# MIT-SPARK/TEASER-plusplus

Measured on AMD Instinct MI355X. Metric: registrations/sec at N=10000 correspondences, 95% outliers, higher is better.
Workload: dtype bf16x3-split MFMA + f32 filter with FP64 fix-up for K1 (bitmap bit-identical to FP64); f64 estimators

## Files before the change

include/teaser_hip.h:

```cpp
#ifndef TEASER_HIP_H_
#define TEASER_HIP_H_

#include <stddef.h>
#include <stdint.h>

#ifdef __cplusplus
extern "C" {
#endif

#define TEASER_HIP_ABI_VERSION 1

#if defined(__GNUC__)
#define TEASER_HIP_API __attribute__((visibility("default")))
#else
#define TEASER_HIP_API
#endif

typedef enum teaser_hip_status {
  TEASER_HIP_OK = 0,
  TEASER_HIP_ERR_BAD_ARG = 1,
  TEASER_HIP_ERR_HIP = 2,
  TEASER_HIP_ERR_NO_DEVICE = 3,
  TEASER_HIP_ERR_UNSUPPORTED = 4,
  TEASER_HIP_ERR_TIME_LIMIT = 5,
// ... 53 lines not shown
  float rotation_ms;
  float translation_ms;
  float d2h_ms;
  float total_ms;
  int64_t tim_graph_pairs;
  int64_t tim_graph_bytes;
  float colour_ms;
  float tim_aux_ms;
} teaser_profile_c;

typedef struct teaser_hip_solver teaser_hip_solver;

TEASER_HIP_API int32_t teaser_hip_params_default(teaser_params_c* params);

TEASER_HIP_API int32_t teaser_hip_solver_create(const teaser_params_c* params, int32_t device,
                                 teaser_hip_solver** out);
TEASER_HIP_API int32_t teaser_hip_solver_destroy(teaser_hip_solver* h);

TEASER_HIP_API int32_t teaser_hip_solver_reset(teaser_hip_solver* h, const teaser_params_c* params);
TEASER_HIP_API int32_t teaser_hip_solver_get_params(const teaser_hip_solver* h, teaser_params_c* params);

TEASER_HIP_API int32_t teaser_hip_solve(teaser_hip_solver* h, const double* src, const double* dst, int32_t n,
                         teaser_solution_c* out);

TEASER_HIP_API int32_t teaser_hip_solve_device(teaser_hip_solver* h, const double* d_src, const double* d_dst,
                                int32_t n, teaser_solution_c* out);

TEASER_HIP_API int32_t teaser_hip_solve_correspondences(teaser_hip_solver* h, const float* src_cloud_xyz,
                                         int32_t n_src, const float* dst_cloud_xyz, int32_t n_dst,
                                         const int32_t* corr_pairs ,
                                         int32_t n_corr, teaser_solution_c* out);

TEASER_HIP_API int32_t teaser_hip_solve_batch(teaser_hip_solver* h, const double* const* src,
                               const double* const* dst, const int32_t* n, int32_t batch,
                               teaser_solution_c* out );

TEASER_HIP_API int32_t teaser_hip_solve_batch_device(teaser_hip_solver* h, const double* d_src,
                                      const double* d_dst, const int64_t* point_offset,
                                      const int32_t* n, int32_t batch, teaser_solution_c* out);

enum { TEASER_HIP_INPUT_DEVICE = 0, TEASER_HIP_INPUT_HOST = 1 };
TEASER_HIP_API int32_t teaser_hip_submit_batch(teaser_hip_solver* h, const double* src, const double* dst,
                                const int64_t* point_offset, const int32_t* n, int32_t batch,
                                int32_t flags, int32_t* ticket);
TEASER_HIP_API int32_t teaser_hip_wait(teaser_hip_solver* h, int32_t ticket, teaser_solution_c* out );
TEASER_HIP_API int32_t teaser_hip_set_pipeline_depth(teaser_hip_solver* h, int32_t depth );

typedef struct teaser_hip_multi teaser_hip_multi;
TEASER_HIP_API int32_t teaser_hip_multi_create(const teaser_params_c* params, const int32_t* devices,
                                int32_t n_devices , teaser_hip_multi** out);
TEASER_HIP_API int32_t teaser_hip_multi_destroy(teaser_hip_multi* mh);
TEASER_HIP_API int32_t teaser_hip_multi_solve_batch(teaser_hip_multi* mh, const double* const* src,
                                     const double* const* dst, const int32_t* n, int32_t batch,
                                     teaser_solution_c* out );
TEASER_HIP_API int32_t teaser_hip_multi_route(teaser_hip_multi* mh, int32_t problem, teaser_hip_solver** h,
                               int32_t* local_problem);
TEASER_HIP_API int32_t teaser_hip_multi_device_count(const teaser_hip_multi* mh);

#define TEASER_HIP_COMM_ID_BYTES 128
typedef struct teaser_hip_comm teaser_hip_comm;
TEASER_HIP_API int32_t teaser_hip_comm_shard(int64_t total, int32_t rank, int32_t world, int64_t* first, int64_t* last);
TEASER_HIP_API int32_t teaser_hip_comm_unique_id(uint8_t* id );
TEASER_HIP_API int32_t teaser_hip_comm_create(const uint8_t* id, int32_t rank, int32_t world, int32_t device,
                               teaser_hip_comm** out);
TEASER_HIP_API int32_t teaser_hip_comm_destroy(teaser_hip_comm* c);
TEASER_HIP_API int32_t teaser_hip_comm_gather_solutions(teaser_hip_comm* c, const teaser_solution_c* local,
                                         int64_t n_local, int64_t total, teaser_solution_c* all );
TEASER_HIP_API int32_t teaser_hip_comm_gather_indices(teaser_hip_comm* c, teaser_hip_solver* h, int64_t n_local,
                                       int64_t total, int32_t k_max, int32_t* lens, int32_t* indices);
TEASER_HIP_API const char* teaser_hip_comm_last_error(const teaser_hip_comm* c);

TEASER_HIP_API int32_t teaser_hip_get_max_clique(teaser_hip_solver* h, int32_t problem, int32_t* buf, int64_t* len);
TEASER_HIP_API int32_t teaser_hip_get_rotation_inliers(teaser_hip_solver* h, int32_t problem, int32_t* buf,
                                        int64_t* len);
TEASER_HIP_API int32_t teaser_hip_get_translation_inliers(teaser_hip_solver* h, int32_t problem, int32_t* buf,
                                           int64_t* len);
TEASER_HIP_API int32_t teaser_hip_get_input_ordered_translation_inliers(teaser_hip_solver* h, int32_t problem,
                                                         int32_t* buf, int64_t* len);
TEASER_HIP_API int32_t teaser_hip_get_inlier_graph_bitmap(teaser_hip_solver* h, int32_t problem, uint64_t* buf,
                                           int64_t* len );
TEASER_HIP_API int32_t teaser_hip_get_degrees(teaser_hip_solver* h, int32_t problem, int32_t* buf, int64_t* len);
TEASER_HIP_API int32_t teaser_hip_get_inlier_graph_rows(teaser_hip_solver* h, int32_t problem, uint64_t* buf,
                                         int64_t* len , int32_t* stride_words);

TEASER_HIP_API int32_t teaser_hip_solve_for_rotation(teaser_hip_solver* h, const double* src, const double* dst,
                                      int32_t k, double noise_bound, double* rotation_rowmajor,
                                      uint8_t* inlier_mask, double* cost, int32_t* iterations);
TEASER_HIP_API int32_t teaser_hip_solve_for_translation(teaser_hip_solver* h, const double* src,
                                         const double* dst, int32_t k, double* translation,
                                         uint8_t* inlier_mask);
TEASER_HIP_API int32_t teaser_hip_scalar_tls(teaser_hip_solver* h, const double* x, const double* ranges,
                              int32_t n, double* estimate, uint8_t* inlier_mask);
TEASER_HIP_API int32_t teaser_hip_solve_for_scale(teaser_hip_solver* h, const double* v1, const double* v2,
                                   int64_t m, double* scale, uint8_t* inlier_mask);

TEASER_HIP_API int32_t teaser_hip_compute_fpfh(teaser_hip_solver* h, const float* cloud_xyz, int32_t n,
                                double normal_radius, double fpfh_radius, float* fpfh_out,
                                float* normals_out);
TEASER_HIP_API int32_t teaser_hip_match_features(teaser_hip_solver* h, const float* src_feat, int32_t n_src,
                                  const float* dst_feat, int32_t n_dst, int32_t dim, int32_t use_crosscheck,
                                  int32_t* pairs, int64_t* n_pairs);
TEASER_HIP_API int32_t teaser_hip_tuple_test(teaser_hip_solver* h, const float* src_xyz, int32_t n_src,
                              const float* dst_xyz, int32_t n_dst, float tuple_scale, uint64_t seed,
                              int32_t* pairs , int64_t* n_pairs );

typedef struct teaser_certifier_params_c {
  double noise_bound;
  double cbar2;
  double sub_optimality;
  double max_iterations;
  double gamma_tau;
} teaser_certifier_params_c;
typedef struct teaser_certification_c {
  int32_t is_optimal;
  int32_t iterations;
  double best_suboptimality;
} teaser_certification_c;
TEASER_HIP_API int32_t teaser_hip_certifier_params_default(teaser_certifier_params_c* p);
TEASER_HIP_API int32_t teaser_hip_certifier_warmup(int32_t device);
TEASER_HIP_API int32_t teaser_hip_certify(teaser_hip_solver* h, const teaser_certifier_params_c* p, const double* R,
                           const double* src, const double* dst, const double* theta, int32_t n,
                           teaser_certification_c* out, double* traj, int32_t traj_cap);
TEASER_HIP_API int32_t teaser_hip_certify_dual_projection(teaser_hip_solver* h, const double* W, const double* theta,
                                                          int32_t n, double* W_dual);
TEASER_HIP_API int32_t teaser_hip_certify_stages(teaser_hip_solver* h, const teaser_certifier_params_c* p, const double* R,
                                                 const double* src, const double* dst, const double* theta, int32_t n,
                                                 int32_t iteration, double* stages, double* traj, int32_t traj_cap,
                                                 teaser_certification_c* out);

TEASER_HIP_API int32_t teaser_hip_max_clique(teaser_hip_solver* h, const uint64_t* bitmap, int32_t n,
                              int32_t* clique, int32_t* clique_size, int32_t* exact_run);

TEASER_HIP_API int32_t teaser_hip_set_profiling(teaser_hip_solver* h, int32_t level );
TEASER_HIP_API int32_t teaser_hip_set_option(teaser_hip_solver* h, const char* name, int64_t value);
TEASER_HIP_API int32_t teaser_hip_get_option(const char* name, int64_t* value);
TEASER_HIP_API int32_t teaser_hip_get_profile(const teaser_hip_solver* h, teaser_profile_c* out);
TEASER_HIP_API void* teaser_hip_get_stream(teaser_hip_solver* h);
TEASER_HIP_API const char* teaser_hip_last_error(const teaser_hip_solver* h);
TEASER_HIP_API int32_t teaser_hip_abi_version(void);
TEASER_HIP_API int32_t teaser_hip_device_count(void);

typedef struct teaser_icp_params_c {
  double max_correspondence_distance;
  int32_t max_iteration;
  double relative_fitness;
  double relative_rmse;
} teaser_icp_params_c;
typedef struct teaser_icp_result_c {
  double transformation[16];
  double fitness;
  double inlier_rmse;
  int32_t iterations;
  int32_t n_correspondences;
} teaser_icp_result_c;
typedef struct teaser_hip_icp teaser_hip_icp;
TEASER_HIP_API int32_t teaser_hip_icp_params_default(teaser_icp_params_c* params);
TEASER_HIP_API int32_t teaser_hip_icp_create(int32_t device, teaser_hip_icp** out);
TEASER_HIP_API int32_t teaser_hip_icp_destroy(teaser_hip_icp* icp);
TEASER_HIP_API const char* teaser_hip_icp_last_error(const teaser_hip_icp* icp);
TEASER_HIP_API int32_t teaser_hip_icp_fill_scratch(teaser_hip_icp* icp, int32_t byte, int64_t* bytes_out);
TEASER_HIP_API int32_t teaser_hip_icp_batch(teaser_hip_icp* icp, int32_t batch, const double* const* src,
                                            const int32_t* n_src, const double* const* dst, const int32_t* n_dst,
                                            const double* init, const teaser_icp_params_c* params,
                                            teaser_icp_result_c* out, int32_t* const* corr);
TEASER_HIP_API int32_t teaser_hip_icp_solve(teaser_hip_icp* icp, const double* src, int32_t n_src,
                                            const double* dst, int32_t n_dst, const double* init,
// ... 711 lines not shown
```

teaser-plusplus_amd/__init__.py:

```python
import ctypes as C
import enum
import os
import subprocess
import typing

import numpy as np

_HERE = os.path.dirname(os.path.abspath(__file__))
_CSRC = os.path.join(_HERE, "csrc")
LIB_PATH = os.path.join(_HERE, "libteaser_hip.so")

STATUS_NAMES = {0: "OK", 1: "BAD_ARG", 2: "HIP", 3: "NO_DEVICE", 4: "UNSUPPORTED", 5: "TIME_LIMIT",
                6: "SCRATCH", 7: "OOM", 8: "BUSY"}


class TeaserHipError(RuntimeError):
    def __init__(self, status, msg=""):
        self.status = status
        super().__init__("teaser_hip status %d (%s) %s" % (status, STATUS_NAMES.get(status, "?"), msg))


class RotationEstimationAlgorithm(enum.IntEnum):
    GNC_TLS = 0
    FGR = 1
    QUATRO = 2


class InlierSelectionMode(enum.IntEnum):
    PMC_EXACT = 0
    PMC_HEU = 1
    KCORE_HEU = 2
    NONE = 3


class InlierGraphFormulation(enum.IntEnum):
    CHAIN = 0
    COMPLETE = 1


class ParamsC(C.Structure):
    _fields_ = [
        ("noise_bound", C.c_double),
        ("cbar2", C.c_double),
        ("estimate_scaling", C.c_int32),
        ("rotation_estimation_algorithm", C.c_int32),
        ("rotation_gnc_factor", C.c_double),
        ("rotation_max_iterations", C.c_int64),
        ("rotation_cost_threshold", C.c_double),
        ("rotation_tim_graph", C.c_int32),
        ("inlier_selection_mode", C.c_int32),
        ("kcore_heuristic_threshold", C.c_double),
        ("use_max_clique", C.c_int32),
        ("max_clique_exact_solution", C.c_int32),
        ("max_clique_time_limit", C.c_double),
        ("max_clique_num_threads", C.c_int32),
    ]


class SolutionC(C.Structure):
    _fields_ = [
        ("valid", C.c_int32),
        ("status", C.c_int32),
        ("scale", C.c_double),
        ("rotation", C.c_double * 9),
        ("translation", C.c_double * 3),
        ("n", C.c_int32),
        ("clique_size", C.c_int32),
        ("n_rotation_inliers", C.c_int32),
        ("n_translation_inliers", C.c_int32),
        ("gnc_cost", C.c_double),
        ("gnc_iterations", C.c_int32),
        ("clique_exact_run", C.c_int32),
        ("heuristic_size", C.c_int32),
        ("colour_uncoloured", C.c_int32),
        ("num_edges", C.c_int64),
    ]


class ProfileC(C.Structure):
    _fields_ = [
        ("h2d_ms", C.c_float),
        ("tim_graph_ms", C.c_float),
        ("tim_graph_launches", C.c_int32),
        ("degree_ms", C.c_float),
        ("heuristic_ms", C.c_float),
        ("peel_ms", C.c_float),
        ("exact_ms", C.c_float),
        ("rotation_ms", C.c_float),
        ("translation_ms", C.c_float),
        ("d2h_ms", C.c_float),
        ("total_ms", C.c_float),
        ("tim_graph_pairs", C.c_int64),
        ("tim_graph_bytes", C.c_int64),
        ("colour_ms", C.c_float),
        ("tim_aux_ms", C.c_float),
    ]


EXPORTED_SYMBOLS = [
    "teaser_hip_params_default", "teaser_hip_solver_create", "teaser_hip_solver_destroy",
    "teaser_hip_solver_reset", "teaser_hip_solver_get_params", "teaser_hip_solve",
    "teaser_hip_solve_device", "teaser_hip_solve_correspondences", "teaser_hip_solve_batch",
    "teaser_hip_solve_batch_device", "teaser_hip_get_max_clique", "teaser_hip_get_rotation_inliers",
    "teaser_hip_get_translation_inliers", "teaser_hip_get_input_ordered_translation_inliers",
    "teaser_hip_get_inlier_graph_bitmap", "teaser_hip_get_inlier_graph_rows", "teaser_hip_get_degrees", "teaser_hip_solve_for_rotation",
    "teaser_hip_solve_for_translation", "teaser_hip_scalar_tls", "teaser_hip_max_clique",
    "teaser_hip_set_profiling", "teaser_hip_set_option", "teaser_hip_get_option", "teaser_hip_get_profile", "teaser_hip_get_stream",
    "teaser_hip_last_error", "teaser_hip_abi_version", "teaser_hip_device_count", "teaser_hip_host_alloc",
    "teaser_hip_host_free",
    "teaser_hip_synth_problem", "teaser_hip_submit_batch", "teaser_hip_wait",
    "teaser_hip_set_pipeline_depth", "teaser_hip_multi_create", "teaser_hip_multi_destroy",
    "teaser_hip_multi_solve_batch", "teaser_hip_multi_route", "teaser_hip_multi_device_count",
    "teaser_hip_solve_for_scale", "teaser_hip_compute_fpfh", "teaser_hip_match_features", "teaser_hip_tuple_test",
    "teaser_hip_certifier_params_default", "teaser_hip_certify", "teaser_hip_certifier_warmup",
    "teaser_hip_certify_dual_projection", "teaser_hip_certify_stages",
    "teaser_hip_comm_shard", "teaser_hip_comm_unique_id", "teaser_hip_comm_create", "teaser_hip_comm_destroy",
    "teaser_hip_comm_gather_solutions", "teaser_hip_comm_gather_indices", "teaser_hip_comm_last_error",
    "teaser_hip_icp_params_default", "teaser_hip_icp_create", "teaser_hip_icp_destroy", "teaser_hip_icp_last_error",
    "teaser_hip_icp_fill_scratch",
    "teaser_hip_icp_batch", "teaser_hip_icp_solve", "teaser_hip_icp_estimation_default", "teaser_hip_icp_batch_ex",
    "teaser_hip_icp_solve_ex", "teaser_hip_icp_batch_cov", "teaser_hip_icp_solve_cov",
    "teaser_hip_icp_covariances_batch", "teaser_hip_icp_normals_batch", "teaser_hip_icp_batch_auto",
    "teaser_hip_icp_solve_auto",
    "teaser_hip_icp_self_knn_batch", "teaser_hip_icp_remove_statistical_outliers_batch",
    "teaser_hip_icp_remove_radius_outliers_batch", "teaser_hip_icp_set_option", "teaser_hip_icp_get_option",
    "teaser_hip_icp_knn_search_batch", "teaser_hip_icp_hybrid_search_batch", "teaser_hip_icp_radius_search_batch",
    "teaser_hip_icp_fpfh_batch", "teaser_hip_icp_boundary_points_batch",
    "teaser_hip_icp_frame_default", "teaser_hip_icp_unproject_depth_batch", "teaser_hip_icp_project_depth_batch",
    "teaser_hip_icp_iss_params_default", "teaser_hip_icp_iss_keypoints_batch",
    "teaser_hip_icp_cluster_dbscan_batch", "teaser_hip_icp_farthest_point_down_sample_batch",
    "teaser_hip_icp_information_batch", "teaser_hip_icp_information",
    "teaser_hip_icp_color_default", "teaser_hip_icp_batch_color", "teaser_hip_icp_solve_color",
    "teaser_hip_icp_color_gradients_batch",
    "teaser_hip_voxel_create", "teaser_hip_voxel_destroy", "teaser_hip_voxel_last_error",
    "teaser_hip_voxel_fill_scratch",
    "teaser_hip_voxel_down_sample_batch", "teaser_hip_voxel_down_sample",
    "teaser_hip_features_create", "teaser_hip_features_destroy", "teaser_hip_features_last_error",
    "teaser_hip_features_fill_scratch",
    "teaser_hip_features_set_budgets", "teaser_hip_features_fpfh_batch", "teaser_hip_features_match_batch",
    "teaser_hip_features_correspondences_batch", "teaser_hip_features_knn_batch",
    "teaser_hip_features_match_knn_batch", "teaser_hip_features_correspondences_knn_batch",
    "teaser_hip_features_tuple_test_batch",
    "teaser_hip_posegraph_create", "teaser_hip_posegraph_destroy", "teaser_hip_posegraph_last_error",
    "teaser_hip_posegraph_fill_scratch",
    "teaser_hip_posegraph_option_default", "teaser_hip_posegraph_optimize_batch", "teaser_hip_posegraph_optimize",
    "teaser_hip_posegraph_linearize_batch", "teaser_hip_posegraph_linearize",
    "teaser_hip_ransac_create", "teaser_hip_ransac_destroy", "teaser_hip_ransac_last_error",
    "teaser_hip_ransac_fill_scratch",
    "teaser_hip_ransac_params_default", "teaser_hip_ransac_correspondence_batch", "teaser_hip_ransac_correspondence",
    "teaser_hip_ransac_set_option", "teaser_hip_ransac_get_option", "teaser_hip_ransac_trials_batch",
    "teaser_hip_fgr_create", "teaser_hip_fgr_destroy", "teaser_hip_fgr_last_error",
    "teaser_hip_fgr_fill_scratch", "teaser_hip_fgr_params_default",
    "teaser_hip_fgr_correspondence_batch", "teaser_hip_fgr_correspondence", "teaser_hip_fgr_set_option",
    "teaser_hip_fgr_get_option", "teaser_hip_fgr_iterations_batch",
    "teaser_hip_plane_create", "teaser_hip_plane_destroy", "teaser_hip_plane_last_error",
    "teaser_hip_plane_fill_scratch",
    "teaser_hip_plane_params_default", "teaser_hip_plane_segment_batch", "teaser_hip_plane_segment",
    "teaser_hip_plane_set_option", "teaser_hip_plane_get_option", "teaser_hip_plane_trials_batch",
    "teaser_hip_tsdf_volume_default", "teaser_hip_tsdf_create", "teaser_hip_tsdf_destroy", "teaser_hip_tsdf_last_error",
    "teaser_hip_tsdf_fill_scratch",
    "teaser_hip_tsdf_reset", "teaser_hip_tsdf_integrate_batch", "teaser_hip_tsdf_extract_point_cloud",
    "teaser_hip_tsdf_extract_voxel_point_cloud", "teaser_hip_tsdf_download", "teaser_hip_tsdf_upload",
    "teaser_hip_tsdf_extract_triangle_mesh", "teaser_hip_tsdf_mesh_tables", "teaser_hip_tsdf_view_default",
    "teaser_hip_tsdf_ray_cast_views",
    "teaser_hip_stsdf_volume_default", "teaser_hip_stsdf_create", "teaser_hip_stsdf_destroy", "teaser_hip_stsdf_last_error",
    "teaser_hip_stsdf_fill_scratch", "teaser_hip_stsdf_last_phases", "teaser_hip_stsdf_reset", "teaser_hip_stsdf_integrate_frames",
    "teaser_hip_stsdf_extract_point_cloud", "teaser_hip_stsdf_extract_voxel_point_cloud", "teaser_hip_stsdf_block_count",
    "teaser_hip_stsdf_block_keys", "teaser_hip_stsdf_download_blocks", "teaser_hip_stsdf_upload_blocks",
    "teaser_hip_stsdf_ray_cast_views", "teaser_hip_stsdf_extract_triangle_mesh",
    "teaser_hip_icp_odometry_option_default", "teaser_hip_icp_rgbd_odometry_batch",
    "teaser_hip_icp_rgbd_odometry_pyramid_batch",
]


def build(force=False):
    args = ["make", "-C", _CSRC, "-j8"]
    if force:
        args.append("-B")
    subprocess.check_call(args, stdout=subprocess.DEVNULL)
    return LIB_PATH


_lib = None
_vp, _ip, _dp = C.c_void_p, C.POINTER(C.c_int32), C.POINTER(C.c_double)
_u8p, _i64p, _u64p = C.POINTER(C.c_uint8), C.POINTER(C.c_int64), C.POINTER(C.c_uint64)


def lib():
    global _lib
    if _lib is not None:
        return _lib
    if not os.path.exists(LIB_PATH):
        raise ImportError("%s is missing: run __graft_entry__.build() (make -C %s)" % (LIB_PATH, _CSRC))
    os.environ.setdefault("GPU_MAX_HW_QUEUES", "8")
    L = C.CDLL(LIB_PATH)
    L.teaser_hip_host_alloc.argtypes = [C.c_size_t, C.POINTER(_vp)]
    L.teaser_hip_host_free.argtypes = [_vp]
    L.teaser_hip_params_default.argtypes = [C.POINTER(ParamsC)]
    L.teaser_hip_solver_create.argtypes = [C.POINTER(ParamsC), C.c_int32, C.POINTER(_vp)]
    L.teaser_hip_solver_destroy.argtypes = [_vp]
    L.teaser_hip_solver_reset.argtypes = [_vp, C.POINTER(ParamsC)]
    L.teaser_hip_solver_get_params.argtypes = [_vp, C.POINTER(ParamsC)]
    L.teaser_hip_solve.argtypes = [_vp, _dp, _dp, C.c_int32, C.POINTER(SolutionC)]
    L.teaser_hip_solve_device.argtypes = [_vp, _vp, _vp, C.c_int32, C.POINTER(SolutionC)]
    L.teaser_hip_solve_correspondences.argtypes = [_vp, C.POINTER(C.c_float), C.c_int32,
                                                   C.POINTER(C.c_float), C.c_int32, _ip, C.c_int32,
                                                   C.POINTER(SolutionC)]
    L.teaser_hip_solve_batch.argtypes = [_vp, C.POINTER(_dp), C.POINTER(_dp), _ip, C.c_int32,
                                         C.POINTER(SolutionC)]
    L.teaser_hip_solve_batch_device.argtypes = [_vp, _vp, _vp, _i64p, _ip, C.c_int32,
                                                C.POINTER(SolutionC)]
    for nm in ("teaser_hip_get_max_clique", "teaser_hip_get_rotation_inliers",
               "teaser_hip_get_translation_inliers",
               "teaser_hip_get_input_ordered_translation_inliers", "teaser_hip_get_degrees"):
        getattr(L, nm).argtypes = [_vp, C.c_int32, _ip, _i64p]
    L.teaser_hip_get_inlier_graph_bitmap.argtypes = [_vp, C.c_int32, _u64p, _i64p]
    L.teaser_hip_get_inlier_graph_rows.argtypes = [_vp, C.c_int32, _u64p, _i64p, _ip]
    L.teaser_hip_solve_for_rotation.argtypes = [_vp, _dp, _dp, C.c_int32, C.c_double, _dp, _u8p, _dp, _ip]
    L.teaser_hip_solve_for_translation.argtypes = [_vp, _dp, _dp, C.c_int32, _dp, _u8p]
    L.teaser_hip_scalar_tls.argtypes = [_vp, _dp, _dp, C.c_int32, _dp, _u8p]
    L.teaser_hip_solve_for_scale.argtypes = [_vp, _dp, _dp, C.c_int64, _dp, _u8p]
    _fp = C.POINTER(C.c_float)
    L.teaser_hip_compute_fpfh.argtypes = [_vp, _fp, C.c_int32, C.c_double, C.c_double, _fp, _fp]
    L.teaser_hip_match_features.argtypes = [_vp, _fp, C.c_int32, _fp, C.c_int32, C.c_int32, C.c_int32, _ip, _i64p]
    L.teaser_hip_tuple_test.argtypes = [_vp, _fp, C.c_int32, _fp, C.c_int32, C.c_float, C.c_uint64, _ip, _i64p]
    L.teaser_hip_certify.argtypes = [_vp, C.c_void_p, _dp, _dp, _dp, _dp, C.c_int32, C.c_void_p, _dp, C.c_int32]
    L.teaser_hip_certify_dual_projection.argtypes = [_vp, _dp, _dp, C.c_int32, _dp]
    L.teaser_hip_certify_stages.argtypes = [_vp, C.c_void_p, _dp, _dp, _dp, _dp, C.c_int32, C.c_int32, _dp, _dp,
                                            C.c_int32, C.c_void_p]
    L.teaser_hip_max_clique.argtypes = [_vp, _u64p, C.c_int32, _ip, _ip, _ip]
    L.teaser_hip_submit_batch.argtypes = [_vp, _vp, _vp, _i64p, _ip, C.c_int32, C.c_int32, _ip]
    L.teaser_hip_wait.argtypes = [_vp, C.c_int32, C.POINTER(SolutionC)]
    L.teaser_hip_set_pipeline_depth.argtypes = [_vp, C.c_int32]
    L.teaser_hip_multi_create.argtypes = [C.POINTER(ParamsC), _ip, C.c_int32, C.POINTER(_vp)]
    L.teaser_hip_multi_destroy.argtypes = [_vp]
    L.teaser_hip_multi_solve_batch.argtypes = [_vp, C.POINTER(_dp), C.POINTER(_dp), _ip, C.c_int32,
                                               C.POINTER(SolutionC)]
    L.teaser_hip_multi_route.argtypes = [_vp, C.c_int32, C.POINTER(_vp), _ip]
    L.teaser_hip_multi_device_count.argtypes = [_vp]
    L.teaser_hip_set_profiling.argtypes = [_vp, C.c_int32]
    L.teaser_hip_set_option.argtypes = [_vp, C.c_char_p, C.c_int64]
    L.teaser_hip_get_option.argtypes = [C.c_char_p, C.POINTER(C.c_int64)]
    L.teaser_hip_get_profile.argtypes = [_vp, C.POINTER(ProfileC)]
    L.teaser_hip_get_stream.argtypes = [_vp]
    L.teaser_hip_get_stream.restype = _vp
    L.teaser_hip_last_error.argtypes = [_vp]
    L.teaser_hip_last_error.restype = C.c_char_p
    L.teaser_hip_synth_problem.argtypes = [C.c_uint64, C.c_int32, C.c_double, C.c_double, _dp, _dp,
                                           _dp, _dp, _u8p]
    from . import icp as _icp
    _icp.declare(L)
    from . import outlier as _outlier
    _outlier.declare(L)
    from . import search as _search
    _search.declare(L)
    from . import fpfh_open3d as _fpfh_open3d
    _fpfh_open3d.declare(L)
    from . import boundary as _boundary
    _boundary.declare(L)
    from . import rgbd as _rgbd
    _rgbd.declare(L)
    from . import keypoints as _keypoints
    _keypoints.declare(L)
    from . import cluster as _cluster
    _cluster.declare(L)
    from . import fps as _fps
    _fps.declare(L)
    from . import voxel as _voxel
    _voxel.declare(L)
    from . import features as _features
    _features.declare(L)
    from . import posegraph as _posegraph
    _posegraph.declare(L)
    from . import ransac as _ransac
    _ransac.declare(L)
    from . import fgr as _fgr
    _fgr.declare(L)
    from . import plane as _plane
    _plane.declare(L)
    from . import tsdf as _tsdf
    _tsdf.declare(L)
    from . import odometry as _odometry
    _odometry.declare(L)
    _lib = L
    return L


def set_option(name, value):
    rc = lib().teaser_hip_set_option(None, name.encode(), int(value))
    if rc != 0:
        raise TeaserHipError(rc, "unknown option %r" % name)


def get_option(name):
    v = C.c_int64()
    rc = lib().teaser_hip_get_option(name.encode(), C.byref(v))
    if rc != 0:
        raise TeaserHipError(rc, "unknown option %r" % name)
    return v.value

# ... 854 lines not shown
```

teaser-plusplus_amd/csrc/internal.h:

```cpp
#pragma once

#include <hip/hip_runtime.h>
#include <stdint.h>

#include <atomic>
#include <mutex>
#include <algorithm>
#include <vector>

#include "teaser_hip.h"

namespace thip {

constexpr int kWave = 64;
constexpr int kMaxStarts = 16;
constexpr int kPeelRounds = 3;
constexpr int kSmallCap = 768;

struct ProbDesc {
  int32_t n;
  int32_t W;
  int64_t pt_off;
  int64_t bm_off;
  int64_t w_off;
// ... 33 lines not shown
  double gnc_cost;
};

struct EstParams {
  double noise_bound;
  double cbar2;
  double gnc_factor;
  double cost_threshold;
  int64_t max_iterations;
  int32_t tim_graph;
  int32_t algorithm;
};

struct DynLdsOptIn {
  static constexpr int kMaxDevices = 64;
  std::mutex m;
  int granted[kMaxDevices] = {};
  void ensure(const void* func, int bytes) {
    int dev = 0;
    (void)hipGetDevice(&dev);
    const bool tracked = dev >= 0 && dev < kMaxDevices;
    std::lock_guard<std::mutex> lk(m);
    if (tracked && granted[dev] >= bytes) return;
    (void)hipFuncSetAttribute(func, hipFuncAttributeMaxDynamicSharedMemorySize, bytes);
    if (tracked) granted[dev] = bytes;
  }
};


enum Setting {
  S_K1_FP64,
  S_FUSED_EST,
  S_SCALE_SORT64,
  S_SCALE_BATCH,
  S_SCALE_MID_BATCH,
  S_SPEC_BOUNDS,
  S_FINISHER,
  S_COPY_STREAM,
  S_H2D_KERNEL,
  S_DEPTH,
  S_STAGGER,
  S_K1_STREAM,
  S_TAIL_CUS,
  S_TAIL_CU_BLOCK,
  S_K4_LDS_STACK,
  S_K4_DONATE,
  S_K4_DONATE_AFTER,
  S_K4_HUNGRY,
  S_K4_EXPAND,
  S_K4_DEBUG,
  S_HEU_BLOCKS,
  S_GREEDY_THREADS,
  S_FIXUP_WGS,
  S_K4_WAVES,
  S_K4_LB_BONUS,
  S_DEG_CLOSURE,
  S_GREEDY_SMALL,
  S_DEG_CLOSURE_WGS,
  S_SCALE_HULL,
  S_SCALE_HULL_SYNC,
  S_COLOUR_PERSISTENT,
  S_HEU_SKIP_CLOSED,
  S_REFERENCE_SNAPSHOT,
  S_TAIL_SKIP,
  S_COLOUR_MIS,
  S_COLOUR_MIS_ANY,
  S_COUNT
};
int64_t setting(Setting id);
bool set_setting(const char* name, int64_t value);
bool get_setting(const char* name, int64_t* value);

void launch_tim_graph(hipStream_t s, const ProbDesc* d_desc, int batch, int max_n,
                      const double* d_src, const double* d_dst, uint64_t* d_bitmap,
                      double noise_bound, double cbar2, int mode, const ProbState* d_state);
int64_t tim_prep_bytes(int batch);
int64_t tim_operand_bytes(int64_t total_tiles);
int64_t tim_work_items(const int32_t* n, int batch);
int tim_probe_worklist(const void* d_prep, const void* d_work, int64_t work_cap, int batch, int max_n,
                       unsigned long long* regions_out, int64_t* stride_words, int64_t* used_regions,
                       unsigned int* seg_counts);
int64_t tim_prep_fill_segments(void* host_prep, const int32_t* n, int batch);
constexpr int kTimUpperOnly = 8, kTimMirror = 3, kTimMirrorOpen = 4;
void launch_tim_graph_mfma(hipStream_t s, int phase, const ProbDesc* d_desc, int batch, int max_n,
                           int64_t total_tiles, const double* d_src, const double* d_dst,
                           void* d_pk, void* d_prep, void* d_work, int64_t work_cap,
                           uint64_t* d_bitmap, ProbState* d_state, int32_t* d_deg, double noise_bound,
                           double cbar2);
void launch_degrees(hipStream_t s, const ProbDesc* d_desc, int batch, int max_n,
                    const uint64_t* d_bitmap, int32_t* d_deg, ProbState* d_state);
int heuristic_blocks_per_problem(int batch, int max_W, int expected_open = -1 );
void launch_heuristic(hipStream_t s, const ProbDesc* d_desc, int batch, int max_W,
                      const uint64_t* d_bitmap, const int32_t* d_deg, ProbState* d_state,
                      int32_t* d_start_cliques , int64_t total_n,
                      int32_t* d_trace , int32_t* d_clique ,
                      int nblk = 0 ,
                      int rows = 0 );
int64_t greedy_small_scratch_bytes(int batch);
int launch_greedy_small(hipStream_t s, const ProbDesc* d_desc, int batch, int max_small_n, const uint64_t* d_bitmap,
                        const int32_t* d_deg, ProbState* d_state, void* d_slots, int32_t* d_best_seen);
int64_t degree_closure_scratch_bytes(int batch);
void launch_degree_closure(hipStream_t s, const ProbDesc* d_desc, int batch, const uint64_t* d_bitmap,
                           const int32_t* d_deg, ProbState* d_state, int32_t* d_clique, void* d_scratch,
                           int32_t* d_counters);
void launch_peel(hipStream_t s, const ProbDesc* d_desc, int batch, int max_n, int max_W,
                 const uint64_t* d_bitmap, const int32_t* d_deg, ProbState* d_state,
                 uint64_t* d_alive_a, uint64_t* d_alive_b);

struct ExactProb {
  int32_t prob;
  int32_t n2, W2;
  int32_t n_roots;
  int32_t lb;
  int32_t n_waves;
  int32_t wave0;
  int32_t lds_bitmap;
  int32_t max_deg;
  int32_t use_x;
  int64_t order_off;
  int64_t bm_off;
  int64_t arena_off;
  int64_t arena_bytes;
  int64_t clique_off;
  int32_t ctrl[8];
};
constexpr int64_t kExactLdsBitmapBytes = 128 * 1024;
constexpr int kExactXCap = 512;
constexpr int kExactExpandPasses = 1;
constexpr int kExactCounterInts = 96;
void launch_exact_count(hipStream_t s, const ProbDesc* d_desc, ExactProb* d_probs, int nprob, int max_W,
                        const uint64_t* d_bitmap, const uint64_t* d_alive, const int32_t* d_deg,
                        const ProbState* d_state, const int32_t* d_xlist, const int32_t* d_keep,
                        uint64_t* d_cand_bits , uint64_t* d_x_bits ,
                        bool speculative = false );
void launch_exact_build(hipStream_t s, const ProbDesc* d_desc, const ExactProb* d_probs, int nprob, int max_W,
                        int max_n2, const uint64_t* d_bitmap, const int32_t* d_deg, const uint64_t* d_cand_bits,
                        const uint64_t* d_x_bits, int32_t* d_order_pool, unsigned long long* d_key_pool,
                        uint64_t* d_bitmap_pool);
void launch_exact_clique(hipStream_t s, ExactProb* d_probs, int nprob, int total_waves, int max_W2,
                         int64_t max_lds_bitmap_bytes, const uint64_t* d_bitmap_pool, char* d_arena_pool,
                         int64_t arena_bytes , int arena_waves ,
                         int32_t* d_clique_pool, char* d_task_pool, int64_t task_pool_bytes,
                         int32_t* d_counters , int64_t deadline_ticks);
void launch_exact_finish(hipStream_t s, const ProbDesc* d_desc, const ExactProb* d_probs, int nprob, int max_W,
                         const int32_t* d_order_pool, const int32_t* d_clique_pool, int32_t* d_clique,
                         ProbState* d_state);
void certifier_warmup_async(int device);
struct CertCapture {
  int iteration;
  double* out;
  bool captured;
};
int certify_on_device(hipStream_t s, const double* R, const double* src, const double* dst, const double* theta, int N,
                      double noise_bound, double cbar2, double sub_optimality, double max_iterations,
                      double gamma_tau, int* is_optimal, double* best_suboptimality, std::vector<double>* traj,
                      CertCapture* cap = nullptr);
int dual_projection_on_device(hipStream_t s, const double* W, const double* theta, int N, double* W_dual);
constexpr int kColourMaxLb = 4096;
constexpr int kColourRounds = 16;
inline int64_t colour_counts_bytes(int nsel) { return 4 * (int64_t)nsel * (kColourRounds + 2 + 16); }
constexpr int kMisMaxColours = 1024;
inline bool colour_mis_fits(int n, int lb) { return lb >= 2 && (int64_t)n <= 128 * (int64_t)std::min(lb, kMisMaxColours); }
int64_t colour_mis_bytes(int nsel, int max_n);
constexpr int kRootPruneCap = 512;
constexpr int kRootPruneSlices = 32;
constexpr int kRootPruneRows = 16;
void launch_colour_bound(hipStream_t s, const ProbDesc* d_desc, const int32_t* d_sel, int nsel,
                         int max_n, const uint64_t* d_bitmap, const uint64_t* d_alive,
                         const int32_t* d_clique, ProbState* d_state, int32_t* d_colour,
                         int32_t* d_tent, int32_t* d_xlist, int32_t* d_class_lists ,
                         int32_t* d_list_a, int32_t* d_list_b, int32_t* d_counts ,
                         uint64_t* d_bits , int64_t total_w, int64_t total_n, int rounds,
                         void* d_mis = nullptr ,
                         const int32_t* d_deg = nullptr );

void launch_kcore_heuristic(hipStream_t s, const ProbDesc* d_desc, int batch, const uint64_t* d_bitmap,
                            const int32_t* d_deg, ProbState* d_state, int32_t* d_rem_deg, int32_t* d_core,
                            int32_t* d_clique, double threshold);

void launch_gnc_tls(hipStream_t s, const ProbDesc* d_desc, int batch, const double* d_src,
                    const double* d_dst, const int32_t* d_clique, ProbState* d_state,
                    EstParams ep, double* d_weights , int32_t* d_rot_inliers,
                    const int64_t* d_tim_off);
void launch_tls_translation(hipStream_t s, const ProbDesc* d_desc, int batch, const double* d_src,
                            const double* d_dst, const int32_t* d_clique, ProbState* d_state,
                            EstParams ep, char* d_scratch, int64_t scratch_stride,
                            int32_t* d_trans_inliers);
// ... 49 lines not shown
```

teaser-plusplus_amd/csrc/kernels_graph.hip:

```cpp
#include <algorithm>
#include <utility>
#include <vector>

#include <cstdio>
#include <cstdlib>

#include "internal.h"
#include "fixup_item.h"
#include "fixup_regions.h"
#include "k1_consts.h"
#include "wave_utils.h"

namespace thip {

struct EdgeConst {
  double beta;
  double beta2;
  double m2beta2;
  double beta4;
  double s_hat;
};

__device__ __forceinline__ bool tim_edge_exact(double ax, double ay, double az, double bx,
                                               double by, double bz, double beta) {
// ... 389 lines not shown
    const double* a = src + 3 * (d.pt_off + i);
    const double* b = dst + 3 * (d.pt_off + i);
    const float sx = (float)((a[0] - prep_centre(pr, 0, 0)) * g), sy = (float)((a[1] - prep_centre(pr, 0, 1)) * g),
                sz = (float)((a[2] - prep_centre(pr, 0, 2)) * g);
    const float dx = (float)((b[0] - prep_centre(pr, 1, 0)) * g), dy = (float)((b[1] - prep_centre(pr, 1, 1)) * g),
                dz = (float)((b[2] - prep_centre(pr, 1, 2)) * g);
    const double na_d = ((double)sx * sx + (double)sy * sy) + (double)sz * sz;
    const double nb_d = ((double)dx * dx + (double)dy * dy) + (double)dz * dz;
    const float na = (float)na_d, nb = (float)nb_d;
    const double beta2s = k1c::pow2_d(kexp - 2);
    const float kappa = (float)k1c::pow2_d(kexp);
    const float delta_row = (float)(nb_d - na_d - beta2s);
    const float delta_col = (float)(nb_d - na_d);
    unsigned short A[48], B[32];
    for (int k = 0; k < 48; ++k) A[k] = 0;
    for (int k = 0; k < 32; ++k) B[k] = 0;
    const float cs[3] = {sx, sy, sz}, cd[3] = {dx, dy, dz};
    const unsigned short one = 0x3c00;
    float h, m, l;
    for (int c = 0; c < 3; ++c) {
      f16_split3(cs[c], &h, &m, &l);
      B[3 * c] = f16_bits(2.0f * h); B[3 * c + 1] = f16_bits(2.0f * m); B[3 * c + 2] = B[3 * c];
      A[3 * c] = f16_bits(h); A[3 * c + 1] = A[3 * c]; A[3 * c + 2] = f16_bits(m);
      A[32 + 3 * c] = f16_bits(kappa * h); A[32 + 3 * c + 1] = A[32 + 3 * c]; A[32 + 3 * c + 2] = f16_bits(kappa * m);
      f16_split3(cd[c], &h, &m, &l);
      B[16 + 3 * c] = f16_bits(-2.0f * h); B[16 + 3 * c + 1] = f16_bits(-2.0f * m); B[16 + 3 * c + 2] = B[16 + 3 * c];
      A[16 + 3 * c] = f16_bits(h); A[16 + 3 * c + 1] = A[16 + 3 * c]; A[16 + 3 * c + 2] = f16_bits(m);
    }
    f16_split3(na, &h, &m, &l);
    B[9] = f16_bits(-h); B[10] = f16_bits(-m);
    A[32 + 9] = f16_bits(kappa); A[32 + 10] = A[32 + 9];
    B[11] = one; B[12] = one; B[13] = one;
    B[14] = f16_bits(kappa); B[15] = B[14];
    A[32 + 14] = f16_bits(-h); A[32 + 15] = f16_bits(-m);
    f16_split3(delta_row, &h, &m, &l);
    A[11] = f16_bits(h); A[12] = f16_bits(m); A[13] = f16_bits(l);
    f16_split3(delta_col, &h, &m, &l);
    A[25] = one; A[26] = one; A[27] = one; B[25] = f16_bits(h); B[26] = f16_bits(m); B[27] = f16_bits(l);
    TimOperandTile3* tile = ops + d.w_off + (ip >> 6);
    const int gq = (ip >> 5) & 1, cc = ip & 31;
    for (int mf = 0; mf < 3; ++mf)
      for (int hh = 0; hh < 2; ++hh) {
        const unsigned short* pa = A + 16 * mf + 8 * hh;
        tile->a[gq][mf][hh][cc] = make_uint4(pa[0] | ((unsigned int)pa[1] << 16), pa[2] | ((unsigned int)pa[3] << 16),
                                             pa[4] | ((unsigned int)pa[5] << 16), pa[6] | ((unsigned int)pa[7] << 16));
        if (mf >= kTimColOperands) continue;
        const unsigned short* pb = B + 16 * mf + 8 * hh;
        tile->b[gq][mf][hh][cc] = make_uint4(pb[0] | ((unsigned int)pb[1] << 16), pb[2] | ((unsigned int)pb[3] << 16),
                                             pb[4] | ((unsigned int)pb[5] << 16), pb[6] | ((unsigned int)pb[7] << 16));
      }
    mx = na > nb ? na : nb;
    if (!(mx == mx)) mx = INFINITY;
    if (ip < d.n) deg[d.pt_off + ip] = 0;
  }
  for (int o = 32; o > 0; o >>= 1) {
    const float t = __shfl_xor(mx, o, 64);
    mx = t > mx ? t : mx;
  }
  if ((threadIdx.x & 63) == 0 && mx > 0.f) atomicMax(&prep[blockIdx.y].r2_bits, __float_as_uint(mx));
}
#endif

__global__ void tim_prep_consts_kernel(TimPrep* __restrict__ prep, int batch, double beta) {
  const int p = blockIdx.x * blockDim.x + threadIdx.x;
  if (p >= batch) return;
  const k1c::ConstsXY c = k1c::consts_xy(beta, k1c::norm_shift(prep_half_extent(prep + p)), prep[p].r2_bits);
  prep[p].band_c = c.C;
  prep[p].use_mfma = c.use_mfma;
}
#ifdef TEASER_K1_LAB
__global__ void tim_prep_consts3_kernel(TimPrep* __restrict__ prep, int batch, double beta) {
  const int p = blockIdx.x * blockDim.x + threadIdx.x;
  if (p >= batch) return;
  const k1c::Consts c = k1c::consts(beta, k1c::norm_shift(prep_half_extent(prep + p)), prep[p].r2_bits);
  prep[p].band_c = c.C;
  prep[p].use_mfma = c.use_mfma;
}
#endif


constexpr bool kK1Pipe = false, kK1Plain = true;
constexpr int kK1Chunks = 1, kK1Occ = 3;

template <bool PIPE, bool PLAIN, int OCC, int CHUNKS, bool LOWER, bool UW3 = false>
__global__ __launch_bounds__(256, OCC) void tim_graph_mfma3_kernel(
    const ProbDesc* __restrict__ descs, const double* __restrict__ src,
    const double* __restrict__ dst, const void* __restrict__ ops, const TimPrep* __restrict__ prep,
    uint64_t* __restrict__ bitmap, double beta, int gyr,
    unsigned long long* __restrict__ work, unsigned int* __restrict__ work_count,
    ProbState* __restrict__ states, int32_t* __restrict__ deg, unsigned long long* __restrict__ regions, int Tmax) {
  const ProbDesc d = descs[blockIdx.y];
  const int n = d.n, W = d.W;
  const int T = W, S = bm_stride(W);
  int Ig, X;
  fxr::decode_block((int)blockIdx.x, (int)gridDim.x, gyr, CHUNKS, &Ig, &X);
  constexpr int kBlockColTiles = kMfmaColTiles * CHUNKS;
  const int I0 = Ig * kMfmaRowTiles, Jbase = X * kBlockColTiles;
  auto region_of = [&](int wv, int chunk) -> unsigned long long* {
    const int Iw = I0 + wv, Xc = X * CHUNKS + chunk;
    return fxr::is_cell(Iw, Xc, Tmax) ? regions + fxr::region_offset((int)blockIdx.y, Tmax, Iw, Xc) : nullptr;
  };
  auto zero_regions = [&]() {
    if ((threadIdx.x & 63) < CHUNKS) {
      unsigned long long* r = region_of((int)(threadIdx.x >> 6), (int)(threadIdx.x & 63));
      if (r) r[0] = 0ull;
    }
  };
  if (I0 >= T || Jbase >= T || Jbase + kBlockColTiles - 1 < I0) {
    zero_regions();
    return;
  }
  const int lane = threadIdx.x & 63;
  const int wave = __builtin_amdgcn_readfirstlane(threadIdx.x >> 6);
  const int I = I0 + wave;

  const double* __restrict__ ps = src + 3 * d.pt_off;
  const double* __restrict__ pd = dst + 3 * d.pt_off;
  uint64_t* __restrict__ bm = bitmap + d.bm_off;
  __shared__ __attribute__((aligned(16))) uint64_t lds_own[kMfmaRowTiles][64][kMfmaColTiles + 1];
  static_assert(sizeof(lds_own[0]) >= sizeof(double) * 64 * 6 && sizeof(lds_own[0]) >= 8 * kWorkBuf, "aliased buffers");
  __shared__ __attribute__((aligned(16))) uint64_t lds_tr[kMfmaColTiles][64][kMfmaRowTiles];
  constexpr int kRowOps = UW3 ? 3 : kTimRowOperands;
  constexpr int kTileBytes = 2 * (kRowOps + kTimColOperands) * 1024, kColBase = 2 * kRowOps * 1024;
  static_assert(UW3 || (kTileBytes == (int)sizeof(TimOperandTile2) && kColBase == (int)offsetof(TimOperandTile2, b)), "tile layout");
  const char* __restrict__ qt = reinterpret_cast<const char*>(ops) + (size_t)d.w_off * kTileBytes;
  const int h = lane >> 5, c = lane & 31;
  typedef unsigned int u32x4 __attribute__((ext_vector_type(4)));
  const __amdgpu_buffer_rsrc_t q_rsrc = __builtin_amdgcn_make_buffer_rsrc(
      (void*)qt, 0, (int)((unsigned int)T * (unsigned int)kTileBytes), 0x00020000);
  auto load_op = [&](int tile, int side, int g, int m) -> uint4 {
    const int soff = tile * kTileBytes + (side ? kColBase + (g * kTimColOperands + m) * 1024 : (g * kRowOps + m) * 1024);
    const u32x4 v = __builtin_amdgcn_raw_buffer_load_b128(q_rsrc, lane * 16, soff, 0);
    return make_uint4(v.x, v.y, v.z, v.w);
  };
  f16x8 ar[2][kRowOps];
  {
    const int It = min(I, T - 1);
    for (int rt = 0; rt < 2; ++rt)
      for (int m = 0; m < kRowOps; ++m) ar[rt][m] = __builtin_bit_cast(f16x8, load_op(It, 0, rt, m));
  }
  const bool rowvalid = I < T;
  const uint64_t rowmask = !rowvalid ? 0ull : (n - I * 64 >= 64) ? ~0ull : ((1ull << (n - I * 64)) - 1ull);
  const int Jfirst = max(Jbase, I), Jend = min(Jbase + kBlockColTiles, T);
  uint4 bX[kTimColOperands], bY[kTimColOperands];
  {
    const int Jf = min(Jfirst, T - 1);
    for (int m = 0; m < kTimColOperands; ++m) bX[m] = load_op(Jf, 1, 0, m);
    if (PIPE)
      for (int m = 0; m < kTimColOperands; ++m) bY[m] = load_op(Jf, 1, 1, m);
  }
  const TimPrep pr = prep[blockIdx.y];
  if (!pr.use_mfma) {
    EdgeConst kc;
    kc.beta = beta;
    kc.beta2 = beta * beta;
    kc.m2beta2 = -2.0 * kc.beta2;
    kc.beta4 = kc.beta2 * kc.beta2;
    kc.s_hat = 1.0;
    if (I < T)
      for (int jb = Jbase; jb < Jbase + kBlockColTiles; jb += kColTilesPerWave)
        if (!(jb + kColTilesPerWave - 1 < I || jb >= T))
          tim_wave_fp64<0>(ps, pd, bm, n, W, I, jb, kc, reinterpret_cast<double*>(&lds_own[wave][0][0]));
    zero_regions();
    return;
  }
  const __amdgpu_buffer_rsrc_t deg_rsrc = __builtin_amdgcn_make_buffer_rsrc(
      (void*)(deg + d.pt_off), 0, (int)((unsigned int)n * 4u), 0x00020000);
  const __amdgpu_buffer_rsrc_t bm_rsrc = __builtin_amdgcn_make_buffer_rsrc(
      (void*)bm, 0, (int)((unsigned int)n * (unsigned int)S * 8u), 0x00020000);
  int degacc = 0;
  const int cq = c - 4 * h;
  const int selfq = (cq >= 0 && (cq & 4) == 0) ? ((cq & 3) | ((cq >> 3) << 2)) : -1;
  unsigned int flags = 0;
  const float thr = pr.band_c;

  struct Acc {
    f32x16 U, W;
  };
  static_assert(!(UW3 && PIPE), "the three-MFMA lab variant has the flat schedule only");
  auto mf = [&](Acc& a, const f16x8(&arow)[kRowOps], const uint4(&b)[kTimColOperands]) {
    f32x16 z;
    for (int k = 0; k < 16; ++k) z[k] = 0.f;
    a.W = __builtin_amdgcn_mfma_f32_32x32x16_f16(arow[0], __builtin_bit_cast(f16x8, b[0]), z, 0, 0, 0);
    a.U = __builtin_amdgcn_mfma_f32_32x32x16_f16(arow[1], __builtin_bit_cast(f16x8, b[1]), a.W, 0, 0, 0);
  };
  auto epi = [&](const Acc& a, bool self_tile) -> unsigned int {
    unsigned int colbits = 0;
    float m = INFINITY;
#pragma unroll
    for (int qp = 7; qp >= 0; --qp) {
      float d0, d1;
      if (PLAIN) {
        d0 = __builtin_fmaf(a.U[2 * qp], a.U[2 * qp], a.W[2 * qp]);
        d1 = __builtin_fmaf(a.U[2 * qp + 1], a.U[2 * qp + 1], a.W[2 * qp + 1]);
      } else {
        const f32x2 u2 = {a.U[2 * qp], a.U[2 * qp + 1]}, w2 = {a.W[2 * qp], a.W[2 * qp + 1]};
        const f32x2 d2 = __builtin_elementwise_fma(u2, u2, w2);
        d0 = d2.x;
        d1 = d2.y;
      }
      float v0 = __builtin_fabsf(d0), v1 = __builtin_fabsf(d1);
      if (self_tile) {
        v0 = (selfq == 2 * qp) ? INFINITY : v0;
        v1 = (selfq == 2 * qp + 1) ? INFINITY : v1;
      }
      m = __builtin_fminf(__builtin_fminf(m, v0), v1);
      colbits = __builtin_amdgcn_alignbit(colbits, __float_as_uint(d1), (qp & 1) ? 27 : 31);
      colbits = __builtin_amdgcn_alignbit(colbits, __float_as_uint(d0), 31);
    }
    asm("v_cmp_nlt_f32_e32 vcc, %2, %1\n\tv_addc_co_u32_e32 %0, vcc, %0, %0, vcc" : "+v"(flags) : "v"(m), "s"(thr) : "vcc");
    return colbits;
  };
  const unsigned int sel16 = (lane & 16) ? 0x03020706u : 0x01000504u;
  auto finish_tile = [&](const int J, const bool diag, const unsigned int (&tr)[2][2]) {
    const int j0 = J * 64;
    unsigned int tw[2], ow[2];
#pragma unroll
    for (int rt = 0; rt < 2; ++rt) {
      const auto r = __builtin_amdgcn_permlane32_swap(tr[0][rt], tr[1][rt], false, false);
      tw[rt] = merge_gap_bytes(r[0], r[1]);
      unsigned int x;
      {
        const auto sw = __builtin_amdgcn_permlane16_swap(tw[rt], tw[rt], false, false);
        x = __builtin_amdgcn_perm(sw[0], sw[1], sel16);
      }
#pragma unroll
      for (int st = 1; st < 5; ++st) {
        const int j = 16 >> st;
        unsigned int p;
        switch (st) {
          case 1: p = __builtin_amdgcn_update_dpp(0u, x, 0x128, 0xf, 0xf, true); break;
          case 2:
            p = __builtin_amdgcn_update_dpp(0u, x, 0x141, 0xf, 0xf, true);
            p = __builtin_amdgcn_update_dpp(0u, p, 0x1b, 0xf, 0xf, true);
            break;
          case 3: p = __builtin_amdgcn_update_dpp(0u, x, 0x4e, 0xf, 0xf, true); break;
          default: p = __builtin_amdgcn_update_dpp(0u, x, 0xb1, 0xf, 0xf, true); break;
        }
        const bool up = (lane & j) != 0;
        const unsigned int shifted = __builtin_amdgcn_alignbit(p, p, up ? j : 32 - j);
        const unsigned int km[5] = {0x0000FFFFu, 0x00FF00FFu, 0x0F0F0F0Fu, 0x33333333u, 0x55555555u};
        const unsigned int keep = up ? ~km[st] : km[st];
        x = bit_select(keep, x, shifted);
      }
      ow[rt] = x;
    }
    const auto ro = __builtin_amdgcn_permlane32_swap(ow[0], ow[1], false, false);
    uint64_t ownw = ((uint64_t)ro[1] << 32) | ro[0];
    const uint64_t trw = ((uint64_t)tw[1] << 32) | tw[0];
    const uint64_t colmask = (n - j0 >= 64) ? ~0ull : ((1ull << (n - j0)) - 1ull);
    ownw &= colmask;
    if (diag) ownw &= ~(1ull << lane);
    lds_own[wave][lane][(J - Jbase) & (kMfmaColTiles - 1)] = ownw;
    degacc += __builtin_popcountll(ownw);
    const uint64_t trw_out = diag ? 0ull : (trw & rowmask);
    lds_tr[(J - Jbase) & (kMfmaColTiles - 1)][lane][wave] = trw_out;
  };

  auto body_flat = [&](const int J, auto diag_tag) {
    constexpr bool DIAG = decltype(diag_tag)::value;
    unsigned int tr[2][2];
#pragma unroll
    for (int ct = 0; ct < 2; ++ct) {
      const f16x8 b0 = __builtin_bit_cast(f16x8, bX[0]), b1 = __builtin_bit_cast(f16x8, bX[1]);
      const int Jn = (ct == 0 || J + 1 >= Jend) ? J : J + 1, gn = ct ^ 1;
      f32x16 z;
      for (int k = 0; k < 16; ++k) z[k] = 0.f;
      Acc acc[2];
      __builtin_amdgcn_s_setprio(2);
      if constexpr (UW3) {
        acc[0].U = __builtin_amdgcn_mfma_f32_32x32x16_f16(ar[0][0], b0, z, 0, 0, 0);
        __builtin_amdgcn_sched_barrier(0);
        acc[1].U = __builtin_amdgcn_mfma_f32_32x32x16_f16(ar[1][0], b0, z, 0, 0, 0);
        __builtin_amdgcn_sched_barrier(0);
        acc[0].W = __builtin_amdgcn_mfma_f32_32x32x16_f16(ar[0][kRowOps - 1], b0, z, 0, 0, 0);
        __builtin_amdgcn_sched_barrier(0);
        acc[1].W = __builtin_amdgcn_mfma_f32_32x32x16_f16(ar[1][kRowOps - 1], b0, z, 0, 0, 0);
      } else {
        acc[0].W = __builtin_amdgcn_mfma_f32_32x32x16_f16(ar[0][0], b0, z, 0, 0, 0);
        __builtin_amdgcn_sched_barrier(0);
        acc[1].W = __builtin_amdgcn_mfma_f32_32x32x16_f16(ar[1][0], b0, z, 0, 0, 0);
      }
      __builtin_amdgcn_sched_barrier(0);
      bX[0] = load_op(Jn, 1, gn, 0);
      __builtin_amdgcn_sched_barrier(0);
      acc[0].U = __builtin_amdgcn_mfma_f32_32x32x16_f16(ar[0][1], b1, UW3 ? acc[0].U : acc[0].W, 0, 0, 0);
      __builtin_amdgcn_sched_barrier(0);
      acc[1].U = __builtin_amdgcn_mfma_f32_32x32x16_f16(ar[1][1], b1, UW3 ? acc[1].U : acc[1].W, 0, 0, 0);
      __builtin_amdgcn_sched_barrier(0);
      bX[1] = load_op(Jn, 1, gn, 1);
      __builtin_amdgcn_s_setprio(0);
      __builtin_amdgcn_sched_barrier(0);
#pragma unroll
      for (int rt = 0; rt < 2; ++rt) tr[ct][rt] = epi(acc[rt], DIAG && ct == rt);
    }
    finish_tile(J, DIAG, tr);
  };

  Acc accA, accB;
#define TIM_K1_INTERLEAVE(N)                                                              \
  __builtin_amdgcn_sched_group_barrier(0x008, 1, 0);                                      \
  __builtin_amdgcn_sched_group_barrier(0x002, N, 0);                                      \
  __builtin_amdgcn_sched_group_barrier(0x008, 1, 0);                                      \
  __builtin_amdgcn_sched_group_barrier(0x002, N, 0);                                      \
  __builtin_amdgcn_sched_group_barrier(0x008, 1, 0);                                      \
  __builtin_amdgcn_sched_group_barrier(0x002, N, 0);                                      \
  __builtin_amdgcn_sched_group_barrier(0x008, 1, 0);                                      \
  __builtin_amdgcn_sched_group_barrier(0x002, N, 0)
  constexpr int kEpiShare = PLAIN ? 13 : 9;
  auto body_pipe = [&](const int J, auto diag_tag) {
    constexpr bool DIAG = decltype(diag_tag)::value;
    const int Jn = min(J + 1, Jend - 1);
    unsigned int tr[2][2];
    mf(accB, ar[1], bX);
    tr[0][0] = epi(accA, DIAG);
    TIM_K1_INTERLEAVE(kEpiShare);
    __builtin_amdgcn_sched_barrier(0);
    for (int m = 0; m < kTimColOperands; ++m) bX[m] = load_op(Jn, 1, 0, m);
    mf(accA, ar[0], bY);
    tr[0][1] = epi(accB, false);
    __builtin_amdgcn_sched_group_barrier(0x020, kTimColOperands, 0);
    TIM_K1_INTERLEAVE(kEpiShare);
    __builtin_amdgcn_sched_barrier(0);
    mf(accB, ar[1], bY);
    tr[1][0] = epi(accA, false);
    TIM_K1_INTERLEAVE(kEpiShare);
    __builtin_amdgcn_sched_barrier(0);
    for (int m = 0; m < kTimColOperands; ++m) bY[m] = load_op(Jn, 1, 1, m);
    mf(accA, ar[0], bX);
    tr[1][1] = epi(accB, DIAG);
    finish_tile(J, DIAG, tr);
    __builtin_amdgcn_sched_group_barrier(0x020, kTimColOperands, 0);
    TIM_K1_INTERLEAVE(kEpiShare + 16);
    __builtin_amdgcn_sched_barrier(0);
  };

#undef TIM_K1_INTERLEAVE
  unsigned long long* wbuf = reinterpret_cast<unsigned long long*>(&lds_own[wave][0][0]);
  bool primed = false;
#pragma nounroll
  for (int chunk = 0; chunk < CHUNKS; ++chunk) {
    const int Jc0 = Jbase + chunk * kMfmaColTiles, Jc1 = min(Jc0 + kMfmaColTiles, Jend);
    unsigned long long* const region = region_of(wave, chunk);
    if (Jc0 >= Jend) {
      if (lane == 0 && region) region[0] = 0ull;
      continue;
    }
    const int Ja = rowvalid ? max(Jc0, Jfirst) : Jc1;
    if (Ja < Jc1) {
      int J = Ja;
      if (PIPE) {
        if (!primed) {
          mf(accA, ar[0], bX);
          __builtin_amdgcn_sched_barrier(0);
          primed = true;
        }
        if (J == I) {
          body_pipe(J, std::true_type());
          ++J;
        }
#pragma nounroll
        for (; J < Jc1; ++J) body_pipe(J, std::false_type());
      } else {
        if (J == I) {
          body_flat(J, std::true_type());
          ++J;
        }
#pragma nounroll
        for (; J < Jc1; ++J) body_flat(J, std::false_type());
      }
    }
    const int nact = max(Jc1 - Ja, 0);
    {
      __syncthreads();
#pragma unroll
      for (int it = 0; it < (kMfmaColTiles * 64) / 256; ++it) {
        const int idx = it * 256 + (int)threadIdx.x, Jr = idx >> 6, r = idx & 63, J = Jc0 + Jr, j = J * 64 + r;
        const uint4 lo = *reinterpret_cast<const uint4*>(&lds_tr[Jr][r][0]);
        const uint4 hi = *reinterpret_cast<const uint4*>(&lds_tr[Jr][r][2]);
        const bool rowok = J < Jc1 && j < n;
        const unsigned int base = ((unsigned int)j * (unsigned int)S + (unsigned int)I0) * 8u;
        if (Jc0 > I0 + 3 && I0 + 3 < T) {
          const int cnt = (__builtin_popcount(lo.x) + __builtin_popcount(lo.y)) + (__builtin_popcount(lo.z) + __builtin_popcount(lo.w)) +
                          (__builtin_popcount(hi.x) + __builtin_popcount(hi.y)) + (__builtin_popcount(hi.z) + __builtin_popcount(hi.w));
          if (LOWER) {
            __builtin_amdgcn_raw_buffer_store_b128(u32x4{lo.x, lo.y, lo.z, lo.w}, bm_rsrc, rowok ? base : kOobOffset, 0, 0);
            __builtin_amdgcn_raw_buffer_store_b128(u32x4{hi.x, hi.y, hi.z, hi.w}, bm_rsrc, rowok ? base + 16u : kOobOffset, 0, 0);
          }
          __builtin_amdgcn_raw_ptr_buffer_atomic_add_i32(cnt, deg_rsrc, (rowok && cnt) ? (unsigned int)j * 4u : kOobOffset, 0, 0);
          continue;
        }
        bool ok[4];
        for (int k = 0; k < 4; ++k) ok[k] = rowok && I0 + k < T && I0 + k < J;
        const unsigned int w32[8] = {lo.x, lo.y, lo.z, lo.w, hi.x, hi.y, hi.z, hi.w};
        int cnt = 0;
        for (int k = 0; k < 4; ++k) cnt += ok[k] ? __builtin_popcount(w32[2 * k]) + __builtin_popcount(w32[2 * k + 1]) : 0;
        if (!LOWER) {
        } else if (ok[3]) {
          __builtin_amdgcn_raw_buffer_store_b128(u32x4{lo.x, lo.y, lo.z, lo.w}, bm_rsrc, base, 0, 0);
          __builtin_amdgcn_raw_buffer_store_b128(u32x4{hi.x, hi.y, hi.z, hi.w}, bm_rsrc, base + 16u, 0, 0);
        } else {
          for (int k = 0; k < 3; ++k)
            __builtin_amdgcn_raw_buffer_store_b64(u32x2{w32[2 * k], w32[2 * k + 1]}, bm_rsrc,
                                                  ok[k] ? base + 8u * k : kOobOffset, 0, 0);
        }
        __builtin_amdgcn_raw_ptr_buffer_atomic_add_i32(cnt, deg_rsrc, cnt ? (unsigned int)j * 4u : kOobOffset, 0, 0);
      }
      if (CHUNKS > 1) __syncthreads();
    }
    if (nact > 0) {
      const int kk = lane & 7, J = Jc0 + kk;
      const bool pad = J >= T, colok = (J >= Ja && J < Jc1) || pad;
      const unsigned int off0 = ((unsigned int)(I * 64 + (lane >> 3)) * (unsigned int)S + (unsigned int)J) * 8u;
#pragma unroll
      for (int it = 0; it < 8; ++it) {
        const int r = it * 8 + (lane >> 3);
        const uint64_t w = pad ? 0ull : lds_own[wave][r][kk];
        __builtin_amdgcn_raw_buffer_store_b64(u32x2{(unsigned int)w, (unsigned int)(w >> 32)}, bm_rsrc,
                                              (colok && I * 64 + r < n) ? off0 + (unsigned int)it * 64u * (unsigned int)S : kOobOffset,
                                              0, 0);
      }
    }
    int wcount = 0;
    {
      unsigned int vf = flags;
      if (I * 64 + 4 * h >= n) vf &= ~0xAAAAAAAAu;
      if (I * 64 + 32 + 4 * h >= n) vf &= ~0x55555555u;
      if (T - 1 >= Ja && T - 1 < Jc1 && (n & 63)) {
        const int sh = 4 * (Jc1 - T);
        if ((T - 1) * 64 + c >= n) vf &= ~(0xCu << sh);
        if ((T - 1) * 64 + 32 + c >= n) vf &= ~(0x3u << sh);
      }
      if (__builtin_amdgcn_ballot_w64(vf != 0u) != 0ull) {
        const int mine = __builtin_popcount(vf);
        int base = 0, total = 0;
#pragma unroll
        for (int bit = 0; bit < 6; ++bit) {
          const uint64_t m = __builtin_amdgcn_ballot_w64(((mine >> bit) & 1) != 0);
          base += (int)__builtin_amdgcn_mbcnt_hi((unsigned int)(m >> 32), __builtin_amdgcn_mbcnt_lo((unsigned int)m, 0u)) << bit;
          total += __builtin_popcountll(m) << bit;
        }
        if (total > kWorkBuf) {
          if (lane == 0) states[blockIdx.y].k1_overflow = 1;
        } else {
          int kk = base;
#pragma nounroll
          while (vf) {
            const int pos = 31 - __builtin_clz(vf);
            vf &= ~(1u << pos);
            const int J = Ja + (nact - 1 - (pos >> 2));
            const int ct = ((pos >> 1) & 1) ^ 1, rt = (pos & 1) ^ 1;
            const unsigned int rowp = (unsigned int)(I * 64 + 32 * rt + 4 * h);
            const unsigned int colp = (unsigned int)(J * 64 + 32 * ct + c);
            const uint64_t tword = lds_tr[(J - Jbase) & (kMfmaColTiles - 1)][32 * ct + c][wave];
            wbuf[kk++] = fxi::pack(rowp, colp, fxi::gather_bits(tword, rt, h));
          }
          wcount = total;
        }
      }
    }
    flags = 0;
    {
      const int nreg = !region ? 0 : (wcount < kRegionItems ? wcount : kRegionItems);
      if (lane == 0 && region) region[0] = (unsigned long long)nreg;
      if (lane < nreg) region[1 + lane] = wbuf[lane];
      if (wcount > nreg) {
        const int extra = wcount - nreg;
        unsigned int base = 0;
        if (lane == 0) base = atomicAdd(work_count + blockIdx.y, (unsigned int)extra);
        base = __builtin_amdgcn_readfirstlane(base);
        if (base + (unsigned int)extra > pr.seg_cap) {
          if (lane == 0) states[blockIdx.y].k1_overflow = 1;
        } else {
          unsigned long long* seg = work + (((size_t)pr.seg_off_hi << 32) | (size_t)pr.seg_off_lo);
#pragma nounroll
          for (int k2i = lane; k2i < extra; k2i += 64) seg[base + k2i] = wbuf[nreg + k2i];
        }
      }
    }
  }
  if (rowvalid)
    __builtin_amdgcn_raw_ptr_buffer_atomic_add_i32(degacc, deg_rsrc, (unsigned int)(I * 64 + lane) * 4u, 0, 0);
}

__global__ __launch_bounds__(256) void tim_fixup_group_kernel(const ProbDesc* __restrict__ descs, int batch,
                                                              const double* __restrict__ src,
                                                              const double* __restrict__ dst,
                                                              uint64_t* __restrict__ bitmap, double beta,
                                                              const unsigned long long* __restrict__ work,
                                                              const unsigned int* __restrict__ work_count,
                                                              ProbState* __restrict__ states,
                                                              int32_t* __restrict__ deg,
                                                              const unsigned long long* __restrict__ regions,
                                                              int Tmax,
                                                              const TimPrep* __restrict__ prep, int upper) {
  TAIL_WAVE_PRIO();
  const int prob = blockIdx.y;
  const unsigned int total = work_count[prob];
  const TimPrep tpr = prep[prob];
  const unsigned int cap = tpr.seg_cap;
  const ProbDesc d = descs[prob];
  const int n = d.n, W = d.W, S = bm_stride(W);
  if (total > cap) {
    const int64_t words = (int64_t)n * S;
    uint64_t* bm = bitmap + d.bm_off;
    for (int64_t w = (int64_t)blockIdx.x * 256 + threadIdx.x; w < words; w += (int64_t)gridDim.x * 256) bm[w] = 0;
    if (blockIdx.x == 0 && threadIdx.x == 0) states[prob].k1_overflow = 1;
    return;
  }
  int32_t* dg = deg + d.pt_off;
  if (!tpr.use_mfma) {
    const uint64_t* bm = bitmap + d.bm_off;
    const int lane = threadIdx.x & 63;
    for (int row = blockIdx.x * 4 + (threadIdx.x >> 6); row < n; row += gridDim.x * 4) {
      const uint64_t* r = bm + (int64_t)row * S;
      int c = 0;
      for (int w = lane; w < W; w += 64) c += __popcll(r[w]);
      c = wave_sum_i(c);
      if (lane == 0) dg[row] = c;
    }
    return;
  }
  const double* ps = src + 3 * d.pt_off;
  const double* pd = dst + 3 * d.pt_off;
  unsigned int* bm32 = reinterpret_cast<unsigned int*>(bitmap + d.bm_off);
  EdgeConst kc;
  kc.beta = beta;
  kc.beta2 = beta * beta;
  kc.m2beta2 = -2.0 * kc.beta2;
  kc.beta4 = kc.beta2 * kc.beta2;
  kc.s_hat = 1.0;
  const int lane = threadIdx.x & 63, q = lane & 15, sub = lane >> 4, wave = threadIdx.x >> 6;
  const int rq = (q & 3) + 8 * (q >> 2);
  __shared__ double row_pts[4][64][6];
  __shared__ __attribute__((aligned(16))) double col_pts[4][64][6];
  auto resolve = [&](unsigned long long it, bool valid, auto staged, int tile, int slot) {
    constexpr bool STAGED = decltype(staged)::value;
    int r = fxi::row0(it) + rq, col = fxi::col(it);
    valid = valid && r < n && col < n && r != col;
    r = valid ? r : (STAGED ? tile * 64 : 0);
    col = valid ? col : 0;
    double sx, sy, sz, dx, dy, dz, cx, cy, cz, ex, ey, ez;
    if (STAGED) {
      const double* rp = row_pts[wave][r & 63];
      sx = rp[0]; sy = rp[1]; sz = rp[2]; dx = rp[3]; dy = rp[4]; dz = rp[5];
      const double* cp = col_pts[wave][slot];
      cx = cp[0]; cy = cp[1]; cz = cp[2]; ex = cp[3]; ey = cp[4]; ez = cp[5];
    } else {
      sx = ps[3 * r]; sy = ps[3 * r + 1]; sz = ps[3 * r + 2];
      dx = pd[3 * r]; dy = pd[3 * r + 1]; dz = pd[3 * r + 2];
      cx = ps[3 * col]; cy = ps[3 * col + 1]; cz = ps[3 * col + 2];
      ex = pd[3 * col]; ey = pd[3 * col + 1]; ez = pd[3 * col + 2];
    }
    unsigned int* wp = bm32 + 2 * ((int64_t)r * S + (col >> 6)) + ((col >> 5) & 1);
    const unsigned int bit = 1u << (col & 31);
    bool prov;
    if (STAGED && (r >> 6) != (col >> 6)) {
      prov = fxi::bit(it, q);
    } else {
      prov = (*wp & bit) != 0u;
    }
    const double ax = cx - sx, ay = cy - sy, az = cz - sz, bx = ex - dx, by = ey - dy, bz = ez - dz;
    bool unc, shortp;
    bool e = tim_edge_fast(ax, ay, az, bx, by, bz, kc, &unc, &shortp);
    e |= shortp;
    if (unc) e = tim_edge_exact(ax, ay, az, bx, by, bz, beta);
    if (!valid || prov == e) return;
    atomicXor(wp, bit);
    atomicAdd(dg + r, e ? 1 : -1);
    if ((r >> 6) != (col >> 6)) {
      if (!upper) atomicXor(bm32 + 2 * ((int64_t)col * S + (r >> 6)) + ((r >> 5) & 1), 1u << (r & 31));
      atomicAdd(dg + col, e ? 1 : -1);
    }
  };
  __shared__ unsigned long long queue[4][2 * kRegionWords];
  static_assert(kRegionWords == 64, "one region = one 64-lane load");
  const int T = W, nch = fxr::n_chunks(T);
  auto round = [&](int cnt, int tile) {
    if (lane < cnt) {
      const int col = min(fxi::col(queue[wave][lane]), n - 1);
      double* cp = col_pts[wave][lane];
      const double c0 = ps[3 * col], c1 = ps[3 * col + 1], c2 = ps[3 * col + 2];
      const double e0 = pd[3 * col], e1 = pd[3 * col + 1], e2 = pd[3 * col + 2];
      cp[0] = c0; cp[1] = c1; cp[2] = c2; cp[3] = e0; cp[4] = e1; cp[5] = e2;
    }
    __builtin_amdgcn_fence(__ATOMIC_ACQ_REL, "wavefront");
#pragma nounroll
    for (int base = 0; base < cnt; base += 4) {
      const int k = base + sub;
      resolve(queue[wave][k], k < cnt, std::true_type(), tile, k);
    }
    __builtin_amdgcn_fence(__ATOMIC_ACQ_REL, "wavefront");
  };
  const int wv = blockIdx.x * 4 + wave, nwv = gridDim.x * 4, npairs = (T + 1) >> 1;
  for (int pi = wv; pi < npairs; pi += nwv) {
    for (int side = 0; side < 2; ++side) {
      const int tile = side ? T - 1 - pi : pi;
      if (side && tile == pi) break;
      {
        const int pr = min(tile * 64 + lane, n - 1);
        double* rp = row_pts[wave][lane];
        rp[0] = ps[3 * pr]; rp[1] = ps[3 * pr + 1]; rp[2] = ps[3 * pr + 2];
        rp[3] = pd[3 * pr]; rp[4] = pd[3 * pr + 1]; rp[5] = pd[3 * pr + 2];
      }
      const int Xc0 = fxr::first_chunk(tile);
      const unsigned long long* reg = regions + fxr::region_offset(prob, Tmax, tile, Xc0);
      int qn = 0;
      unsigned long long mine = reg[lane];
      for (int Xc = Xc0; Xc < nch; ++Xc) {
        const unsigned long long cur = mine;
        if (Xc + 1 < nch) mine = reg[(size_t)(Xc + 1 - Xc0) * kRegionWords + lane];
        const int cnt = min((int)__builtin_amdgcn_readfirstlane((unsigned int)cur), kRegionItems);
        if (cnt <= 0) continue;
        if (lane >= 1 && lane <= cnt) queue[wave][qn + lane - 1] = cur;
        qn += cnt;
        if (qn >= kRegionWords) {
          __builtin_amdgcn_fence(__ATOMIC_ACQ_REL, "wavefront");
          round(kRegionWords, tile);
          qn -= kRegionWords;
          const unsigned long long moved = queue[wave][kRegionWords + lane];
          __builtin_amdgcn_fence(__ATOMIC_ACQ_REL, "wavefront");
          if (lane < qn) queue[wave][lane] = moved;
        }
      }
      if (qn > 0) {
        __builtin_amdgcn_fence(__ATOMIC_ACQ_REL, "wavefront");
        round(qn, tile);
      }
    }
  }
  const unsigned long long* seg = work + (((size_t)tpr.seg_off_hi << 32) | (size_t)tpr.seg_off_lo);
  const unsigned int ngrp = gridDim.x * 16;
  for (unsigned int w = (blockIdx.x * 256 + threadIdx.x) >> 4; w < total; w += ngrp) resolve(seg[w], true, std::false_type(), 0, 0);
}

constexpr int kMirrorRun = 8;
__global__ __launch_bounds__(256) void tim_mirror_lower_kernel(const ProbDesc* __restrict__ descs,
                                                               uint64_t* __restrict__ bitmap,
                                                               const ProbState* __restrict__ states, int skip_closed) {
  const ProbDesc d = descs[blockIdx.y];
  const int n = d.n, W = d.W, T = W, S = bm_stride(W);
  if (T < 2 || (skip_closed && states[blockIdx.y].deg_closed)) return;
  const int lane = threadIdx.x & 63;
  const int runs = (T + kMirrorRun - 1) / kMirrorRun;
  uint64_t* bm = bitmap + d.bm_off;
  for (int wv = blockIdx.x * 4 + (int)(threadIdx.x >> 6); wv < T * runs; wv += gridDim.x * 4) {
    const int J = wv / runs, Ia = (wv % runs) * kMirrorRun, Ib = min(Ia + kMirrorRun, J);
    if (Ia >= Ib) continue;
    uint64_t out[kMirrorRun];
#pragma unroll
    for (int k = 0; k < kMirrorRun; ++k) {
      out[k] = 0ull;
      if (Ia + k >= Ib) continue;
      const uint64_t x = bm[(int64_t)(64 * (Ia + k) + lane) * S + J];
#pragma unroll
      for (int c = 0; c < 64; ++c) {
        const uint64_t m = __builtin_amdgcn_ballot_w64(((x >> c) & 1ull) != 0ull);
        out[k] = lane == c ? m : out[k];
      }
    }
    const int row = 64 * J + lane;
    if (row < n) {
#pragma unroll
      for (int k = 0; k < kMirrorRun; ++k)
        if (Ia + k < Ib) bm[(int64_t)row * S + Ia + k] = out[k];
    }
  }
}

void launch_tim_graph(hipStream_t s, const ProbDesc* d_desc, int batch, int max_n,
                      const double* d_src, const double* d_dst, uint64_t* d_bitmap,
                      double noise_bound, double cbar2, int mode, const ProbState* d_state) {
  if (batch <= 0 || max_n <= 0) return;
  const int T = (max_n + 63) / 64;
  const double beta = 2 * noise_bound * sqrt(cbar2);
  const int gx = (T + kColTilesPerBlock - 1) / kColTilesPerBlock, gy = T;
  dim3 grid(gx * gy, batch);
  if (mode == 0)
    hipLaunchKernelGGL(tim_graph_kernel<0>, grid, dim3(256), 0, s, d_desc, d_src, d_dst, d_bitmap,
                       beta, gx, gy, d_state);
  else
    hipLaunchKernelGGL(tim_graph_kernel<1>, grid, dim3(256), 0, s, d_desc, d_src, d_dst, d_bitmap,
                       beta, gx, gy, d_state);
}

int64_t tim_prep_bytes(int batch) { return (int64_t)batch * ((int64_t)sizeof(TimPrep) + 4) + 64; }
#ifdef TEASER_K1_LAB
int64_t tim_operand_bytes(int64_t total_tiles) { return total_tiles * (int64_t)sizeof(TimOperandTile3); }
#else
int64_t tim_operand_bytes(int64_t total_tiles) { return total_tiles * (int64_t)sizeof(TimOperandTile2); }
#endif

static int tim_mfma_blocks(int T, int chunks) { return fxr::blocks(T, chunks); }
static int64_t tim_region_words(int max_n) { return fxr::arena_words((max_n + 63) / 64); }

static int64_t tim_segment_items(int n) {
  const int64_t seg = std::max<int64_t>((int64_t)n * (n - 1) / 2 / 256, 1 << 16);
  return std::min<int64_t>(seg, 0x7fffffffll);
}
int64_t tim_work_items(const int32_t* n, int batch) {
  int64_t segs = 0;
  int max_n = 0;
  for (int b = 0; b < batch; ++b) {
    segs += tim_segment_items(n[b]);
    max_n = std::max(max_n, n[b]);
  }
  return segs + tim_region_words(max_n) * std::max(batch, 1);
}
int64_t tim_prep_fill_segments(void* host_prep, const int32_t* n, int batch) {
  TimPrep* pr = reinterpret_cast<TimPrep*>(host_prep);
  int64_t off = 0;
  for (int b = 0; b < batch; ++b) {
    const int64_t seg = tim_segment_items(n[b]);
    pr[b].seg_off_lo = (unsigned int)((uint64_t)off & 0xffffffffu);
    pr[b].seg_off_hi = (unsigned int)((uint64_t)off >> 32);
    pr[b].seg_cap = (unsigned int)seg;
    off += seg;
  }
  return off;
}

int tim_probe_worklist(const void* d_prep, const void* d_work, int64_t work_cap, int batch, int max_n,
                       unsigned long long* regions_out, int64_t* stride_words, int64_t* used_regions,
                       unsigned int* seg_counts) {
  const int64_t reg_words = tim_region_words(max_n);
  *stride_words = reg_words;
  *used_regions = fxr::cells((max_n + 63) / 64);
  if (!regions_out) return 0;
  const unsigned long long* regions = reinterpret_cast<const unsigned long long*>(d_work) + (work_cap - reg_words * (int64_t)batch);
  hipError_t e = hipMemcpy(regions_out, regions, (size_t)reg_words * (size_t)batch * 8, hipMemcpyDeviceToHost);
  if (e == hipSuccess && seg_counts)
    e = hipMemcpy(seg_counts, reinterpret_cast<const char*>(d_prep) + sizeof(TimPrep) * (size_t)batch, 4 * (size_t)batch,
                  hipMemcpyDeviceToHost);
  return (int)e;
}

#ifdef TEASER_K1_LAB
struct K1Variant { int pipe, plain, chunks, occ4, uw3; };
static K1Variant k1_lab_variant() {
  const char* ev = getenv("TEASER_K1_VARIANT");
  const int v = ev ? atoi(ev) : 0;
  K1Variant k;
  k.uw3 = (v / 10000) % 10 != 0;
  k.occ4 = (v / 1000) % 10 != 0;
  k.pipe = v % 10 != 0;
  k.plain = (v / 10) % 10 != 0;
  k.chunks = 1 << ((v / 100) % 10);
  return k;
}
#endif

void launch_tim_graph_mfma(hipStream_t s, int phase, const ProbDesc* d_desc, int batch, int max_n,
                           int64_t total_tiles, const double* d_src, const double* d_dst,
                           void* d_pk, void* d_prep, void* d_work, int64_t work_cap,
                           uint64_t* d_bitmap, ProbState* d_state, int32_t* d_deg, double noise_bound,
                           double cbar2) {
  if (batch <= 0 || max_n <= 0) return;
  (void)total_tiles;
  const int T = (max_n + 63) / 64;
  if (phase == kTimMirror || phase == kTimMirrorOpen) {
    if (T < 2) return;
    const int waves = T * ((T + kMirrorRun - 1) / kMirrorRun);
    hipLaunchKernelGGL(tim_mirror_lower_kernel, dim3((unsigned)std::min(64, (waves + 3) / 4), batch), dim3(256), 0, s, d_desc,
                       d_bitmap, d_state, phase == kTimMirrorOpen ? 1 : 0);
    return;
  }
#ifdef TEASER_K1_LAB
  const bool upper = false;
#else
  const bool upper = (phase & kTimUpperOnly) != 0;
#endif
  phase &= ~kTimUpperOnly;
  const double beta = 2 * noise_bound * sqrt(cbar2);
  TimPrep* prep = reinterpret_cast<TimPrep*>(d_prep);
  unsigned long long* work = reinterpret_cast<unsigned long long*>(d_work);
  unsigned int* work_count = reinterpret_cast<unsigned int*>(reinterpret_cast<char*>(d_prep) +
                                                            sizeof(TimPrep) * (size_t)batch);
  const int64_t reg_words = tim_region_words(max_n);
  unsigned long long* regions = work + (work_cap - reg_words * (int64_t)batch);
#ifdef TEASER_K1_LAB
  const K1Variant lab = k1_lab_variant();
#endif
  if (phase == 0) {
    hipLaunchKernelGGL(tim_prep_bbox_kernel, dim3((max_n + 1023) / 1024, batch), dim3(256), 0, s, d_desc,
                       d_src, d_dst, prep);
#ifdef TEASER_K1_LAB
    if (lab.uw3) {
      hipLaunchKernelGGL(tim_prep_pack3_kernel, dim3((T * 64 + 255) / 256, batch), dim3(256), 0, s, d_desc, d_src,
                         d_dst, prep, reinterpret_cast<TimOperandTile3*>(d_pk), d_deg, beta);
      hipLaunchKernelGGL(tim_prep_consts3_kernel, dim3((batch + 63) / 64), dim3(64), 0, s, prep, batch, beta);
      return;
    }
#endif
    hipLaunchKernelGGL(tim_prep_pack2_kernel, dim3((T * 64 + 255) / 256, batch), dim3(256), 0, s, d_desc, d_src,
                       d_dst, prep, reinterpret_cast<TimOperandTile2*>(d_pk), d_deg, beta);
    hipLaunchKernelGGL(tim_prep_consts_kernel, dim3((batch + 63) / 64), dim3(64), 0, s, prep, batch, beta);
  } else if (phase == 1) {
    const int gyr = (T + kMfmaRowTiles - 1) / kMfmaRowTiles;
#define TIM_K1_LAUNCH(PIPE, PLAIN, CHUNKS) TIM_K1_LAUNCH_OCC(PIPE, PLAIN, kK1Occ, CHUNKS, true)
#define TIM_K1_LAUNCH_OCC(PIPE, PLAIN, OCC, CHUNKS, ...)                                                                       \
  hipLaunchKernelGGL((tim_graph_mfma3_kernel<PIPE, PLAIN, OCC, CHUNKS, __VA_ARGS__>), dim3(tim_mfma_blocks(T, CHUNKS), batch), \
                     dim3(256), 0, s, d_desc, d_src, d_dst, (const void*)d_pk, prep, d_bitmap, beta, gyr, work, work_count,    \
                     d_state, d_deg, regions, T)
#ifdef TEASER_K1_LAB
#define TIM_K1_LAB_CASE(PIPE, PLAIN)                             \
  if (lab.pipe == (PIPE ? 1 : 0) && lab.plain == (PLAIN ? 1 : 0)) { \
    if (lab.chunks == 1) { TIM_K1_LAUNCH(PIPE, PLAIN, 1); }      \
    else if (lab.chunks == 2) { TIM_K1_LAUNCH(PIPE, PLAIN, 2); } \
    else { TIM_K1_LAUNCH(PIPE, PLAIN, 4); }                      \
  }
    if (lab.uw3) {
      if (lab.plain) { TIM_K1_LAUNCH_OCC(false, true, kK1Occ, 1, true, true); } else { TIM_K1_LAUNCH_OCC(false, false, kK1Occ, 1, true, true); }
    } else if (lab.occ4) {
      if (lab.plain) { TIM_K1_LAUNCH_OCC(false, true, 4, 1, true); } else { TIM_K1_LAUNCH_OCC(false, false, 4, 1, true); }
    } else {
      TIM_K1_LAB_CASE(false, false)
      TIM_K1_LAB_CASE(false, true)
      TIM_K1_LAB_CASE(true, false)
      TIM_K1_LAB_CASE(true, true)
    }
#undef TIM_K1_LAB_CASE
#else
    if (upper) {
      TIM_K1_LAUNCH_OCC(kK1Pipe, kK1Plain, kK1Occ, kK1Chunks, false);
    } else {
      TIM_K1_LAUNCH(kK1Pipe, kK1Plain, kK1Chunks);
    }
#endif
#undef TIM_K1_LAUNCH
#undef TIM_K1_LAUNCH_OCC
  } else {
    const int64_t forced_wgs = setting(S_FIXUP_WGS);
    const int64_t fix_wgs = forced_wgs > 0 ? forced_wgs : ((T + 1) / 2 + 3) / 4;
    hipLaunchKernelGGL(tim_fixup_group_kernel, dim3((unsigned)std::max<int64_t>(4, fix_wgs), batch),
                       dim3(256), 0, s, d_desc, batch, d_src, d_dst, d_bitmap, beta, work, work_count, d_state, d_deg,
                       regions, T, prep, upper ? 1 : 0);
  }
}

__global__ __launch_bounds__(256) void degree_kernel(const ProbDesc* __restrict__ descs,
                                                     const uint64_t* __restrict__ bitmap,
                                                     int32_t* __restrict__ deg) {
  const ProbDesc d = descs[blockIdx.y];
  const int lane = threadIdx.x & 63;
  for (int row = blockIdx.x * 4 + (threadIdx.x >> 6); row < d.n; row += gridDim.x * 4) {
    const uint64_t* r = bitmap + d.bm_off + (int64_t)row * bm_stride(d.W);
    int c = 0;
    for (int w = lane; w < d.W; w += 64) c += __popcll(r[w]);
    c = wave_sum_i(c);
    if (lane == 0) deg[d.pt_off + row] = c;
  }
}

void launch_degrees(hipStream_t s, const ProbDesc* d_desc, int batch, int max_n,
                    const uint64_t* d_bitmap, int32_t* d_deg, ProbState* d_state) {
  if (batch <= 0 || max_n <= 0) return;
  dim3 grid((max_n + 3) / 4, batch);
  hipLaunchKernelGGL(degree_kernel, grid, dim3(256), 0, s, d_desc, d_bitmap, d_deg);
}

__global__ __launch_bounds__(256) void trims_kernel(const double* __restrict__ src,
                                                    const double* __restrict__ dst, int n,
                                                    double beta, double* __restrict__ raw,
                                                    double* __restrict__ alpha) {
  const int i = blockIdx.x;
  if (i >= n - 1) return;
  const int64_t seg = (int64_t)i * n - (int64_t)i * (i + 1) / 2;
  const double six = src[3 * i], siy = src[3 * i + 1], siz = src[3 * i + 2];
  const double dix = dst[3 * i], diy = dst[3 * i + 1], diz = dst[3 * i + 2];
  for (int j = i + 1 + threadIdx.x; j < n; j += 256) {
    const double ax = src[3 * j] - six, ay = src[3 * j + 1] - siy, az = src[3 * j + 2] - siz;
    const double bx = dst[3 * j] - dix, by = dst[3 * j + 1] - diy, bz = dst[3 * j + 2] - diz;
    const double v1 = __builtin_sqrt((ax * ax + ay * ay) + az * az);
    const double v2 = __builtin_sqrt((bx * bx + by * by) + bz * bz);
    const int64_t k = seg + (j - i - 1);
    raw[k] = v2 / v1;
    alpha[k] = beta * (1.0 / v1);
  }
}

void launch_trims(hipStream_t s, const double* d_src, const double* d_dst, int n, double beta,
                  double* d_raw, double* d_alpha) {
  if (n < 2) return;
  hipLaunchKernelGGL(trims_kernel, dim3(n - 1), dim3(256), 0, s, d_src, d_dst, n, beta, d_raw,
                     d_alpha);
}

__global__ void fill_identity_clique_kernel(const ProbDesc* __restrict__ descs,
                                            int32_t* __restrict__ clique,
                                            ProbState* __restrict__ states) {
  const ProbDesc d = descs[blockIdx.y];
  const int i = blockIdx.x * blockDim.x + threadIdx.x;
  if (i < d.n) clique[d.pt_off + i] = i;
  if (i == 0) {
    ProbState* st = states + blockIdx.y;
    st->lb = d.n;
    st->clique_size = d.n;
    st->proven = 1;
    st->peel_done = 1;
  }
}

void launch_fill_identity_clique(hipStream_t s, const ProbDesc* d_desc, int batch, int max_n,
                                 int32_t* d_clique, ProbState* d_state) {
  if (batch <= 0) return;
  const int bx = max_n > 0 ? (max_n + 255) / 256 : 1;
  hipLaunchKernelGGL(fill_identity_clique_kernel, dim3(bx, batch), dim3(256), 0, s, d_desc,
                     d_clique, d_state);
}

}
```

teaser-plusplus_amd/csrc/kernels_heuristic.hip:

```cpp
#include <algorithm>
#include <utility>
#include <vector>

#include <cstdio>
#include <cstdlib>

#include "internal.h"
#include "wave_utils.h"

namespace thip {

constexpr int kGreedyMaxThreads = 512;
constexpr int kCap = 640;
constexpr int kCapW = kCap / 64;
constexpr int kCapStride = kCapW + 1;

template <int kGreedyWaves>
__device__ __forceinline__ int blockN_sum_i(int v, int* red ) {
  v = wave_sum_i(v);
  __syncthreads();
  if ((threadIdx.x & 63) == 0) red[threadIdx.x >> 6] = v;
  __syncthreads();
  int s = 0;
#pragma unroll
// ... 450 lines not shown
          const unsigned long long kk =
              ((unsigned long long)(unsigned int)(dv[j] + 1) << 32) | (0xffffffffu - (unsigned int)c);
          bestk = kk > bestk ? kk : bestk;
        }
      }
      bestk = blockN_max_u64<kGreedyWaves>(bestk, red64);
      csize = misc[0];
      int left = 0;
      for (int w = 0; w < Wc; ++w) left += __popcll(Pc[w]);
      __syncthreads();
      if (left > 0 && bestk) {
        const int bc = (int)(0xffffffffu - (unsigned int)(bestk & 0xffffffffu));
        if (tid == 0) {
          C[csize] = cand[bc];
          misc[0] = csize + 1;
        }
        ++csize;
        if (tid < Wc) Pc[tid] &= A[bc * kCapStride + tid];
        __syncthreads();
        pcnt = 0;
        for (int w = 0; w < Wc; ++w) pcnt += __popcll(Pc[w]);
      } else {
        pcnt = 0;
      }
    }
  }
  (void)gave_up;
  stamp(4);
  if (tid == 0) {
    st->start_size[sidx] = csize;
    atomicMax(&st->heu_best, csize);
  }
  return csize;
}

template <int kGreedyThreads>
__device__ __attribute__((noinline)) void closure_round(const uint64_t* __restrict__ bm, int W, int S , const uint64_t* Pa,
                                                        uint64_t* Pb, const int* alist, int cnt, int csize, int tid) {
  constexpr int kLanesPerRow = 16, kRowsPerGroup = 4, kChunk = 5;
  constexpr int kRowsPerPass = kGreedyThreads / kLanesPerRow * kRowsPerGroup;
  const int gid = tid / kLanesPerRow, sub = tid % kLanesPerRow;
#pragma unroll 1
  for (int k0 = 0; k0 < cnt; k0 += kRowsPerPass) {
    int v[kRowsPerGroup], c[kRowsPerGroup];
    const uint64_t* row[kRowsPerGroup];
#pragma unroll
    for (int r = 0; r < kRowsPerGroup; ++r) {
      const int k = k0 + gid * kRowsPerGroup + r;
      v[r] = k < cnt ? alist[k] : -1;
      row[r] = bm + (int64_t)(v[r] < 0 ? 0 : v[r]) * S;
      c[r] = 0;
    }
#pragma unroll 1
    for (int x0 = 0; x0 < W; x0 += kLanesPerRow * kChunk) {
      uint64_t buf[kRowsPerGroup][kChunk];
#pragma unroll
      for (int r = 0; r < kRowsPerGroup; ++r)
#pragma unroll
        for (int u = 0; u < kChunk; ++u) {
          const int x = x0 + u * kLanesPerRow + sub;
          buf[r][u] = (x < W && v[r] >= 0) ? row[r][x] : 0ull;
        }
#pragma unroll
      for (int u = 0; u < kChunk; ++u) {
        const int x = x0 + u * kLanesPerRow + sub;
        const uint64_t pa = x < W ? Pa[x] : 0ull;
#pragma unroll
        for (int r = 0; r < kRowsPerGroup; ++r) c[r] += __popcll(buf[r][u] & pa);
      }
    }
#pragma unroll
    for (int r = 0; r < kRowsPerGroup; ++r) {
      int cc = c[r];
      cc += __shfl_xor(cc, 8, 64);
      cc += __shfl_xor(cc, 4, 64);
      cc += __shfl_xor(cc, 2, 64);
      cc += __shfl_xor(cc, 1, 64);
      if (v[r] >= 0 && sub == 0 && cc >= csize)
        atomicOr(reinterpret_cast<unsigned long long*>(&Pb[v[r] >> 6]), 1ull << (v[r] & 63));
    }
  }
}

constexpr int kCoreCap = 2048;
constexpr int kCoreWords = kCoreCap / 64;
constexpr int kDegBins = kCoreCap;
constexpr int kDegMaxW = 1024;
constexpr int kDegThreads = 256;
static_assert(kDegBins % kDegThreads == 0 && (kDegBins / kDegThreads) % 4 == 0, "bins per thread");

template <typename Out>
__device__ __forceinline__ void list_bits_ascending(const uint64_t* P, int W, Out* out, int* csum, int tid) {
  const int lane = tid & 63, wave = tid >> 6;
  const int wpt = (W + kDegThreads - 1) / kDegThreads;
  const int w0 = tid * wpt, w1 = min(W, w0 + wpt);
  int mycnt = 0;
  for (int w = w0; w < w1; ++w) mycnt += __popcll(P[w]);
  __syncthreads();
  csum[tid] = mycnt;
  __syncthreads();
  if (wave == 0) {
    const int a0 = csum[4 * lane], a1 = csum[4 * lane + 1], a2 = csum[4 * lane + 2], a3 = csum[4 * lane + 3];
    const int tot = a0 + a1 + a2 + a3;
    int incl = tot;
#pragma unroll
    for (int o = 1; o < 64; o <<= 1) {
      const int t = __shfl_up(incl, o, 64);
      if (lane >= o) incl += t;
    }
    const int ex = incl - tot;
    csum[4 * lane] = ex;
    csum[4 * lane + 1] = ex + a0;
    csum[4 * lane + 2] = ex + a0 + a1;
    csum[4 * lane + 3] = ex + a0 + a1 + a2;
  }
  __syncthreads();
  int pos = csum[tid];
  for (int w = w0; w < w1; ++w) {
    uint64_t bits = P[w];
    while (bits) {
      out[pos++] = w * 64 + __builtin_ctzll(bits);
      bits &= bits - 1;
    }
  }
  __syncthreads();
}

template <int kBins>
__device__ __forceinline__ void suffix_counts(const int* hist, int* above, int tid) {
  constexpr int kPerT = kBins / kDegThreads;
  const int lane = tid & 63, wave = tid >> 6;
  int s = 0;
#pragma unroll
  for (int k = 0; k < kPerT; ++k) s += hist[tid * kPerT + k];
  above[tid] = s;
  __syncthreads();
  if (wave == 0) {
    int a[4], tot = 0;
#pragma unroll
    for (int k = 0; k < 4; ++k) {
      a[k] = above[4 * lane + k];
      tot += a[k];
    }
    int incl = tot;
#pragma unroll
    for (int o = 1; o < 64; o <<= 1) {
      const int t = __shfl_down(incl, o, 64);
      if (lane + o < 64) incl += t;
    }
    int ab = incl - tot + hist[kBins];
#pragma unroll
    for (int k = 3; k >= 0; --k) {
      above[4 * lane + k] = ab;
      ab += a[k];
    }
  }
  __syncthreads();
}

__global__ __launch_bounds__(kDegThreads) void degree_closure_order_kernel(
    const ProbDesc* __restrict__ descs, const int32_t* __restrict__ deg, ProbState* __restrict__ states,
    uint32_t* __restrict__ key_pool ,
    int32_t* __restrict__ counters , int batch) {
  TAIL_WAVE_PRIO();
  __shared__ uint64_t Pa[kDegMaxW];
  __shared__ int hist[kDegBins + 1];
  __shared__ unsigned int slot[kCoreCap];
  __shared__ unsigned int keys[kCoreCap];
// ... 434 lines not shown
        auto pick = [&](int e, int c) {
          const int a = miss_a[e], b = miss_b[e];
          const unsigned int ka = keys[a], kb2 = keys[b];
          const bool a_first = (ka >> 16) < (kb2 >> 16) || ((ka >> 16) == (kb2 >> 16) && (ka & 0xffffu) > (kb2 & 0xffffu));
          return (c == 0) == a_first ? a : b;
        };
        int e = first_uncovered(0);
        if (e < 0) {
          found = 0;
        } else {
          edge_at[0] = e;
          choice[0] = 0;
          for (int guard = 0; guard < 4096; ++guard) {
            if (choice[depth] > 1) {
              if (--depth < 0) break;
              ++choice[depth];
              continue;
            }
            drop[depth] = pick(edge_at[depth], choice[depth]);
            const int e2 = first_uncovered(depth + 1);
            if (e2 < 0) {
              found = depth + 1 == extra ? 1 : -1;
              break;
            }
            if (depth + 1 == extra) {
              ++choice[depth];
              continue;
            }
            ++depth;
            edge_at[depth] = e2;
            choice[depth] = 0;
          }
        }
        miss_verdict = found == 1 ? 1 : (found == 0 && depth < 0 ? 2 : 0);
        if (found == 1)
          for (int i = 0; i < extra; ++i) miss_a[i] = (unsigned short)drop[i];
      }
      __syncthreads();
      const int verdict = miss_verdict;
      if (verdict == 0) return;
      if (verdict == 2) {
        kmax = k - 1;
        continue;
      }
      if (tid < extra) {
        const int r = miss_a[tid];
        atomicAnd(reinterpret_cast<unsigned long long*>(&Sa[r >> 6]), ~(1ull << (r & 63)));
      }
      __syncthreads();
      cnt = k;
      tie = 1;
    }
    if (cnt < k) {
      kmax = k - 1;
      continue;
    }
    for (int w = tid; w < W; w += kDegThreads) Pa[w] = 0;
    __syncthreads();
    for (int r = tid; r < m; r += kDegThreads)
      if ((Sa[r >> 6] >> (r & 63)) & 1ull) {
        const int v = (int)(keys[r] & 0xffffu);
        atomicOr(reinterpret_cast<unsigned long long*>(&Pa[v >> 6]), 1ull << (v & 63));
      }
    __syncthreads();
    list_bits_ascending(Pa, W, clique + d.pt_off, csum, tid);
    if (tid == 0) {
      st->lb = k;
      st->best_start = -1;
      st->clique_size = k;
      st->alive_count = k;
      st->proven = 1;
      st->peel_done = 1;
      st->heu_closed = 1;
      st->deg_closed = tie ? 2 : 1;
    }
    return;
  }
}

int64_t degree_closure_scratch_bytes(int batch) {
  return (int64_t)std::max(batch, 1) * (2 * (int64_t)kCoreCap * kCoreWords * 8  + (int64_t)kCoreCap * 8);
}

void launch_degree_closure(hipStream_t s, const ProbDesc* d_desc, int batch, const uint64_t* d_bitmap,
                           const int32_t* d_deg, ProbState* d_state, int32_t* d_clique, void* d_scratch,
                           int32_t* d_counters) {
  if (batch <= 0) return;
  const int forced = (int)setting(S_DEG_CLOSURE_WGS);
  const int G = forced > 0 ? std::min(forced, 64) : std::max(1, std::min(16, 1024 / batch));
  uint64_t* comp = reinterpret_cast<uint64_t*>(d_scratch);
  uint64_t* part = comp + (size_t)batch * kCoreCap * kCoreWords;
  int32_t* hp = reinterpret_cast<int32_t*>(part + (size_t)batch * kCoreCap * kCoreWords);
  uint32_t* kp = reinterpret_cast<uint32_t*>(hp + (size_t)batch * kCoreCap);
  hipLaunchKernelGGL(degree_closure_order_kernel, dim3(1, batch), dim3(kDegThreads), 0, s, d_desc, d_deg, d_state, kp,
                     d_counters, batch);
  hipLaunchKernelGGL(degree_closure_rows_kernel, dim3(G, batch), dim3(kDegThreads), 0, s, d_desc, d_bitmap, part, kp,
                     d_counters, batch);
  hipLaunchKernelGGL(degree_closure_symmetrise_kernel, dim3(std::min(G, 8), batch), dim3(kDegThreads), 0, s, part, comp, hp, kp,
                     d_counters, batch);
  hipLaunchKernelGGL(degree_closure_verdict_kernel, dim3(batch), dim3(kDegThreads), 0, s, d_desc, d_state, d_clique, comp, hp,
                     kp, d_counters, batch);
}

template <int kGreedyThreads>
__global__ __launch_bounds__(kGreedyThreads) void greedy_clique_kernel(
    const ProbDesc* __restrict__ descs, const uint64_t* __restrict__ bitmap,
    const int32_t* __restrict__ deg, ProbState* __restrict__ states,
    int32_t* __restrict__ start_cliques, int64_t total_n, long long* __restrict__ trace, int batch) {
  TAIL_WAVE_PRIO();
  constexpr int kGreedyWaves = kGreedyThreads / 64;
  extern __shared__ __attribute__((aligned(16))) char smem[];
  __shared__ int next_s;
  __shared__ int red_c[kGreedyWaves];
  for (int rank = blockIdx.y;; rank += gridDim.y) {
  int prob = rank;
  if ((int)gridDim.y < batch) {
    __syncthreads();
    int seen = 0, hit = -1;
    for (int p0 = 0; p0 < batch && hit < 0; p0 += kGreedyThreads) {
      const int p = p0 + (int)threadIdx.x;
      const bool open = p < batch && !states[p].deg_closed;
      const uint64_t m = __ballot(open);
      if ((threadIdx.x & 63) == 0) red_c[threadIdx.x >> 6] = __builtin_popcountll(m);
      __syncthreads();
      int before = seen;
      for (int w = 0; w < (int)(threadIdx.x >> 6); ++w) before += red_c[w];
      if (open && before + __builtin_popcountll(m & ((1ull << (threadIdx.x & 63)) - 1ull)) == rank) next_s = p;
      int tot = 0;
      for (int w = 0; w < kGreedyWaves; ++w) tot += red_c[w];
      __syncthreads();
      if (seen + tot > rank) hit = next_s;
      seen += tot;
      __syncthreads();
    }
    if (hit < 0) return;
    prob = hit;
  } else if (rank >= batch) {
    return;
  }
  ProbState* st = states + prob;
  if (st->deg_closed) {
    if ((int)gridDim.y < batch) continue;
    return;
  }
  const ProbDesc d = descs[prob];
  int sidx = blockIdx.x;
  while (sidx < kMaxStarts) {
    const int csize = greedy_one_start<kGreedyThreads>(descs, bitmap, deg, states, start_cliques, total_n, smem, sidx, trace, prob);
    if (gridDim.x >= kMaxStarts) break;
    const int W = d.W, tid = threadIdx.x;
    uint64_t* Pa = reinterpret_cast<uint64_t*>(smem);
    uint64_t* Pb = Pa + ((W + 1) & ~1);
    const uint64_t* bm = bitmap + d.bm_off;
    int cnt = 0;
    __syncthreads();
    for (int w = tid >> 6; w < W; w += kGreedyWaves) {
      const int v = w * 64 + (tid & 63);
      const uint64_t bits = __ballot(v < d.n && deg[d.pt_off + v] >= csize);
      if ((tid & 63) == 0) {
        Pa[w] = bits;
        cnt += __popcll(bits);
      }
    }
    cnt = blockN_sum_i<kGreedyWaves>(cnt, red_c);
    constexpr int kClosureCap = 4096;
    int* alist = reinterpret_cast<int*>(Pb + ((W + 1) & ~1));
    for (int round = 0; round < 8 && cnt > csize && cnt <= 2 * csize + 256 && cnt <= kClosureCap; ++round) {
      if (tid == 0) next_s = 0;
      for (int w = tid; w < W; w += kGreedyThreads) Pb[w] = 0;
      __syncthreads();
      for (int w = tid; w < W; w += kGreedyThreads) {
        uint64_t bits = Pa[w];
        if (bits) {
          int pos = atomicAdd(&next_s, __popcll(bits));
          while (bits) {
            alist[pos++] = w * 64 + __builtin_ctzll(bits);
            bits &= bits - 1;
          }
        }
      }
// ... 534 lines not shown
```

teaser-plusplus_amd/csrc/solver.hip:

```cpp
#include <algorithm>
#include <cmath>
#include <cstdio>
#include <cstdlib>
#include <cstring>
#include <atomic>
#include <chrono>
#include <condition_variable>
#include <deque>
#include <memory>
#include <mutex>
#include <string>
#include <thread>
#include <vector>

#include "host_common.h"
#include "internal.h"

namespace thip {
void launch_select_best(hipStream_t s, const ProbDesc* d_desc, int batch, int max_W,
                        const int32_t* d_deg, ProbState* d_state, const int32_t* d_start_cliques,
                        int64_t total_n, int32_t* d_clique, uint64_t* d_alive_a, int do_peel,
                        const void* d_small_slots = nullptr, int small_G = 0);
void launch_peel_rounds(hipStream_t s, const ProbDesc* d_desc, int batch, int max_W,
                        const uint64_t* d_bitmap, ProbState* d_state, uint64_t* d_alive_a,
// ... 170 lines not shown
  }
  hipError_t ensure(size_t bytes) {
    if (bytes <= cap && !view) return hipSuccess;
    release();
    size_t want = bytes + bytes / 4 + 256;
    hipError_t e = hipMalloc(&p, want);
    if (e != hipSuccess) {
      e = hipMalloc(&p, bytes);
      want = bytes;
    }
    if (e == hipSuccess) cap = want;
    return e;
  }
  void release() {
    if (p && !view) (void)hipFree(p);
    p = nullptr;
    cap = 0;
    view = false;
  }
  template <typename T>
  T* as() const {
    return reinterpret_cast<T*>(p);
  }
};

struct PinnedBuf {
  void* p = nullptr;
  size_t cap = 0;
  PinnedBuf() = default;
  PinnedBuf(const PinnedBuf&) = delete;
  PinnedBuf& operator=(const PinnedBuf&) = delete;
  ~PinnedBuf() { release(); }
  hipError_t ensure(size_t bytes) {
    if (bytes <= cap) return hipSuccess;
    release();
    const size_t want = bytes + bytes / 2 + 256;
    hipError_t e = hipHostMalloc(&p, want, hipHostMallocDefault);
    if (e == hipSuccess) cap = want;
    return e;
  }
  void release() {
    if (p) (void)hipHostFree(p);
    p = nullptr;
    cap = 0;
  }
};

enum Stage { ST_H2D = 0, ST_TIM, ST_DEG, ST_HEU, ST_PEEL, ST_EXACT, ST_ROT, ST_TRANS, ST_D2H, ST_COLOUR, ST_TIMAUX, ST_COUNT };

}

struct LaneFinisher {
  std::thread th;
  std::mutex m;
  std::condition_variable cv;
  std::atomic<int> state{0};
  std::vector<teaser_solution_c> out;
  int32_t rc = TEASER_HIP_OK;
};

struct teaser_hip_solver : HandleBase {
  teaser_params_c params;
  teaser_params_c params_given;
  int profiling = 0;
  teaser_profile_c prof;
  std::vector<hipEvent_t> ev_pool;
  struct Span { int stage; hipEvent_t a, b; };
  std::vector<Span> spans;
  size_t ev_used = 0;

  int batch = 0;
  int max_n = 0, max_W = 0;
  int64_t total_n = 0, total_bm = 0, total_w = 0, total_tims = 0;
  std::vector<ProbDesc> descs;
  std::vector<ProbState> states;
  std::vector<int64_t> tim_off;
  std::vector<int32_t> exact_run;
  std::vector<int32_t> heu_size;
  std::vector<int32_t> prob_status;
  const double* cur_src = nullptr;
  const double* cur_dst = nullptr;
  bool have_graph = false;
  bool bm_lower_missing = false;

  std::vector<uint64_t> bm_stage;
  SolverBuf d_desc, d_state, d_src, d_dst, d_bitmap, d_deg, d_clique, d_start_cliques, d_alive_a,
      d_alive_b, d_next_count, d_weights, d_rot_inl, d_trans_inl, d_tls_scratch, d_tim_off,
      d_pk, d_prep, d_work, d_core, d_small;
  SolverBuf c_sel, c_colour, c_tent, c_xlist, c_list_a, c_list_b, c_counts, c_bits, c_class, c_mis;
  std::vector<int32_t> colour_x;
  SolverBuf x_order, x_src, x_dst, x_bitmap, x_ctrl, x_clique, x_arena, x_probs, x_probs2, x_keys, x_xbits, x_tasks;
  SolverBuf s_a, s_b, s_c, s_d, s_e;
  teaser_hip_features* features = nullptr;

  PinnedBuf pin_states;
  PinnedBuf pin_in;
  PinnedBuf pin_pts;
  PinnedBuf pin_ep;
  bool spec_bounds_next = false;
  bool spec_mis_fits = true;
  int last_unproven = 0;
  bool skip_heuristic_next = false;
  int closure_open_prev = 0;
  int heu_blocks = 0;
  int heu_rows = 0;

  struct Pending {
    const double* d_src = nullptr;
    const double* d_dst = nullptr;
    int batch = 0, mode = 0;
    bool need_graph = false;
    bool spec_bounds = false;
    bool closure = false;
    bool heuristic_enqueued = true;
    int64_t total_n = 0, tls_stride = 0;
  } pend;
  std::vector<teaser_hip_solver*> lanes;
  std::vector<std::pair<int, int>> route;
  hipEvent_t k1_done = nullptr;
  hipEvent_t wait_before_k1 = nullptr;
  bool k1_recorded = false;
  int depth = 2;
  int next_lane = 0, last_lane = -1;
  bool stagger_k1 = true;
  int stagger_point = 1;
  hipStream_t k1_stream = nullptr;
  bool shared_k1_stream = false;
  bool k1_kernel_only = false;
  int tail_cus = 0;
  bool tail_cu_block = false;
  hipEvent_t k1_phase_done = nullptr;
  hipEvent_t inputs_ready = nullptr;
  bool inputs_pending = false;
  bool is_lane = false;
  std::unique_ptr<LaneFinisher> fin;
  struct Job {
    bool busy = false;
    std::vector<int64_t> off;
    std::vector<int32_t> n;
    const double* d_src = nullptr;
    const double* d_dst = nullptr;
    int in_set = -1;
    int32_t ticket = -1;
  } job;
  SolverBuf hdr;
  struct InSet {
    SolverBuf src, dst;
    hipEvent_t ready = nullptr;
    bool in_use = false;
    ~InSet() {
      if (ready) (void)hipEventDestroy(ready);
    }
  };
  std::deque<InSet> in_sets;
  hipStream_t copy_stream = nullptr;
  struct Staged {
    bool active = false;
    int32_t ticket = -1;
    int in_set = -1;
    std::vector<int64_t> off;
    std::vector<int32_t> n;
  } staged;
  int32_t staged_rc = TEASER_HIP_OK;
  std::string staged_err;
  std::vector<int> ticket_lane;
};

struct teaser_hip_multi {
  std::vector<teaser_hip_solver*> handles;
  std::vector<int32_t> first;
};

namespace {

#define HIPCHK(h, call)                                                                     \
  do {                                                                                      \
    hipError_t _e = (call);                                                                 \
    if (_e != hipSuccess) {                                                                 \
      (h)->err = std::string(#call) + ": " + hipGetErrorString(_e);                         \
      return _e == hipErrorOutOfMemory ? TEASER_HIP_ERR_OOM : TEASER_HIP_ERR_HIP;           \
    }                                                                                       \
  } while (0)

struct StageScope {
  teaser_hip_solver* h;
  bool on;
// ... 485 lines not shown
        e.ctrl[2] = e.ctrl[3] = e.ctrl[4] = 0;
        again.push_back(e);
      } else if (e.ctrl[4] == 2) {
        h->prob_status[(size_t)e.prob] = TEASER_HIP_ERR_TIME_LIMIT;
      }
    }
    run.swap(again);
  }
  return TEASER_HIP_OK;
}

bool spec_bounds_enabled() { return setting(S_SPEC_BOUNDS) != 0; }

int32_t enqueue_bounds_speculative(teaser_hip_solver* h, int batch, int64_t total_n) {
  hipStream_t s = h->stream;
  const ProbDesc* dd = h->d_desc.as<ProbDesc>();
  ProbState* ds = h->d_state.as<ProbState>();
  const auto [final_alive, spare_alive] = alive_masks(h);
  const int64_t tw = std::max<int64_t>(h->total_w, 1);
  const int32_t rc = ensure_bound_scratch(h, batch, total_n);
  if (rc != TEASER_HIP_OK) return rc;
  HIPCHK(h, h->pin_ep.ensure(sizeof(ExactProb) * (size_t)batch));
  bool mis = setting(S_COLOUR_MIS) > 0 && h->max_n >= setting(S_COLOUR_MIS) && h->max_n <= 65536;
  if (mis && setting(S_COLOUR_MIS_ANY) == 0) mis = h->spec_mis_fits;
  if (mis) HIPCHK(h, h->c_mis.ensure((size_t)colour_mis_bytes(batch, h->max_n)));
  {
    StageScope sc(h, ST_COLOUR);
    launch_colour_bound(s, dd, nullptr, batch, h->max_n, h->d_bitmap.as<uint64_t>(), final_alive,
                        h->d_clique.as<int32_t>(), ds, h->c_colour.as<int32_t>(), h->c_tent.as<int32_t>(),
                        h->c_xlist.as<int32_t>(), h->c_class.as<int32_t>(), h->c_list_a.as<int32_t>(),
                        h->c_list_b.as<int32_t>(), h->c_counts.as<int32_t>(), h->c_bits.as<uint64_t>(), tw, total_n,
                        kColourRounds, mis ? h->c_mis.p : nullptr, h->d_deg.as<int32_t>());
  }
  {
    StageScope sc(h, ST_EXACT);
    HIPCHK(h, hipMemsetAsync(h->x_probs.p, 0, sizeof(ExactProb) * (size_t)batch, s));
    launch_exact_count(s, dd, h->x_probs.as<ExactProb>(), batch, h->max_W, h->d_bitmap.as<uint64_t>(), final_alive,
                       h->d_deg.as<int32_t>(), ds, h->c_xlist.as<int32_t>(), h->c_tent.as<int32_t>(), spare_alive,
                       h->x_xbits.as<uint64_t>(), true);
    HIPCHK(h, hipMemcpyAsync(h->pin_ep.p, h->x_probs.p, sizeof(ExactProb) * (size_t)batch, hipMemcpyDeviceToHost, s));
  }
  HIPCHK(h, hipGetLastError());
  return TEASER_HIP_OK;
}

int32_t enqueue_estimators(teaser_hip_solver* h) {
  hipStream_t s = h->stream;
  const int batch = h->pend.batch;
  const ProbDesc* dd = h->d_desc.as<ProbDesc>();
  ProbState* ds = h->d_state.as<ProbState>();
  const EstParams ep = est_params(h->params);
  const bool fused = setting(S_FUSED_EST) != 0;
  static_assert(sizeof(ProbState) % 8 == 0, "ProbState is moved in 8-byte pieces");
  HIPCHK(h, h->pin_states.ensure(sizeof(ProbState) * (size_t)batch));
  if (fused) {
    StageScope sc(h, ST_ROT);
    launch_estimate_fused(s, dd, batch, h->pend.d_src, h->pend.d_dst, h->d_clique.as<int32_t>(), ds, ep,
                          h->d_weights.as<double>(), h->d_rot_inl.as<int32_t>(), h->d_tim_off.as<int64_t>(),
                          h->d_tls_scratch.as<char>(), h->pend.tls_stride, h->d_trans_inl.as<int32_t>(),
                          h->pin_states.p);
    HIPCHK(h, hipGetLastError());
    return TEASER_HIP_OK;
  }
  {
    StageScope sc(h, ST_ROT);
    launch_gnc_tls(s, dd, batch, h->pend.d_src, h->pend.d_dst, h->d_clique.as<int32_t>(), ds, ep,
                   h->d_weights.as<double>(), h->d_rot_inl.as<int32_t>(), h->d_tim_off.as<int64_t>());
  }
  {
    StageScope sc(h, ST_TRANS);
    launch_tls_translation(s, dd, batch, h->pend.d_src, h->pend.d_dst, h->d_clique.as<int32_t>(), ds, ep,
                           h->d_tls_scratch.as<char>(), h->pend.tls_stride, h->d_trans_inl.as<int32_t>());
  }
  HIPCHK(h, hipGetLastError());
  {
    StageScope sc(h, ST_D2H);
    const int n8 = (int)(sizeof(ProbState) * (size_t)batch / 8);
    hipLaunchKernelGGL(state_push_kernel, dim3((unsigned)std::min(8, (n8 + 255) / 256)), dim3(256), 0, s,
                       h->d_state.as<uint2>(), reinterpret_cast<uint2*>(h->pin_states.p), n8);
  }
  return TEASER_HIP_OK;
}

int32_t enqueue_heuristic_stage(teaser_hip_solver* h, int batch, int mode, bool record_stagger) {
  hipStream_t s = h->stream;
  const ProbDesc* dd = h->d_desc.as<ProbDesc>();
  ProbState* ds = h->d_state.as<ProbState>();
  const int64_t total_n = std::max<int64_t>(h->total_n, 1);
  {
    StageScope sc(h, ST_HEU);
    if (h->bm_lower_missing)
      launch_tim_graph_mfma(s, kTimMirrorOpen, dd, batch, h->max_n, 0, nullptr, nullptr, nullptr, nullptr, nullptr, 0,
                            h->d_bitmap.as<uint64_t>(), ds, nullptr, 0.0, 0.0);
    int32_t* heu_trace = nullptr;
    if (setting(S_K4_DEBUG) && batch <= 4) {
      HIPCHK(h, h->s_e.ensure(sizeof(long long) * 8 * kMaxStarts * (size_t)batch));
      HIPCHK(h, hipMemsetAsync(h->s_e.p, 0, sizeof(long long) * 8 * kMaxStarts * (size_t)batch, s));
      heu_trace = h->s_e.as<int32_t>();
    }
    launch_heuristic(s, dd, batch, h->max_W, h->d_bitmap.as<uint64_t>(), h->d_deg.as<int32_t>(), ds,
                     h->d_start_cliques.as<int32_t>(), total_n, heu_trace, h->d_clique.as<int32_t>(), h->heu_blocks, h->heu_rows);
    if (record_stagger && h->k1_done && h->stagger_point == 2) {
      HIPCHK(h, hipEventRecord(h->k1_done, s));
      h->k1_recorded = true;
    }
    int small_G = 0;
    if (setting(S_GREEDY_SMALL) != 0) {
      int max_small = 0;
      for (int b = 0; b < batch; ++b)
        if (h->descs[(size_t)b].n <= kSmallCap) max_small = std::max(max_small, h->descs[(size_t)b].n);
      if (max_small >= 2) {
        HIPCHK(h, h->d_small.ensure((size_t)greedy_small_scratch_bytes(batch)));
        small_G = launch_greedy_small(s, dd, batch, max_small, h->d_bitmap.as<uint64_t>(), h->d_deg.as<int32_t>(), ds,
                                      h->d_small.p, h->d_next_count.as<int32_t>() + 4 * (size_t)batch);
      }
    }
    launch_select_best(s, dd, batch, h->max_W, h->d_deg.as<int32_t>(), ds,
                       h->d_start_cliques.as<int32_t>(), total_n, h->d_clique.as<int32_t>(),
                       h->d_alive_a.as<uint64_t>(), mode == TEASER_INLIER_PMC_EXACT ? 1 : 0, h->d_small.p, small_G);
  }
  if (mode == TEASER_INLIER_PMC_EXACT) {
    StageScope sc(h, ST_PEEL);
    launch_peel_rounds(s, dd, batch, h->max_W, h->d_bitmap.as<uint64_t>(), ds,
                       h->d_alive_a.as<uint64_t>(), h->d_alive_b.as<uint64_t>(),
                       h->d_next_count.as<int32_t>(), kPeelRounds);
  }
  HIPCHK(h, hipGetLastError());
  return TEASER_HIP_OK;
}

ProbDesc problem_desc(int n, int64_t pt_off, int64_t bm_off, int64_t w_off) {
  ProbDesc d;
  d.n = n;
  d.W = (n + 63) / 64;
  d.pt_off = pt_off;
  d.bm_off = bm_off;
  d.w_off = w_off;
  return d;
}

ProbState initial_state(int heu_blocks) {
  ProbState st;
  memset(&st, 0, sizeof(st));
  st.scale = 1.0;
  st.R[0] = st.R[4] = st.R[8] = 1.0;
  st.gnc_cost = INFINITY;
  st.next_start = heu_blocks;
  for (int k = 0; k < kMaxStarts; ++k) st.start_vertex[k] = -1;
  return st;
}

int32_t layout_batch(teaser_hip_solver* h, const int64_t* pt_off, const int32_t* n, int batch, bool closure) {
  h->batch = batch;
  h->descs.assign((size_t)batch, ProbDesc());
  h->tim_off.assign((size_t)batch, 0);
  h->exact_run.assign((size_t)batch, 0);
  h->heu_size.assign((size_t)batch, 0);
  h->prob_status.assign((size_t)batch, TEASER_HIP_OK);
  h->colour_x.assign((size_t)batch, -1);
  int max_n = 0;
  for (int b = 0; b < batch; ++b) max_n = std::max(max_n, n[b]);
  const bool closure_ahead = closure && max_n <= 65536;
  h->heu_blocks = heuristic_blocks_per_problem(batch, (max_n + 63) / 64, closure_ahead ? h->closure_open_prev : -1);
  h->heu_rows = closure_ahead && h->closure_open_prev * 4 <= batch ? std::min(batch, std::max(4, 2 * h->closure_open_prev)) : 0;
  h->states.assign((size_t)batch, initial_state(h->heu_blocks));
  int64_t bm = 0, wo = 0, tims = 0, maxpt = 0;
  for (int b = 0; b < batch; ++b) {
    if (n[b] < 0) return TEASER_HIP_ERR_BAD_ARG;
    const ProbDesc d = h->descs[(size_t)b] = problem_desc(n[b], pt_off[b], bm, wo);
    bm += (int64_t)d.n * bm_stride(d.W);
    wo += d.W;
    h->tim_off[(size_t)b] = tims;
    const int64_t kt = h->params.rotation_tim_graph == TEASER_TIM_CHAIN ? (int64_t)d.n : (int64_t)d.n * (d.n - 1) / 2;
    tims += kt + 2;
    maxpt = std::max<int64_t>(maxpt, d.pt_off + d.n);
  }
  h->max_n = max_n;
  h->max_W = (max_n + 63) / 64;
  h->total_n = maxpt;
  h->total_bm = bm;
  h->total_w = wo;
  h->total_tims = tims;
  return TEASER_HIP_OK;
}

int32_t solve_packed_enqueue(teaser_hip_solver* h, const double* d_src, const double* d_dst,
                             const int64_t* pt_off, const int32_t* n, int batch, bool fp64_k1) {
  hipStream_t s = h->stream;
  hipStream_t s1 = s;
  const teaser_params_c& P = h->params;
  if (!params_supported(P)) {
    h->err = "rotation_estimation_algorithm must be GNC_TLS, FGR or QUATRO";
    return TEASER_HIP_ERR_UNSUPPORTED;
  }
  const int mode = effective_mode(P);
  h->cur_src = d_src;
  h->cur_dst = d_dst;
  h->have_graph = false;
  h->pend.closure = false;
  h->pend.heuristic_enqueued = true;
  const int32_t lrc = layout_batch(h, pt_off, n, batch, mode == TEASER_INLIER_PMC_EXACT && setting(S_DEG_CLOSURE) != 0);
  if (lrc != TEASER_HIP_OK) return lrc;
  const int max_n = h->max_n;
  const int64_t bm = h->total_bm, wo = h->total_w, tims = h->total_tims;
  if (tims > ((int64_t)1 << 31)) {
    h->err = "rotation_tim_graph = COMPLETE needs too many TIMs for this batch";
    return TEASER_HIP_ERR_UNSUPPORTED;
  }
  if (mode == TEASER_INLIER_KCORE_HEU && max_n > 65536) {
    h->err = "inlier_selection_mode = KCORE_HEU supports at most 65536 correspondences per problem";
    return TEASER_HIP_ERR_UNSUPPORTED;
  }
  const int64_t total_n = std::max<int64_t>(h->total_n, 1);

  const size_t b_desc = sizeof(ProbDesc) * (size_t)batch, b_state = sizeof(ProbState) * (size_t)batch,
               b_off = 8 * (size_t)batch,
               b_next = 20 * (size_t)batch ,
               b_prep = (size_t)tim_prep_bytes(batch);
  auto al256 = [](size_t x) { return (x + 255) & ~(size_t)255; };
  const size_t o_desc = 0, o_state = al256(o_desc + b_desc), o_off = al256(o_state + b_state),
               o_next = al256(o_off + b_off), o_prep = al256(o_next + b_next),
               hdr_bytes = al256(o_prep + b_prep);
  HIPCHK(h, h->hdr.ensure(hdr_bytes));
  {
    char* base = h->hdr.as<char>();
    h->d_desc.set_view(base + o_desc, b_desc);
    h->d_state.set_view(base + o_state, b_state);
    h->d_tim_off.set_view(base + o_off, b_off);
    h->d_next_count.set_view(base + o_next, b_next);
    h->d_prep.set_view(base + o_prep, b_prep);
  }
  HIPCHK(h, h->d_clique.ensure(4 * (size_t)total_n));
  HIPCHK(h, h->d_weights.ensure(8 * (size_t)std::max<int64_t>(tims, 1)));
  HIPCHK(h, h->d_rot_inl.ensure(4 * (size_t)std::max<int64_t>(tims, 1)));
  HIPCHK(h, h->d_trans_inl.ensure(4 * (size_t)total_n));
  const int64_t tls_stride = tls_scratch_bytes(std::max(max_n, 1));
  HIPCHK(h, h->d_tls_scratch.ensure((size_t)tls_stride * (size_t)batch));
  const bool need_graph = (mode != TEASER_INLIER_NONE) && max_n >= 1;
  const bool mfma_k1 = need_graph && !P.estimate_scaling && max_n <= 65536 && !fp64_k1 && setting(S_K1_FP64) == 0;
  if (need_graph) {
    HIPCHK(h, h->d_bitmap.ensure(8 * (size_t)std::max<int64_t>(bm, 1)));
    HIPCHK(h, h->d_deg.ensure(4 * (size_t)total_n));
    HIPCHK(h, h->d_start_cliques.ensure(4 * (size_t)total_n * kMaxStarts));
    HIPCHK(h, h->d_alive_a.ensure(8 * (size_t)std::max<int64_t>(wo, 1)));
    HIPCHK(h, h->d_alive_b.ensure(8 * (size_t)std::max<int64_t>(wo, 1)));
    if (mfma_k1) {
      HIPCHK(h, h->d_pk.ensure((size_t)tim_operand_bytes(wo)));
      HIPCHK(h, h->d_work.ensure(8 * (size_t)tim_work_items(n, batch) + 64));
    }
  }
  const bool closure = need_graph && mode == TEASER_INLIER_PMC_EXACT && max_n <= 65536 && setting(S_DEG_CLOSURE) != 0 &&
                       !(setting(S_TAIL_SKIP) & 2);
  const bool upper_k1 = mfma_k1 && closure;
  if (need_graph) h->bm_lower_missing = upper_k1;
  const bool k1_only = mfma_k1 && h->is_lane && h->k1_stream && h->k1_kernel_only;
  if (mfma_k1 && h->is_lane && h->k1_stream && !k1_only) {
    s1 = h->k1_stream;
    if (h->inputs_pending) {
      HIPCHK(h, hipEventRecord(h->inputs_ready, s));
      HIPCHK(h, hipStreamWaitEvent(s1, h->inputs_ready, 0));
    }
  }
  h->inputs_pending = false;
  {
    StageScope sc(h, ST_H2D, s1);
    HIPCHK(h, h->pin_in.ensure(hdr_bytes));
    char* stage = reinterpret_cast<char*>(h->pin_in.p);
    memset(stage, 0, hdr_bytes);
    memcpy(stage + o_desc, h->descs.data(), b_desc);
    memcpy(stage + o_state, h->states.data(), b_state);
    memcpy(stage + o_off, h->tim_off.data(), b_off);
    if (mfma_k1) (void)tim_prep_fill_segments(stage + o_prep, n, batch);
    hipLaunchKernelGGL(hdr_fetch_kernel, dim3((unsigned)std::min<size_t>(8, (hdr_bytes / 16 + 255) / 256)), dim3(256), 0,
                       s1, reinterpret_cast<const uint4*>(stage), h->hdr.as<uint4>(), (int)(hdr_bytes / 16));
  }
  const ProbDesc* dd = h->d_desc.as<ProbDesc>();
  ProbState* ds = h->d_state.as<ProbState>();

  if (P.estimate_scaling) {
    StageScope sc(h, ST_TIM);
    int32_t rc = scale_stage_batch(h, batch, fp64_k1);
    if (rc != TEASER_HIP_OK) return rc;
  }
  if (need_graph) {
    if (!mfma_k1) {
      StageScope sc(h, ST_TIM);
      launch_tim_graph(s, dd, batch, max_n, d_src, d_dst, h->d_bitmap.as<uint64_t>(), P.noise_bound,
                       P.cbar2, P.estimate_scaling ? 1 : 0, ds);
    } else {
      const int64_t cap = tim_work_items(n, batch);
      const int64_t tail_skip = setting(S_TAIL_SKIP);
      for (int phase = 0; phase < 3; ++phase) {
        if ((phase == 2 && (tail_skip & 1)) || (phase == 0 && (tail_skip & 16))) continue;
        if (phase == 1 && h->wait_before_k1 && s1 == s && !k1_only) {
          HIPCHK(h, hipStreamWaitEvent(s, h->wait_before_k1, 0));
          h->wait_before_k1 = nullptr;
        }
        hipStream_t sp = (k1_only && phase == 1) ? h->k1_stream : s1;
        if (k1_only && phase == 1) {
          HIPCHK(h, hipEventRecord(h->inputs_ready, s));
          HIPCHK(h, hipStreamWaitEvent(sp, h->inputs_ready, 0));
        }
        {
          StageScope sc(h, phase == 1 ? ST_TIM : ST_TIMAUX, sp);
          launch_tim_graph_mfma(sp, (upper_k1 && phase > 0) ? (phase | kTimUpperOnly) : phase, dd, batch, max_n, wo, d_src, d_dst, h->d_pk.p, h->d_prep.p,
                                h->d_work.p, cap, h->d_bitmap.as<uint64_t>(), ds, h->d_deg.as<int32_t>(),
                                P.noise_bound, P.cbar2);
        }
        if (k1_only && phase == 1) {
          HIPCHK(h, hipEventRecord(h->k1_phase_done, sp));
          HIPCHK(h, hipStreamWaitEvent(s, h->k1_phase_done, 0));
        }
        if (phase == 1 && h->k1_done && s1 == s && !k1_only && h->stagger_point == 1) {
          HIPCHK(h, hipEventRecord(h->k1_done, s));
          h->k1_recorded = true;
        }
      }
      if (s1 != s) {
        HIPCHK(h, hipEventRecord(h->k1_phase_done, s1));
        HIPCHK(h, hipStreamWaitEvent(s, h->k1_phase_done, 0));
      }
    }
    for (int b = 0; b < batch; ++b) {
      const int64_t nn = h->descs[(size_t)b].n;
      h->prof.tim_graph_pairs += nn * (nn - 1) / 2;
      h->prof.tim_graph_bytes += 48 * nn + 8 * nn * ((nn + 63) / 64);
    }
    if (!mfma_k1) {
      StageScope sc(h, ST_DEG);
      launch_degrees(s, dd, batch, max_n, h->d_bitmap.as<uint64_t>(), h->d_deg.as<int32_t>(), ds);
    }
    if (closure) {
      StageScope sc(h, ST_HEU);
      HIPCHK(h, h->d_core.ensure((size_t)degree_closure_scratch_bytes(batch)));
      launch_degree_closure(s, dd, batch, h->d_bitmap.as<uint64_t>(), h->d_deg.as<int32_t>(), ds,
                            h->d_clique.as<int32_t>(), h->d_core.p, h->d_next_count.as<int32_t>() + 2 * (size_t)batch);
    }
    h->pend.closure = closure;
    h->pend.heuristic_enqueued = !(closure && h->skip_heuristic_next && setting(S_HEU_SKIP_CLOSED) != 0);
    if (h->pend.heuristic_enqueued && !(setting(S_TAIL_SKIP) & 4)) {
      int32_t rc = enqueue_heuristic_stage(h, batch, mode, mfma_k1);
      if (rc != TEASER_HIP_OK) return rc;
    }
    if (mode == TEASER_INLIER_KCORE_HEU) {
      StageScope sc(h, ST_PEEL);
      HIPCHK(h, h->c_colour.ensure(4 * (size_t)total_n));
      HIPCHK(h, h->c_tent.ensure(4 * (size_t)total_n));
      launch_kcore_heuristic(s, dd, batch, h->d_bitmap.as<uint64_t>(), h->d_deg.as<int32_t>(), ds,
                             h->c_colour.as<int32_t>(), h->c_tent.as<int32_t>(), h->d_clique.as<int32_t>(),
                             P.kcore_heuristic_threshold);
    }
    if (mfma_k1 && h->k1_done && (h->stagger_point == 3 || (h->stagger_point == 2 && !h->pend.heuristic_enqueued))) {
      HIPCHK(h, hipEventRecord(h->k1_done, s));
      h->k1_recorded = true;
    }
    h->have_graph = true;
  } else {
    launch_fill_identity_clique(s, dd, batch, max_n, h->d_clique.as<int32_t>(), ds);
  }
  HIPCHK(h, hipGetLastError());

  h->pend.d_src = d_src;
  h->pend.d_dst = d_dst;
  h->pend.batch = batch;
  h->pend.mode = mode;
  h->pend.need_graph = need_graph;
  h->pend.total_n = total_n;
  h->pend.tls_stride = tls_stride;
  h->pend.spec_bounds = false;
  int32_t rc = (setting(S_TAIL_SKIP) & 8) ? TEASER_HIP_OK : enqueue_estimators(h);
  if (rc == TEASER_HIP_OK && need_graph && mode == TEASER_INLIER_PMC_EXACT && h->spec_bounds_next && spec_bounds_enabled() &&
      h->pend.heuristic_enqueued) {
    rc = enqueue_bounds_speculative(h, batch, total_n);
    h->pend.spec_bounds = rc == TEASER_HIP_OK;
    g_trace.mark(h, "submit: bound stage enqueued speculatively");
  }
  return rc;
}

int32_t solve_packed_finish(teaser_hip_solver* h, teaser_solution_c* out, bool* k1_overflow) {
  const int batch = h->pend.batch;
  HIPCHK(h, hipStreamSynchronize(h->stream));
  g_trace.mark(h, "finish: first sync done");
  memcpy(h->states.data(), h->pin_states.p, sizeof(ProbState) * (size_t)batch);
  *k1_overflow = false;
  for (int b = 0; b < batch; ++b)
    if (h->states[(size_t)b].k1_overflow || h->states[(size_t)b].scale_overflow) *k1_overflow = true;
  if (*k1_overflow) return TEASER_HIP_OK;
  if (h->pend.closure) {
    int open = 0;
    for (int b = 0; b < batch; ++b) open += h->states[(size_t)b].deg_closed ? 0 : 1;
    if (open > 0 && !h->pend.heuristic_enqueued) {
      g_trace.mark(h, "finish: heuristic stage for the problems the degree closure left open");
      int32_t rc = enqueue_heuristic_stage(h, batch, h->pend.mode, false);
      if (rc == TEASER_HIP_OK) rc = enqueue_estimators(h);
      if (rc != TEASER_HIP_OK) return rc;
      HIPCHK(h, hipStreamSynchronize(h->stream));
      memcpy(h->states.data(), h->pin_states.p, sizeof(ProbState) * (size_t)batch);
    }
    h->skip_heuristic_next = open == 0;
    h->closure_open_prev = open;
  }
  for (int b = 0; b < batch; ++b) h->heu_size[(size_t)b] = h->states[(size_t)b].lb;
  if (setting(S_K4_DEBUG) && batch <= 4)
    for (int b = 0; b < batch; ++b) {
      const ProbState& st = h->states[(size_t)b];
      fprintf(stderr, "[teaser_hip] heuristic, problem %d: lb %d (start %d), degree closure %d, proven %d, alive %d; starts (vertex:size):",
              b, st.lb, st.best_start, st.deg_closed, st.proven, st.alive_count);
      for (int k = 0; k < kMaxStarts; ++k) fprintf(stderr, " %d:%d", st.start_vertex[k], st.start_size[k]);
      fprintf(stderr, "\n");
      long long tr[kMaxStarts][8];
      if (h->s_e.p && hipMemcpy(tr, h->s_e.as<long long>() + (size_t)b * kMaxStarts * 8, sizeof(tr), hipMemcpyDeviceToHost) == hipSuccess) {
        fprintf(stderr, "[teaser_hip]   per start, us: select | shrink (static picks, vote rounds) | gather | vote | total:");
        for (int k = 0; k < kMaxStarts; ++k)
          fprintf(stderr, " [%.0f %.0f (%lld,%lld) %.0f %.0f = %.0f]", (tr[k][1] - tr[k][0]) * 0.01, (tr[k][2] - tr[k][1]) * 0.01, tr[k][6],
                  tr[k][7], (tr[k][3] - tr[k][2]) * 0.01, (tr[k][4] - tr[k][3]) * 0.01, (tr[k][4] - tr[k][0]) * 0.01);
        fprintf(stderr, "\n");
      }
    }
  h->last_unproven = 0;
  if (h->pend.need_graph && h->pend.mode == TEASER_INLIER_PMC_EXACT) {
    bool changed = false;
    int32_t rc = close_clique_bounds(h, batch, h->pend.total_n, &changed);
    if (rc != TEASER_HIP_OK) return rc;
    if (changed) {
      rc = enqueue_estimators(h);
      if (rc != TEASER_HIP_OK) return rc;
      HIPCHK(h, hipStreamSynchronize(h->stream));
      memcpy(h->states.data(), h->pin_states.p, sizeof(ProbState) * (size_t)batch);
    }
  }

  for (int b = 0; b < batch; ++b) {
    const ProbState& st = h->states[(size_t)b];
    teaser_solution_c& o = out[b];
    memset(&o, 0, sizeof(o));
    o.n = h->descs[(size_t)b].n;
    o.status = h->prob_status[(size_t)b];
    o.scale = st.scale;
    o.clique_size = st.clique_size;
    o.heuristic_size = h->heu_size[(size_t)b];
    o.clique_exact_run = h->exact_run[(size_t)b];
    o.colour_uncoloured = st.deg_closed ? (st.deg_closed == 2 ? -3 : -2) : (b < (int)h->colour_x.size() ? h->colour_x[(size_t)b] : -1);
    o.num_edges = (int64_t)(st.deg_sum / 2);
    if (st.clique_size <= 1) {
      o.valid = 0;
      o.rotation[0] = o.rotation[4] = o.rotation[8] = 1.0;
      o.gnc_cost = INFINITY;
      continue;
    }
    o.valid = 1;
    memcpy(o.rotation, st.R, sizeof(o.rotation));
    memcpy(o.translation, st.t, sizeof(o.translation));
    o.n_rotation_inliers = st.n_rot;
    o.n_translation_inliers = st.n_trans;
    o.gnc_cost = st.gnc_cost;
    o.gnc_iterations = st.gnc_iters;
  }
  return TEASER_HIP_OK;
}

int32_t solve_packed_impl(teaser_hip_solver* h, const double* d_src, const double* d_dst,
                          const int64_t* pt_off, const int32_t* n, int batch,
                          teaser_solution_c* out, bool fp64_k1, bool* k1_overflow) {
  const int32_t rc = solve_packed_enqueue(h, d_src, d_dst, pt_off, n, batch, fp64_k1);
  if (rc != TEASER_HIP_OK) return rc;
  return solve_packed_finish(h, out, k1_overflow);
}

int32_t make_lane(teaser_hip_solver* h, teaser_hip_solver** out);
void destroy_handle(teaser_hip_solver* h);

int32_t solve_packed(teaser_hip_solver* h, const double* d_src, const double* d_dst,
                     const int64_t* pt_off, const int32_t* n, int batch, teaser_solution_c* out) {
  h->route.clear();
  if (batch > kMaxBatch) return over_batch_limit(h);
  bool overflow = false;
  int32_t rc = solve_packed_impl(h, d_src, d_dst, pt_off, n, batch, out, false, &overflow);
  if (rc == TEASER_HIP_OK && overflow)
    rc = solve_packed_impl(h, d_src, d_dst, pt_off, n, batch, out, true, &overflow);
  h->spec_bounds_next = rc == TEASER_HIP_OK && h->last_unproven > 0;
  return rc;
}

// ... 592 lines not shown
  std::vector<double> s((size_t)n_corr * 3), d((size_t)n_corr * 3);
  for (int32_t i = 0; i < n_corr; ++i) {
    const int32_t a = corr[2 * i], b = corr[2 * i + 1];
    if (a < 0 || a >= n_src || b < 0 || b >= n_dst) return TEASER_HIP_ERR_BAD_ARG;
    for (int r = 0; r < 3; ++r) {
      s[3 * (size_t)i + r] = (double)src_cloud[3 * (size_t)a + r];
      d[3 * (size_t)i + r] = (double)dst_cloud[3 * (size_t)b + r];
    }
  }
  return teaser_hip_solve(h, s.data(), d.data(), n_corr, out);
}

int32_t teaser_hip_solve_batch(teaser_hip_solver* h, const double* const* src,
                               const double* const* dst, const int32_t* n, int32_t batch,
                               teaser_solution_c* out) {
  if (!h || batch < 0 || (batch > 0 && (!src || !dst || !n || !out))) return TEASER_HIP_ERR_BAD_ARG;
  if (batch == 0) return TEASER_HIP_OK;
  (void)hipSetDevice(h->device);
  return upload_and_solve(h, src, dst, n, batch, out);
}

int32_t teaser_hip_solve_batch_device(teaser_hip_solver* h, const double* d_src,
                                      const double* d_dst, const int64_t* point_offset,
                                      const int32_t* n, int32_t batch, teaser_solution_c* out) {
  if (!h || batch < 0 || (batch > 0 && (!d_src || !d_dst || !point_offset || !n || !out)))
    return TEASER_HIP_ERR_BAD_ARG;
  if (batch == 0) return TEASER_HIP_OK;
  (void)hipSetDevice(h->device);
  profile_begin(h);
  int32_t rc = solve_packed(h, d_src, d_dst, point_offset, n, batch, out);
  profile_end(h);
  return rc;
}

#define CHECK_PROBLEM(h, problem)                                                      \
  if (!(h) || (problem) < 0 || (problem) >= (h)->batch) return TEASER_HIP_ERR_BAD_ARG; \
  (void)hipSetDevice((h)->device);                                                     \
  (h) = route_problem((h), &(problem))

int32_t teaser_hip_get_max_clique(teaser_hip_solver* h, int32_t problem, int32_t* buf, int64_t* len) {
  CHECK_PROBLEM(h, problem);
  const ProbDesc& d = h->descs[(size_t)problem];
  return copy_out(h, h->d_clique.as<int32_t>() + d.pt_off, h->states[(size_t)problem].clique_size,
                  buf, len);
}

int32_t teaser_hip_get_rotation_inliers(teaser_hip_solver* h, int32_t problem, int32_t* buf,
                                        int64_t* len) {
  CHECK_PROBLEM(h, problem);
  const ProbState& st = h->states[(size_t)problem];
  return copy_out(h, h->d_rot_inl.as<int32_t>() + h->tim_off[(size_t)problem],
                  st.clique_size > 1 ? st.n_rot : 0, buf, len);
}

int32_t teaser_hip_get_translation_inliers(teaser_hip_solver* h, int32_t problem, int32_t* buf,
                                           int64_t* len) {
  CHECK_PROBLEM(h, problem);
  const ProbDesc& d = h->descs[(size_t)problem];
  const ProbState& st = h->states[(size_t)problem];
  return copy_out(h, h->d_trans_inl.as<int32_t>() + d.pt_off, st.clique_size > 1 ? st.n_trans : 0,
                  buf, len);
}

int32_t teaser_hip_get_input_ordered_translation_inliers(teaser_hip_solver* h, int32_t problem,
                                                         int32_t* buf, int64_t* len) {
  CHECK_PROBLEM(h, problem);
  if (!len) return TEASER_HIP_ERR_BAD_ARG;
  const ProbDesc& d = h->descs[(size_t)problem];
  const ProbState& st = h->states[(size_t)problem];
  const int64_t cnt = st.clique_size > 1 ? st.n_trans : 0;
  const int64_t cap = *len;
  *len = cnt;
  if (!buf) return TEASER_HIP_OK;
  if (cap < cnt) return TEASER_HIP_ERR_BAD_ARG;
  std::vector<int32_t> ti((size_t)cnt), cl((size_t)st.clique_size);
  if (cnt > 0) {
    HIPCHK(h, hipMemcpy(ti.data(), h->d_trans_inl.as<int32_t>() + d.pt_off, (size_t)cnt * 4, hipMemcpyDeviceToHost));
    HIPCHK(h, hipMemcpy(cl.data(), h->d_clique.as<int32_t>() + d.pt_off, (size_t)st.clique_size * 4, hipMemcpyDeviceToHost));
  }
  for (int64_t k = 0; k < cnt; ++k) buf[k] = cl[(size_t)ti[(size_t)k]];
  return TEASER_HIP_OK;
}

int32_t teaser_hip_get_inlier_graph_bitmap(teaser_hip_solver* h, int32_t problem, uint64_t* buf,
                                           int64_t* len) {
  CHECK_PROBLEM(h, problem);
  if (!h->have_graph) {
    if (len) *len = 0;
    return len ? TEASER_HIP_OK : TEASER_HIP_ERR_BAD_ARG;
  }
  const ProbDesc& d = h->descs[(size_t)problem];
  if (buf && h->bm_lower_missing) {
    launch_tim_graph_mfma(h->stream, kTimMirror, h->d_desc.as<ProbDesc>(), h->batch, h->max_n, 0, nullptr, nullptr, nullptr,
                          nullptr, nullptr, 0, h->d_bitmap.as<uint64_t>(), h->d_state.as<ProbState>(), nullptr, 0.0, 0.0);
    HIPCHK(h, hipGetLastError());
    HIPCHK(h, hipStreamSynchronize(h->stream));
    h->bm_lower_missing = false;
  }
  if (!len) return TEASER_HIP_ERR_BAD_ARG;
  const int64_t cap = *len, count = (int64_t)d.n * d.W;
  *len = count;
  if (!buf) return TEASER_HIP_OK;
  if (cap < count) return TEASER_HIP_ERR_BAD_ARG;
  const int S = bm_stride(d.W);
  const uint64_t* rows = h->d_bitmap.as<uint64_t>() + d.bm_off;
  if (S == d.W) {
    if (count > 0) HIPCHK(h, hipMemcpy(buf, rows, (size_t)count * 8, hipMemcpyDeviceToHost));
    return TEASER_HIP_OK;
  }
  const int64_t blk = std::max<int64_t>(1, ((int64_t)4 << 20) / S);
  std::vector<uint64_t> stage((size_t)(std::min<int64_t>(blk, d.n) * S));
  for (int64_t r0 = 0; r0 < d.n; r0 += blk) {
    const int64_t nr = std::min<int64_t>(blk, d.n - r0);
    HIPCHK(h, hipMemcpy(stage.data(), rows + r0 * S, (size_t)(nr * S) * 8, hipMemcpyDeviceToHost));
    for (int64_t r = 0; r < nr; ++r) memcpy(buf + (r0 + r) * d.W, stage.data() + r * S, (size_t)d.W * 8);
  }
  return TEASER_HIP_OK;
}

int32_t teaser_hip_get_inlier_graph_rows(teaser_hip_solver* h, int32_t problem, uint64_t* buf, int64_t* len,
                                         int32_t* stride_words) {
  CHECK_PROBLEM(h, problem);
  const ProbDesc& d = h->descs[(size_t)problem];
  if (stride_words) *stride_words = bm_stride(d.W);
  if (!h->have_graph) {
    if (len) *len = 0;
    return len ? TEASER_HIP_OK : TEASER_HIP_ERR_BAD_ARG;
  }
  return copy_out(h, h->d_bitmap.as<uint64_t>() + d.bm_off, (int64_t)d.n * bm_stride(d.W), buf, len);
}

int32_t teaser_hip_get_degrees(teaser_hip_solver* h, int32_t problem, int32_t* buf, int64_t* len) {
  CHECK_PROBLEM(h, problem);
  if (!h->have_graph) {
    if (len) *len = 0;
    return len ? TEASER_HIP_OK : TEASER_HIP_ERR_BAD_ARG;
  }
  const ProbDesc& d = h->descs[(size_t)problem];
  return copy_out(h, h->d_deg.as<int32_t>() + d.pt_off, (int64_t)d.n, buf, len);
}

TEASER_HIP_API int32_t teaser_hip_probe_k1_worklist(teaser_hip_solver* h, uint64_t* regions, int64_t* stride_words,
                                                    int64_t* used_regions, int32_t* problems, uint32_t* seg_counts) {
  int32_t problem = 0;
  CHECK_PROBLEM(h, problem);
  if (!stride_words || !used_regions || !problems || !h->d_work.p || !h->d_prep.p) return TEASER_HIP_ERR_BAD_ARG;
  std::vector<int32_t> n((size_t)h->batch);
  int max_n = 0;
  for (int b = 0; b < h->batch; ++b) max_n = std::max(max_n, n[(size_t)b] = h->descs[(size_t)b].n);
  *problems = h->batch;
  HIPCHK(h, hipDeviceSynchronize());
  HIPCHK(h, (hipError_t)tim_probe_worklist(h->d_prep.p, h->d_work.p, tim_work_items(n.data(), h->batch), h->batch, max_n,
                                           reinterpret_cast<unsigned long long*>(regions), stride_words, used_regions,
                                           seg_counts));
  return TEASER_HIP_OK;
}

int32_t teaser_hip_solve_for_rotation(teaser_hip_solver* h, const double* src, const double* dst,
                                      int32_t k, double noise_bound, double* rotation,
                                      uint8_t* inlier_mask, double* cost, int32_t* iterations) {
  if (!h || !src || !dst || k <= 0 || !rotation) return TEASER_HIP_ERR_BAD_ARG;
  (void)hipSetDevice(h->device);
  hipStream_t s = h->stream;
  HIPCHK(h, h->s_a.ensure((size_t)k * 24));
  HIPCHK(h, h->s_b.ensure((size_t)k * 24));
  HIPCHK(h, h->s_c.ensure((size_t)k * 8));
  HIPCHK(h, h->s_d.ensure(128));
  HIPCHK(h, hipMemcpyAsync(h->s_a.p, src, (size_t)k * 24, hipMemcpyHostToDevice, s));
  HIPCHK(h, hipMemcpyAsync(h->s_b.p, dst, (size_t)k * 24, hipMemcpyHostToDevice, s));
  launch_gnc_tls_raw(s, h->s_a.as<double>(), h->s_b.as<double>(), k, noise_bound, est_params(h->params),
                     h->s_c.as<double>(), h->s_d.as<double>(), reinterpret_cast<int32_t*>(h->s_d.as<double>() + 12));
  HIPCHK(h, hipGetLastError());
  double outv[13];
  HIPCHK(h, hipMemcpyAsync(outv, h->s_d.p, sizeof(outv), hipMemcpyDeviceToHost, s));
  std::vector<double> w((size_t)k);
  HIPCHK(h, hipMemcpyAsync(w.data(), h->s_c.p, (size_t)k * 8, hipMemcpyDeviceToHost, s));
  HIPCHK(h, hipStreamSynchronize(s));
  memcpy(rotation, outv, 9 * sizeof(double));
  if (cost) *cost = outv[9];
  if (iterations) memcpy(iterations, &outv[12], 4);
  if (inlier_mask)
    for (int32_t j = 0; j < k; ++j) inlier_mask[j] = w[(size_t)j] >= 0.5;
  return TEASER_HIP_OK;
}

int32_t teaser_hip_solve_for_translation(teaser_hip_solver* h, const double* src,
                                         const double* dst, int32_t k, double* translation,
                                         uint8_t* inlier_mask) {
  if (!h || !src || !dst || k <= 1 || !translation) return TEASER_HIP_ERR_BAD_ARG;
  (void)hipSetDevice(h->device);
  hipStream_t s = h->stream;
  const ProbDesc d = problem_desc(k, 0, 0, 0);
  ProbState st = initial_state(0);
  st.clique_size = k;
  std::vector<int32_t> ident((size_t)k);
  for (int32_t i = 0; i < k; ++i) ident[(size_t)i] = i;
  const int64_t stride = tls_scratch_bytes(k);
  HIPCHK(h, h->s_a.ensure((size_t)k * 24));
  HIPCHK(h, h->s_b.ensure((size_t)k * 24));
  HIPCHK(h, h->s_c.ensure((size_t)k * 4));
  HIPCHK(h, h->s_d.ensure(sizeof(ProbDesc) + sizeof(ProbState) + 64));
  HIPCHK(h, h->s_e.ensure((size_t)k * 4));
  HIPCHK(h, h->d_tls_scratch.ensure((size_t)stride));
  char* dp = h->s_d.as<char>();
  HIPCHK(h, hipMemcpyAsync(h->s_a.p, src, (size_t)k * 24, hipMemcpyHostToDevice, s));
  HIPCHK(h, hipMemcpyAsync(h->s_b.p, dst, (size_t)k * 24, hipMemcpyHostToDevice, s));
  HIPCHK(h, hipMemcpyAsync(h->s_c.p, ident.data(), (size_t)k * 4, hipMemcpyHostToDevice, s));
  HIPCHK(h, hipMemcpyAsync(dp, &d, sizeof(d), hipMemcpyHostToDevice, s));
  HIPCHK(h, hipMemcpyAsync(dp + 64, &st, sizeof(st), hipMemcpyHostToDevice, s));
  launch_tls_translation(s, reinterpret_cast<ProbDesc*>(dp), 1, h->s_a.as<double>(), h->s_b.as<double>(),
                         h->s_c.as<int32_t>(), reinterpret_cast<ProbState*>(dp + 64),
                         est_params(h->params), h->d_tls_scratch.as<char>(), stride, h->s_e.as<int32_t>());
// ... 19 lines not shown
  const bool large = n > kScalarTlsSingleMax;
  HIPCHK(h, h->s_c.ensure((size_t)(large ? scalar_tls_large_workspace_bytes(n) : scalar_tls_small_workspace_bytes(n))));
  HIPCHK(h, h->s_d.ensure(64));
  HIPCHK(h, h->s_e.ensure((size_t)n + 16));
  int32_t* d_flag = reinterpret_cast<int32_t*>(h->s_d.as<char>() + 8);
  for (int attempt = 0; attempt < 2; ++attempt) {
    if (large) {
      HIPCHK(h, hipMemsetAsync(d_flag, 0, 4, s));
      HIPCHK(h, launch_scalar_tls_large(s, d_x, d_r, n, h->s_c.as<char>(), h->s_d.as<double>(), h->s_e.as<uint8_t>(),
                                        attempt == 0 ? d_flag : nullptr));
    } else {
      launch_scalar_tls(s, d_x, d_r, (int32_t)n, h->s_c.as<char>(), h->s_d.as<double>(), h->s_e.as<uint8_t>());
    }
    HIPCHK(h, hipGetLastError());
    int32_t flag = 0;
    HIPCHK(h, hipMemcpyAsync(estimate, h->s_d.p, 8, hipMemcpyDeviceToHost, s));
    if (large) HIPCHK(h, hipMemcpyAsync(&flag, d_flag, 4, hipMemcpyDeviceToHost, s));
    if (inlier_mask) HIPCHK(h, hipMemcpyAsync(inlier_mask, h->s_e.p, (size_t)n, hipMemcpyDeviceToHost, s));
    HIPCHK(h, hipStreamSynchronize(s));
    if (!flag) break;
  }
  return TEASER_HIP_OK;
}
}

int32_t teaser_hip_scalar_tls(teaser_hip_solver* h, const double* x, const double* ranges,
                              int32_t n, double* estimate, uint8_t* inlier_mask) {
  if (!h || !x || !ranges || n <= 0 || !estimate) return TEASER_HIP_ERR_BAD_ARG;
  (void)hipSetDevice(h->device);
  HIPCHK(h, h->s_a.ensure((size_t)n * 8));
  HIPCHK(h, h->s_b.ensure((size_t)n * 8));
  HIPCHK(h, hipMemcpyAsync(h->s_a.p, x, (size_t)n * 8, hipMemcpyHostToDevice, h->stream));
  HIPCHK(h, hipMemcpyAsync(h->s_b.p, ranges, (size_t)n * 8, hipMemcpyHostToDevice, h->stream));
  return run_scalar_tls(h, h->s_a.as<double>(), h->s_b.as<double>(), n, estimate, inlier_mask);
}

int32_t teaser_hip_solve_for_scale(teaser_hip_solver* h, const double* v1, const double* v2, int64_t m,
                                   double* scale, uint8_t* inlier_mask) {
  if (!h || !v1 || !v2 || m <= 0 || !scale) return TEASER_HIP_ERR_BAD_ARG;
  if (m > ((int64_t)1 << 30)) {
    h->err = "solveForScale: at most 2^30 TIMs (as the reference)";
    return TEASER_HIP_ERR_UNSUPPORTED;
  }
  (void)hipSetDevice(h->device);
  hipStream_t s = h->stream;
  const double beta = 2 * h->params.noise_bound * std::sqrt(h->params.cbar2);
  HIPCHK(h, h->s_a.ensure((size_t)m * 24));
  HIPCHK(h, h->s_b.ensure((size_t)m * 24));
  HIPCHK(h, hipMemcpyAsync(h->s_a.p, v1, (size_t)m * 24, hipMemcpyHostToDevice, s));
  HIPCHK(h, hipMemcpyAsync(h->s_b.p, v2, (size_t)m * 24, hipMemcpyHostToDevice, s));
  *scale = 1.0;
  if (h->params.estimate_scaling) {
    HIPCHK(h, h->x_src.ensure((size_t)m * 8));
    HIPCHK(h, h->x_dst.ensure((size_t)m * 8));
    launch_tim_scale_terms(s, h->s_a.as<double>(), h->s_b.as<double>(), m, beta, 1, h->x_src.as<double>(),
                           h->x_dst.as<double>(), nullptr);
    return run_scalar_tls(h, h->x_src.as<double>(), h->x_dst.as<double>(), m, scale, inlier_mask);
  }
  HIPCHK(h, h->s_e.ensure((size_t)m + 16));
  launch_tim_scale_terms(s, h->s_a.as<double>(), h->s_b.as<double>(), m, beta, 0, nullptr, nullptr,
                         h->s_e.as<uint8_t>());
  HIPCHK(h, hipGetLastError());
  if (inlier_mask) HIPCHK(h, hipMemcpyAsync(inlier_mask, h->s_e.p, (size_t)m, hipMemcpyDeviceToHost, s));
  HIPCHK(h, hipStreamSynchronize(s));
  return TEASER_HIP_OK;
}

int32_t teaser_hip_max_clique(teaser_hip_solver* h, const uint64_t* bitmap, int32_t n,
                              int32_t* clique, int32_t* clique_size, int32_t* exact_run) {
  if (!h || !bitmap || n <= 0 || !clique || !clique_size) return TEASER_HIP_ERR_BAD_ARG;
  (void)hipSetDevice(h->device);
  hipStream_t s = h->stream;
  const int W = (n + 63) / 64, S = bm_stride(W);
  const int mode = effective_mode(h->params);
  if (mode == TEASER_INLIER_KCORE_HEU && n > 65536) {
    h->err = "KCORE_HEU supports at most 65536 vertices";
    return TEASER_HIP_ERR_UNSUPPORTED;
  }
  const int64_t off = 0;
  int32_t rc = layout_batch(h, &off, &n, 1, false);
  if (rc != TEASER_HIP_OK) return rc;
  h->batch = 0;
  h->pend.spec_bounds = false;
  h->bm_lower_missing = false;
  ProbState& st = h->states[0];
  HIPCHK(h, h->d_desc.ensure(sizeof(ProbDesc)));
  HIPCHK(h, h->d_state.ensure(sizeof(ProbState)));
  HIPCHK(h, h->d_bitmap.ensure((size_t)n * S * 8));
  HIPCHK(h, h->d_deg.ensure((size_t)n * 4));
  HIPCHK(h, h->d_clique.ensure((size_t)n * 4));
  HIPCHK(h, h->d_start_cliques.ensure((size_t)n * 4 * kMaxStarts));
  HIPCHK(h, h->d_alive_a.ensure((size_t)W * 8));
  HIPCHK(h, h->d_alive_b.ensure((size_t)W * 8));
  HIPCHK(h, h->d_next_count.ensure(32));
  HIPCHK(h, hipMemcpyAsync(h->d_desc.p, h->descs.data(), sizeof(ProbDesc), hipMemcpyHostToDevice, s));
  HIPCHK(h, hipMemcpyAsync(h->d_state.p, &st, sizeof(st), hipMemcpyHostToDevice, s));
  const uint64_t* up = bitmap;
  if (S != W) {
    h->bm_stage.assign((size_t)n * S, 0ull);
    for (int64_t r = 0; r < n; ++r) memcpy(h->bm_stage.data() + r * S, bitmap + r * W, (size_t)W * 8);
    up = h->bm_stage.data();
  }
  HIPCHK(h, hipMemcpyAsync(h->d_bitmap.p, up, (size_t)n * S * 8, hipMemcpyHostToDevice, s));
  HIPCHK(h, hipMemsetAsync(h->d_next_count.p, 0, 32, s));
  const bool exact = (mode == TEASER_INLIER_PMC_EXACT);
  launch_degrees(s, h->d_desc.as<ProbDesc>(), 1, n, h->d_bitmap.as<uint64_t>(), h->d_deg.as<int32_t>(),
                 h->d_state.as<ProbState>());
  rc = enqueue_heuristic_stage(h, 1, mode, false);
  if (rc != TEASER_HIP_OK) return rc;
  if (mode == TEASER_INLIER_KCORE_HEU) {
    HIPCHK(h, h->c_colour.ensure(4 * (size_t)n));
    HIPCHK(h, h->c_tent.ensure(4 * (size_t)n));
    launch_kcore_heuristic(s, h->d_desc.as<ProbDesc>(), 1, h->d_bitmap.as<uint64_t>(), h->d_deg.as<int32_t>(),
                           h->d_state.as<ProbState>(), h->c_colour.as<int32_t>(), h->c_tent.as<int32_t>(),
                           h->d_clique.as<int32_t>(), h->params.kcore_heuristic_threshold);
  }
  HIPCHK(h, hipGetLastError());
  HIPCHK(h, hipMemcpyAsync(&st, h->d_state.p, sizeof(st), hipMemcpyDeviceToHost, s));
  HIPCHK(h, hipStreamSynchronize(s));
  if (exact && n >= 2) {
    bool changed = false;
    rc = close_clique_bounds(h, 1, n, &changed);
    if (rc != TEASER_HIP_OK) return rc;
  }
  if (exact_run) *exact_run = h->exact_run[0];
  *clique_size = st.clique_size;
  if (st.clique_size > 0)
    HIPCHK(h, hipMemcpy(clique, h->d_clique.p, (size_t)st.clique_size * 4, hipMemcpyDeviceToHost));
  return h->prob_status[0];
}

int32_t teaser_hip_submit_batch(teaser_hip_solver* h, const double* src, const double* dst,
                                const int64_t* point_offset, const int32_t* n, int32_t batch,
                                int32_t flags, int32_t* ticket) {
  if (!h || !ticket || batch <= 0 || !src || !dst || !point_offset || !n) return TEASER_HIP_ERR_BAD_ARG;
  if (batch > kMaxBatch) return over_batch_limit(h);
  (void)hipSetDevice(h->device);
  g_trace.mark(h, "submit: begin");
  const int32_t rc = submit_impl(h, src, dst, point_offset, n, batch, flags, ticket);
  g_trace.mark(h, "submit: end");
  return rc;
}

int32_t teaser_hip_wait(teaser_hip_solver* h, int32_t ticket, teaser_solution_c* out) {
  if (!h || !out) return TEASER_HIP_ERR_BAD_ARG;
  (void)hipSetDevice(h->device);
  g_trace.mark(h, "wait: begin");
  const int32_t rc = wait_impl(h, ticket, out);
  g_trace.mark(h, "wait: end");
  return rc;
}

int32_t teaser_hip_set_pipeline_depth(teaser_hip_solver* h, int32_t depth) {
  if (!h || depth < 1 || depth > 16) return TEASER_HIP_ERR_BAD_ARG;
  for (teaser_hip_solver* lane : h->lanes)
    if (lane->job.busy) return TEASER_HIP_ERR_BUSY;
  if (h->staged.active) return TEASER_HIP_ERR_BUSY;
  h->ticket_lane.assign((size_t)depth + 1, -2);
  if (depth < (int32_t)h->lanes.size()) {
    (void)hipSetDevice(h->device);
    for (size_t k = (size_t)depth; k < h->lanes.size(); ++k) destroy_handle(h->lanes[k]);
    h->lanes.resize((size_t)depth);
    h->route.clear();
    h->batch = 0;
  }
  h->depth = depth;
  h->next_lane = 0;
// ... 265 lines not shown
```

Before: 115,400.

## Skip K1 off-diagonal bitmap stores when degree closure usually closes; rebuild lazily

Adds a no-store K1 route, chosen when the previous batch's degree closure left few problems open. In that route the MFMA graph kernel writes only diagonal tiles and degrees, and the fix-up kernel records corrected edge masks back into the work items instead of XORing off-diagonal bitmap words. The closure then works from the recorded pairs without reading the bitmap. The full adjacency rows are rebuilt by a grid-strided kernel only for problems that stay open, or when the caller asks for the bitmap. The aim is to avoid writing the O(n²) bitmap on the common path, at the cost of a recompute when closure fails and more complex state tracking.

```diff
diff --git a/include/teaser_hip.h b/include/teaser_hip.h
--- a/include/teaser_hip.h
+++ b/include/teaser_hip.h
@@ -159,6 +159,7 @@
 TEASER_HIP_API int32_t teaser_hip_get_degrees(teaser_hip_solver* h, int32_t problem, int32_t* buf, int64_t* len);
 TEASER_HIP_API int32_t teaser_hip_get_inlier_graph_rows(teaser_hip_solver* h, int32_t problem, uint64_t* buf,
                                          int64_t* len , int32_t* stride_words);
+TEASER_HIP_API int32_t teaser_hip_get_graph_route(teaser_hip_solver* h, int32_t problem, int32_t* route, int64_t* rebuilt);
 
 TEASER_HIP_API int32_t teaser_hip_solve_for_rotation(teaser_hip_solver* h, const double* src, const double* dst,
                                       int32_t k, double noise_bound, double* rotation_rowmajor,
diff --git a/teaser-plusplus_amd/__init__.py b/teaser-plusplus_amd/__init__.py
--- a/teaser-plusplus_amd/__init__.py
+++ b/teaser-plusplus_amd/__init__.py
@@ -103,7 +103,7 @@
     "teaser_hip_solve_device", "teaser_hip_solve_correspondences", "teaser_hip_solve_batch",
     "teaser_hip_solve_batch_device", "teaser_hip_get_max_clique", "teaser_hip_get_rotation_inliers",
     "teaser_hip_get_translation_inliers", "teaser_hip_get_input_ordered_translation_inliers",
-    "teaser_hip_get_inlier_graph_bitmap", "teaser_hip_get_inlier_graph_rows", "teaser_hip_get_degrees", "teaser_hip_solve_for_rotation",
+    "teaser_hip_get_inlier_graph_bitmap", "teaser_hip_get_inlier_graph_rows", "teaser_hip_get_graph_route", "teaser_hip_get_degrees", "teaser_hip_solve_for_rotation",
     "teaser_hip_solve_for_translation", "teaser_hip_scalar_tls", "teaser_hip_max_clique",
     "teaser_hip_set_profiling", "teaser_hip_set_option", "teaser_hip_get_option", "teaser_hip_get_profile", "teaser_hip_get_stream",
     "teaser_hip_last_error", "teaser_hip_abi_version", "teaser_hip_device_count", "teaser_hip_host_alloc",
@@ -216,6 +216,7 @@
         getattr(L, nm).argtypes = [_vp, C.c_int32, _ip, _i64p]
     L.teaser_hip_get_inlier_graph_bitmap.argtypes = [_vp, C.c_int32, _u64p, _i64p]
     L.teaser_hip_get_inlier_graph_rows.argtypes = [_vp, C.c_int32, _u64p, _i64p, _ip]
+    L.teaser_hip_get_graph_route.argtypes = [_vp, C.c_int32, _ip, _i64p]
     L.teaser_hip_solve_for_rotation.argtypes = [_vp, _dp, _dp, C.c_int32, C.c_double, _dp, _u8p, _dp, _ip]
     L.teaser_hip_solve_for_translation.argtypes = [_vp, _dp, _dp, C.c_int32, _dp, _u8p]
     L.teaser_hip_scalar_tls.argtypes = [_vp, _dp, _dp, C.c_int32, _dp, _u8p]
diff --git a/teaser-plusplus_amd/csrc/internal.h b/teaser-plusplus_amd/csrc/internal.h
--- a/teaser-plusplus_amd/csrc/internal.h
+++ b/teaser-plusplus_amd/csrc/internal.h
@@ -139,6 +139,7 @@
                        unsigned int* seg_counts);
 int64_t tim_prep_fill_segments(void* host_prep, const int32_t* n, int batch);
 constexpr int kTimUpperOnly = 8, kTimMirror = 3, kTimMirrorOpen = 4;
+constexpr int kTimNoStore = 16, kTimRebuild = 5, kTimRebuildOpen = 6, kTimClosurePairs = 7;
 void launch_tim_graph_mfma(hipStream_t s, int phase, const ProbDesc* d_desc, int batch, int max_n,
                            int64_t total_tiles, const double* d_src, const double* d_dst,
                            void* d_pk, void* d_prep, void* d_work, int64_t work_cap,
@@ -160,6 +161,18 @@
 void launch_degree_closure(hipStream_t s, const ProbDesc* d_desc, int batch, const uint64_t* d_bitmap,
                            const int32_t* d_deg, ProbState* d_state, int32_t* d_clique, void* d_scratch,
                            int32_t* d_counters);
+constexpr int kCoreCap = 2048;
+constexpr int kCoreWords = kCoreCap / 64;
+struct ClosurePools {
+  uint64_t* comp;
+  uint64_t* part;
+  int32_t* h;
+  uint32_t* keys;
+};
+ClosurePools degree_closure_pools(void* d_scratch, int batch);
+int degree_closure_wgs(int batch);
+void launch_degree_closure_order(hipStream_t s, const ProbDesc* d_desc, int batch, const int32_t* d_deg, ProbState* d_state,
+                                 void* d_scratch, int32_t* d_counters);
 void launch_peel(hipStream_t s, const ProbDesc* d_desc, int batch, int max_n, int max_W,
                  const uint64_t* d_bitmap, const int32_t* d_deg, ProbState* d_state,
                  uint64_t* d_alive_a, uint64_t* d_alive_b);
diff --git a/teaser-plusplus_amd/csrc/kernels_graph.hip b/teaser-plusplus_amd/csrc/kernels_graph.hip
--- a/teaser-plusplus_amd/csrc/kernels_graph.hip
+++ b/teaser-plusplus_amd/csrc/kernels_graph.hip
@@ -495,21 +495,31 @@
 constexpr bool kK1Pipe = false, kK1Plain = true;
 constexpr int kK1Chunks = 1, kK1Occ = 3;
 
-template <bool PIPE, bool PLAIN, int OCC, int CHUNKS, bool LOWER, bool UW3 = false>
+constexpr int kK1NoStore = 1, kK1Rebuild = 2;
+template <bool PIPE, bool PLAIN, int OCC, int CHUNKS, bool LOWER, bool UW3 = false, int NS = 0>
 __global__ __launch_bounds__(256, OCC) void tim_graph_mfma3_kernel(
     const ProbDesc* __restrict__ descs, const double* __restrict__ src,
     const double* __restrict__ dst, const void* __restrict__ ops, const TimPrep* __restrict__ prep,
     uint64_t* __restrict__ bitmap, double beta, int gyr,
     unsigned long long* __restrict__ work, unsigned int* __restrict__ work_count,
-    ProbState* __restrict__ states, int32_t* __restrict__ deg, unsigned long long* __restrict__ regions, int Tmax) {
+    ProbState* __restrict__ states, int32_t* __restrict__ deg, unsigned long long* __restrict__ regions, int Tmax,
+    int rb_open, int nlb_arg) {
+  static_assert(NS == 0 || (NS == kK1NoStore && !LOWER) || (NS == kK1Rebuild && LOWER), "store modes");
+  if constexpr (NS == kK1Rebuild) {
+    if ((rb_open && states[blockIdx.y].deg_closed) || !prep[blockIdx.y].use_mfma) return;
+  }
   const ProbDesc d = descs[blockIdx.y];
   const int n = d.n, W = d.W;
   const int T = W, S = bm_stride(W);
+  int lb = (int)blockIdx.x;
+  const int nlb = NS == kK1Rebuild ? nlb_arg : (int)gridDim.x;
+  do {
   int Ig, X;
-  fxr::decode_block((int)blockIdx.x, (int)gridDim.x, gyr, CHUNKS, &Ig, &X);
+  fxr::decode_block(lb, nlb, gyr, CHUNKS, &Ig, &X);
   constexpr int kBlockColTiles = kMfmaColTiles * CHUNKS;
   const int I0 = Ig * kMfmaRowTiles, Jbase = X * kBlockColTiles;
   auto region_of = [&](int wv, int chunk) -> unsigned long long* {
+    if constexpr (NS == kK1Rebuild) return nullptr;
     const int Iw = I0 + wv, Xc = X * CHUNKS + chunk;
     return fxr::is_cell(Iw, Xc, Tmax) ? regions + fxr::region_offset((int)blockIdx.y, Tmax, Iw, Xc) : nullptr;
   };
@@ -521,7 +531,7 @@
   };
   if (I0 >= T || Jbase >= T || Jbase + kBlockColTiles - 1 < I0) {
     zero_regions();
-    return;
+    continue;
   }
   const int lane = threadIdx.x & 63;
   const int wave = __builtin_amdgcn_readfirstlane(threadIdx.x >> 6);
@@ -575,7 +585,7 @@
         if (!(jb + kColTilesPerWave - 1 < I || jb >= T))
           tim_wave_fp64<0>(ps, pd, bm, n, W, I, jb, kc, reinterpret_cast<double*>(&lds_own[wave][0][0]));
     zero_regions();
-    return;
+    continue;
   }
   const __amdgpu_buffer_rsrc_t deg_rsrc = __builtin_amdgcn_make_buffer_rsrc(
       (void*)(deg + d.pt_off), 0, (int)((unsigned int)n * 4u), 0x00020000);
@@ -664,7 +674,7 @@
     const uint64_t colmask = (n - j0 >= 64) ? ~0ull : ((1ull << (n - j0)) - 1ull);
     ownw &= colmask;
     if (diag) ownw &= ~(1ull << lane);
-    lds_own[wave][lane][(J - Jbase) & (kMfmaColTiles - 1)] = ownw;
+    if (NS != kK1NoStore || diag) lds_own[wave][lane][(J - Jbase) & (kMfmaColTiles - 1)] = ownw;
     degacc += __builtin_popcountll(ownw);
     const uint64_t trw_out = diag ? 0ull : (trw & rowmask);
     lds_tr[(J - Jbase) & (kMfmaColTiles - 1)][lane][wave] = trw_out;
@@ -821,7 +831,14 @@
       }
       if (CHUNKS > 1) __syncthreads();
     }
-    if (nact > 0) {
+    if (NS == kK1NoStore) {
+      if (Ja == I && Ja < Jc1) {
+        const uint64_t w = lds_own[wave][lane][(I - Jbase) & (kMfmaColTiles - 1)];
+        __builtin_amdgcn_raw_buffer_store_b64(u32x2{(unsigned int)w, (unsigned int)(w >> 32)}, bm_rsrc,
+                                              I * 64 + lane < n ? ((unsigned int)(I * 64 + lane) * (unsigned int)S + (unsigned int)I) * 8u : kOobOffset,
+                                              0, 0);
+      }
+    } else if (nact > 0) {
       const int kk = lane & 7, J = Jc0 + kk;
       const bool pad = J >= T, colok = (J >= Ja && J < Jc1) || pad;
       const unsigned int off0 = ((unsigned int)(I * 64 + (lane >> 3)) * (unsigned int)S + (unsigned int)J) * 8u;
@@ -835,7 +852,7 @@
       }
     }
     int wcount = 0;
-    {
+    if constexpr (NS != kK1Rebuild) {
       unsigned int vf = flags;
       if (I * 64 + 4 * h >= n) vf &= ~0xAAAAAAAAu;
       if (I * 64 + 32 + 4 * h >= n) vf &= ~0x55555555u;
@@ -873,7 +890,7 @@
       }
     }
     flags = 0;
-    {
+    if constexpr (NS != kK1Rebuild) {
       const int nreg = !region ? 0 : (wcount < kRegionItems ? wcount : kRegionItems);
       if (lane == 0 && region) region[0] = (unsigned long long)nreg;
       if (lane < nreg) region[1 + lane] = wbuf[lane];
@@ -894,20 +911,25 @@
   }
   if (rowvalid)
     __builtin_amdgcn_raw_ptr_buffer_atomic_add_i32(degacc, deg_rsrc, (unsigned int)(I * 64 + lane) * 4u, 0, 0);
-}
-
+  } while (NS == kK1Rebuild && (__syncthreads(), (lb += (int)gridDim.x) < nlb));
+}
+
+constexpr int kFixUpper = 1;
+template <bool NOSTORE>
 __global__ __launch_bounds__(256) void tim_fixup_group_kernel(const ProbDesc* __restrict__ descs, int batch,
                                                               const double* __restrict__ src,
                                                               const double* __restrict__ dst,
                                                               uint64_t* __restrict__ bitmap, double beta,
-                                                              const unsigned long long* __restrict__ work,
+                                                              unsigned long long* __restrict__ work,
                                                               const unsigned int* __restrict__ work_count,
                                                               ProbState* __restrict__ states,
                                                               int32_t* __restrict__ deg,
-                                                              const unsigned long long* __restrict__ regions,
+                                                              unsigned long long* __restrict__ regions,
                                                               int Tmax,
-                                                              const TimPrep* __restrict__ prep, int upper) {
+                                                              const TimPrep* __restrict__ prep, int mode) {
   TAIL_WAVE_PRIO();
+  constexpr bool nostore = NOSTORE;
+  const bool upper = nostore || (mode & kFixUpper) != 0;
   const int prob = blockIdx.y;
   const unsigned int total = work_count[prob];
   const TimPrep tpr = prep[prob];
@@ -947,8 +969,9 @@
   const int rq = (q & 3) + 8 * (q >> 2);
   __shared__ double row_pts[4][64][6];
   __shared__ __attribute__((aligned(16))) double col_pts[4][64][6];
-  auto resolve = [&](unsigned long long it, bool valid, auto staged, int tile, int slot) {
+  auto resolve = [&](unsigned long long it, bool valid, auto staged, int tile, int slot, unsigned long long* home) {
     constexpr bool STAGED = decltype(staged)::value;
+    const bool live = valid;
     int r = fxi::row0(it) + rq, col = fxi::col(it);
     valid = valid && r < n && col < n && r != col;
     r = valid ? r : (STAGED ? tile * 64 : 0);
@@ -967,8 +990,9 @@
     }
     unsigned int* wp = bm32 + 2 * ((int64_t)r * S + (col >> 6)) + ((col >> 5) & 1);
     const unsigned int bit = 1u << (col & 31);
+    const bool offdiag = (r >> 6) != (col >> 6);
     bool prov;
-    if (STAGED && (r >> 6) != (col >> 6)) {
+    if ((STAGED || nostore) && offdiag) {
       prov = fxi::bit(it, q);
     } else {
       prov = (*wp & bit) != 0u;
@@ -978,18 +1002,23 @@
     bool e = tim_edge_fast(ax, ay, az, bx, by, bz, kc, &unc, &shortp);
     e |= shortp;
     if (unc) e = tim_edge_exact(ax, ay, az, bx, by, bz, beta);
+    if constexpr (nostore) {
+      const uint64_t em = __builtin_amdgcn_ballot_w64(valid && e);
+      if (q == 0 && live) *home = fxi::pack((unsigned int)fxi::row0(it), (unsigned int)fxi::col(it), (unsigned int)(em >> (16 * sub)) & 0xffffu);
+    }
     if (!valid || prov == e) return;
-    atomicXor(wp, bit);
+    if (!nostore || !offdiag) atomicXor(wp, bit);
     atomicAdd(dg + r, e ? 1 : -1);
-    if ((r >> 6) != (col >> 6)) {
+    if (offdiag) {
       if (!upper) atomicXor(bm32 + 2 * ((int64_t)col * S + (r >> 6)) + ((r >> 5) & 1), 1u << (r & 31));
       atomicAdd(dg + col, e ? 1 : -1);
     }
   };
   __shared__ unsigned long long queue[4][2 * kRegionWords];
   static_assert(kRegionWords == 64, "one region = one 64-lane load");
+  __shared__ unsigned short qsrc[nostore ? 4 : 1][nostore ? 2 * kRegionWords : 1];
   const int T = W, nch = fxr::n_chunks(T);
-  auto round = [&](int cnt, int tile) {
+  auto round = [&](int cnt, int tile, unsigned long long* run) {
     if (lane < cnt) {
       const int col = min(fxi::col(queue[wave][lane]), n - 1);
       double* cp = col_pts[wave][lane];
@@ -1001,7 +1030,7 @@
 #pragma nounroll
     for (int base = 0; base < cnt; base += 4) {
       const int k = base + sub;
-      resolve(queue[wave][k], k < cnt, std::true_type(), tile, k);
+      resolve(queue[wave][k], k < cnt, std::true_type(), tile, k, nostore ? run + qsrc[nostore ? wave : 0][nostore ? k : 0] : nullptr);
     }
     __builtin_amdgcn_fence(__ATOMIC_ACQ_REL, "wavefront");
   };
@@ -1017,7 +1046,7 @@
         rp[3] = pd[3 * pr]; rp[4] = pd[3 * pr + 1]; rp[5] = pd[3 * pr + 2];
       }
       const int Xc0 = fxr::first_chunk(tile);
-      const unsigned long long* reg = regions + fxr::region_offset(prob, Tmax, tile, Xc0);
+      unsigned long long* reg = regions + fxr::region_offset(prob, Tmax, tile, Xc0);
       int qn = 0;
       unsigned long long mine = reg[lane];
       for (int Xc = Xc0; Xc < nch; ++Xc) {
@@ -1025,26 +1054,139 @@
         if (Xc + 1 < nch) mine = reg[(size_t)(Xc + 1 - Xc0) * kRegionWords + lane];
         const int cnt = min((int)__builtin_amdgcn_readfirstlane((unsigned int)cur), kRegionItems);
         if (cnt <= 0) continue;
-        if (lane >= 1 && lane <= cnt) queue[wave][qn + lane - 1] = cur;
+        if (lane >= 1 && lane <= cnt) {
+          queue[wave][qn + lane - 1] = cur;
+          if constexpr (nostore) qsrc[wave][qn + lane - 1] = (unsigned short)((Xc - Xc0) * kRegionWords + lane);
+        }
         qn += cnt;
         if (qn >= kRegionWords) {
           __builtin_amdgcn_fence(__ATOMIC_ACQ_REL, "wavefront");
-          round(kRegionWords, tile);
+          round(kRegionWords, tile, reg);
           qn -= kRegionWords;
           const unsigned long long moved = queue[wave][kRegionWords + lane];
+          unsigned short moved_src = 0;
+          if constexpr (nostore) moved_src = qsrc[wave][kRegionWords + lane];
           __builtin_amdgcn_fence(__ATOMIC_ACQ_REL, "wavefront");
-          if (lane < qn) queue[wave][lane] = moved;
+          if (lane < qn) {
+            queue[wave][lane] = moved;
+            if constexpr (nostore) qsrc[wave][lane] = moved_src;
+          }
         }
       }
       if (qn > 0) {
         __builtin_amdgcn_fence(__ATOMIC_ACQ_REL, "wavefront");
-        round(qn, tile);
+        round(qn, tile, reg);
+      }
+    }
+  }
+  unsigned long long* seg = work + (((size_t)tpr.seg_off_hi << 32) | (size_t)tpr.seg_off_lo);
+  const unsigned int ngrp = gridDim.x * 16;
+  for (unsigned int w = (blockIdx.x * 256 + threadIdx.x) >> 4; w < total; w += ngrp) resolve(seg[w], true, std::false_type(), 0, 0, seg + w);
+}
+
+__global__ __launch_bounds__(256) void tim_fixup_replay_kernel(const ProbDesc* __restrict__ descs,
+                                                               uint64_t* __restrict__ bitmap,
+                                                               const unsigned long long* __restrict__ work,
+                                                               const unsigned int* __restrict__ work_count,
+                                                               const ProbState* __restrict__ states,
+                                                               const unsigned long long* __restrict__ regions,
+                                                               int Tmax, const TimPrep* __restrict__ prep, int open_only) {
+  const int prob = blockIdx.y;
+  const TimPrep tpr = prep[prob];
+  const unsigned int total = work_count[prob];
+  if (!tpr.use_mfma || total > tpr.seg_cap || (open_only && states[prob].deg_closed)) return;
+  const ProbDesc d = descs[prob];
+  const int n = d.n, W = d.W, S = bm_stride(W), T = W, nch = fxr::n_chunks(T);
+  unsigned int* bm32 = reinterpret_cast<unsigned int*>(bitmap + d.bm_off);
+  const int lane = threadIdx.x & 63, q = lane & 15, sub = lane >> 4;
+  const int rq = fxi::row_of(q);
+  auto replay = [&](unsigned long long it, bool live) {
+    const int r = fxi::row0(it) + rq, col = fxi::col(it);
+    if (!live || r >= n || col >= n || r == col) return;
+    unsigned int* wp = bm32 + 2 * ((int64_t)r * S + (col >> 6)) + ((col >> 5) & 1);
+    const unsigned int bit = 1u << (col & 31);
+    if (((*wp & bit) != 0u) == fxi::bit(it, q)) return;
+    atomicXor(wp, bit);
+    if ((r >> 6) != (col >> 6)) atomicXor(bm32 + 2 * ((int64_t)col * S + (r >> 6)) + ((r >> 5) & 1), 1u << (r & 31));
+  };
+  const int wv = blockIdx.x * 4 + (int)(threadIdx.x >> 6), nwv = gridDim.x * 4;
+  for (int tile = wv; tile < T; tile += nwv) {
+    const int Xc0 = fxr::first_chunk(tile);
+    const unsigned long long* reg = regions + fxr::region_offset(prob, Tmax, tile, Xc0);
+    for (int Xc = Xc0; Xc < nch; ++Xc) {
+      const unsigned long long cur = reg[(size_t)(Xc - Xc0) * kRegionWords + lane];
+      const int cnt = min((int)__builtin_amdgcn_readfirstlane((unsigned int)cur), kRegionItems);
+      for (int base = 0; base < cnt; base += 4) {
+        const int k = base + sub;
+        const unsigned long long it = __shfl(cur, min(k + 1, 63));
+        replay(it, k < cnt);
       }
     }
   }
   const unsigned long long* seg = work + (((size_t)tpr.seg_off_hi << 32) | (size_t)tpr.seg_off_lo);
   const unsigned int ngrp = gridDim.x * 16;
-  for (unsigned int w = (blockIdx.x * 256 + threadIdx.x) >> 4; w < total; w += ngrp) resolve(seg[w], true, std::false_type(), 0, 0);
+  for (unsigned int w = (blockIdx.x * 256 + threadIdx.x) >> 4; w < total; w += ngrp) replay(seg[w], true);
+}
+
+__global__ __launch_bounds__(256) void tim_closure_pairs_kernel(const ProbDesc* __restrict__ descs,
+                                                                const double* __restrict__ src,
+                                                                const double* __restrict__ dst,
+                                                                uint64_t* __restrict__ part_pool ,
+                                                                const uint32_t* __restrict__ key_pool ,
+                                                                const int32_t* __restrict__ counters, double beta) {
+  TAIL_WAVE_PRIO();
+  const int m = counters[blockIdx.y];
+  if (m < 2) return;
+  const ProbDesc d = descs[blockIdx.y];
+  const double* ps = src + 3 * d.pt_off;
+  const double* pd = dst + 3 * d.pt_off;
+  const uint32_t* keys = key_pool + (size_t)blockIdx.y * kCoreCap;
+  uint64_t* part = part_pool + (size_t)blockIdx.y * kCoreCap * kCoreWords;
+  EdgeConst kc;
+  kc.beta = beta;
+  kc.beta2 = beta * beta;
+  kc.m2beta2 = -2.0 * kc.beta2;
+  kc.beta4 = kc.beta2 * kc.beta2;
+  kc.s_hat = 1.0;
+  __shared__ double row_pts[4][64][6];
+  const int lane = threadIdx.x & 63, wave = threadIdx.x >> 6;
+  const int ng = (m + 63) >> 6, units = ng * (ng + 1) / 2;
+  for (int u = blockIdx.x * 4 + wave; u < units; u += gridDim.x * 4) {
+    int A = 0, rem = u;
+    while (rem >= ng - A) {
+      rem -= ng - A;
+      ++A;
+    }
+    const int B = A + rem, ra = 64 * A + lane, rb = 64 * B + lane;
+    {
+      const int v = (int)(keys[min(ra, m - 1)] & 0xffffu);
+      double* rp = row_pts[wave][lane];
+      rp[0] = ps[3 * v]; rp[1] = ps[3 * v + 1]; rp[2] = ps[3 * v + 2];
+      rp[3] = pd[3 * v]; rp[4] = pd[3 * v + 1]; rp[5] = pd[3 * v + 2];
+    }
+    const int vb = (int)(keys[min(rb, m - 1)] & 0xffffu);
+    const double cx = ps[3 * vb], cy = ps[3 * vb + 1], cz = ps[3 * vb + 2];
+    const double ex = pd[3 * vb], ey = pd[3 * vb + 1], ez = pd[3 * vb + 2];
+    __builtin_amdgcn_fence(__ATOMIC_ACQ_REL, "wavefront");
+    uint64_t word = 0ull;
+    const int rows = min(64, m - 64 * A);
+    for (int r = 0; r < rows; ++r) {
+      const double* rp = row_pts[wave][r];
+      const double ax = cx - rp[0], ay = cy - rp[1], az = cz - rp[2], bx = ex - rp[3], by = ey - rp[4], bz = ez - rp[5];
+      bool unc, shortp;
+      bool e = tim_edge_fast(ax, ay, az, bx, by, bz, kc, &unc, &shortp);
+      e |= shortp;
+      if (unc) e = tim_edge_exact(ax, ay, az, bx, by, bz, beta);
+      const uint64_t mk = __builtin_amdgcn_ballot_w64(e && rb < m && 64 * A + r < rb);
+      word = lane == r ? mk : word;
+    }
+    if (ra < m) {
+      part[(size_t)ra * kCoreWords + B] = word;
+      if (A == B)
+        for (int Bz = 0; Bz < A; ++Bz) part[(size_t)ra * kCoreWords + Bz] = 0ull;
+    }
+    __builtin_amdgcn_fence(__ATOMIC_ACQ_REL, "wavefront");
+  }
 }
 
 constexpr int kMirrorRun = 8;
@@ -1178,13 +1320,23 @@
                        d_bitmap, d_state, phase == kTimMirrorOpen ? 1 : 0);
     return;
   }
+  const double beta = 2 * noise_bound * sqrt(cbar2);
+  if (phase == kTimClosurePairs) {
+    int32_t* counters = reinterpret_cast<int32_t*>(d_prep);
+    launch_degree_closure_order(s, d_desc, batch, d_deg, d_state, d_pk, counters);
+    const ClosurePools cp = degree_closure_pools(d_pk, batch);
+    hipLaunchKernelGGL(tim_closure_pairs_kernel, dim3(degree_closure_wgs(batch), batch), dim3(256), 0, s, d_desc, d_src, d_dst,
+                       cp.part, cp.keys, counters, beta);
+    return;
+  }
 #ifdef TEASER_K1_LAB
-  const bool upper = false;
+  const bool upper = false, nostore = false;
+  if (phase == kTimRebuild || phase == kTimRebuildOpen) return;
 #else
   const bool upper = (phase & kTimUpperOnly) != 0;
+  const bool nostore = (phase & kTimNoStore) != 0;
 #endif
-  phase &= ~kTimUpperOnly;
-  const double beta = 2 * noise_bound * sqrt(cbar2);
+  phase &= ~(kTimUpperOnly | kTimNoStore);
   TimPrep* prep = reinterpret_cast<TimPrep*>(d_prep);
   unsigned long long* work = reinterpret_cast<unsigned long long*>(d_work);
   unsigned int* work_count = reinterpret_cast<unsigned int*>(reinterpret_cast<char*>(d_prep) +
@@ -1214,7 +1366,7 @@
 #define TIM_K1_LAUNCH_OCC(PIPE, PLAIN, OCC, CHUNKS, ...)                                                                       \
   hipLaunchKernelGGL((tim_graph_mfma3_kernel<PIPE, PLAIN, OCC, CHUNKS, __VA_ARGS__>), dim3(tim_mfma_blocks(T, CHUNKS), batch), \
                      dim3(256), 0, s, d_desc, d_src, d_dst, (const void*)d_pk, prep, d_bitmap, beta, gyr, work, work_count,    \
-                     d_state, d_deg, regions, T)
+                     d_state, d_deg, regions, T, 0, 0)
 #ifdef TEASER_K1_LAB
 #define TIM_K1_LAB_CASE(PIPE, PLAIN)                             \
   if (lab.pipe == (PIPE ? 1 : 0) && lab.plain == (PLAIN ? 1 : 0)) { \
@@ -1234,7 +1386,9 @@
     }
 #undef TIM_K1_LAB_CASE
 #else
-    if (upper) {
+    if (nostore) {
+      TIM_K1_LAUNCH_OCC(kK1Pipe, kK1Plain, kK1Occ, kK1Chunks, false, false, kK1NoStore);
+    } else if (upper) {
       TIM_K1_LAUNCH_OCC(kK1Pipe, kK1Plain, kK1Occ, kK1Chunks, false);
     } else {
       TIM_K1_LAUNCH(kK1Pipe, kK1Plain, kK1Chunks);
@@ -1242,12 +1396,26 @@
 #endif
 #undef TIM_K1_LAUNCH
 #undef TIM_K1_LAUNCH_OCC
+#ifndef TEASER_K1_LAB
+  } else if (phase == kTimRebuild || phase == kTimRebuildOpen) {
+    const int gyr = (T + kMfmaRowTiles - 1) / kMfmaRowTiles, nlb = tim_mfma_blocks(T, kK1Chunks);
+    const int open_only = phase == kTimRebuildOpen ? 1 : 0;
+    hipLaunchKernelGGL((tim_graph_mfma3_kernel<kK1Pipe, kK1Plain, 2, kK1Chunks, true, false, kK1Rebuild>),
+                       dim3(open_only ? std::min(64, nlb) : nlb, batch), dim3(256), 0, s, d_desc, d_src, d_dst,
+                       (const void*)d_pk, prep, d_bitmap, beta, gyr, work, work_count, d_state, d_deg, regions, T, open_only, nlb);
+    hipLaunchKernelGGL(tim_fixup_replay_kernel, dim3((unsigned)std::max(4, ((T + 3) / 4 + 1) / 2), batch), dim3(256), 0, s,
+                       d_desc, d_bitmap, work, work_count, d_state, regions, T, prep, open_only);
+#endif
   } else {
     const int64_t forced_wgs = setting(S_FIXUP_WGS);
     const int64_t fix_wgs = forced_wgs > 0 ? forced_wgs : ((T + 1) / 2 + 3) / 4;
-    hipLaunchKernelGGL(tim_fixup_group_kernel, dim3((unsigned)std::max<int64_t>(4, fix_wgs), batch),
-                       dim3(256), 0, s, d_desc, batch, d_src, d_dst, d_bitmap, beta, work, work_count, d_state, d_deg,
-                       regions, T, prep, upper ? 1 : 0);
+    const dim3 fix_grid((unsigned)std::max<int64_t>(4, fix_wgs), batch);
+    if (nostore)
+      hipLaunchKernelGGL(tim_fixup_group_kernel<true>, fix_grid, dim3(256), 0, s, d_desc, batch, d_src, d_dst, d_bitmap, beta,
+                         work, work_count, d_state, d_deg, regions, T, prep, 0);
+    else
+      hipLaunchKernelGGL(tim_fixup_group_kernel<false>, fix_grid, dim3(256), 0, s, d_desc, batch, d_src, d_dst, d_bitmap, beta,
+                         work, work_count, d_state, d_deg, regions, T, prep, upper ? kFixUpper : 0);
   }
 }
 
diff --git a/teaser-plusplus_amd/csrc/kernels_heuristic.hip b/teaser-plusplus_amd/csrc/kernels_heuristic.hip
--- a/teaser-plusplus_amd/csrc/kernels_heuristic.hip
+++ b/teaser-plusplus_amd/csrc/kernels_heuristic.hip
@@ -556,8 +556,6 @@
   }
 }
 
-constexpr int kCoreCap = 2048;
-constexpr int kCoreWords = kCoreCap / 64;
 constexpr int kDegBins = kCoreCap;
 constexpr int kDegMaxW = 1024;
 constexpr int kDegThreads = 256;
@@ -1158,20 +1156,40 @@
   return (int64_t)std::max(batch, 1) * (2 * (int64_t)kCoreCap * kCoreWords * 8  + (int64_t)kCoreCap * 8);
 }
 
+int degree_closure_wgs(int batch) {
+  const int forced = (int)setting(S_DEG_CLOSURE_WGS);
+  return forced > 0 ? std::min(forced, 64) : std::max(1, std::min(16, 1024 / std::max(batch, 1)));
+}
+
+ClosurePools degree_closure_pools(void* d_scratch, int batch) {
+  ClosurePools cp;
+  cp.comp = reinterpret_cast<uint64_t*>(d_scratch);
+  cp.part = cp.comp + (size_t)batch * kCoreCap * kCoreWords;
+  cp.h = reinterpret_cast<int32_t*>(cp.part + (size_t)batch * kCoreCap * kCoreWords);
+  cp.keys = reinterpret_cast<uint32_t*>(cp.h + (size_t)batch * kCoreCap);
+  return cp;
+}
+
+void launch_degree_closure_order(hipStream_t s, const ProbDesc* d_desc, int batch, const int32_t* d_deg, ProbState* d_state,
+                                 void* d_scratch, int32_t* d_counters) {
+  hipLaunchKernelGGL(degree_closure_order_kernel, dim3(1, batch), dim3(kDegThreads), 0, s, d_desc, d_deg, d_state,
+                     degree_closure_pools(d_scratch, batch).keys, d_counters, batch);
+}
+
 void launch_degree_closure(hipStream_t s, const ProbDesc* d_desc, int batch, const uint64_t* d_bitmap,
                            const int32_t* d_deg, ProbState* d_state, int32_t* d_clique, void* d_scratch,
                            int32_t* d_counters) {
   if (batch <= 0) return;
-  const int forced = (int)setting(S_DEG_CLOSURE_WGS);
-  const int G = forced > 0 ? std::min(forced, 64) : std::max(1, std::min(16, 1024 / batch));
-  uint64_t* comp = reinterpret_cast<uint64_t*>(d_scratch);
-  uint64_t* part = comp + (size_t)batch * kCoreCap * kCoreWords;
-  int32_t* hp = reinterpret_cast<int32_t*>(part + (size_t)batch * kCoreCap * kCoreWords);
-  uint32_t* kp = reinterpret_cast<uint32_t*>(hp + (size_t)batch * kCoreCap);
-  hipLaunchKernelGGL(degree_closure_order_kernel, dim3(1, batch), dim3(kDegThreads), 0, s, d_desc, d_deg, d_state, kp,
-                     d_counters, batch);
-  hipLaunchKernelGGL(degree_closure_rows_kernel, dim3(G, batch), dim3(kDegThreads), 0, s, d_desc, d_bitmap, part, kp,
-                     d_counters, batch);
+  const int G = degree_closure_wgs(batch);
+  const ClosurePools cp = degree_closure_pools(d_scratch, batch);
+  uint64_t *comp = cp.comp, *part = cp.part;
+  int32_t* hp = cp.h;
+  uint32_t* kp = cp.keys;
+  if (d_bitmap) {
+    launch_degree_closure_order(s, d_desc, batch, d_deg, d_state, d_scratch, d_counters);
+    hipLaunchKernelGGL(degree_closure_rows_kernel, dim3(G, batch), dim3(kDegThreads), 0, s, d_desc, d_bitmap, part, kp,
+                       d_counters, batch);
+  }
   hipLaunchKernelGGL(degree_closure_symmetrise_kernel, dim3(std::min(G, 8), batch), dim3(kDegThreads), 0, s, part, comp, hp, kp,
                      d_counters, batch);
   hipLaunchKernelGGL(degree_closure_verdict_kernel, dim3(batch), dim3(kDegThreads), 0, s, d_desc, d_state, d_clique, comp, hp,
diff --git a/teaser-plusplus_amd/csrc/solver.hip b/teaser-plusplus_amd/csrc/solver.hip
--- a/teaser-plusplus_amd/csrc/solver.hip
+++ b/teaser-plusplus_amd/csrc/solver.hip
@@ -276,11 +276,15 @@
   const double* cur_dst = nullptr;
   bool have_graph = false;
   bool bm_lower_missing = false;
+  bool bm_rows_missing = false;
+  int64_t work_cap = 0;
+  int graph_route = 0;
+  int64_t rebuilt = 0;
 
   std::vector<uint64_t> bm_stage;
   SolverBuf d_desc, d_state, d_src, d_dst, d_bitmap, d_deg, d_clique, d_start_cliques, d_alive_a,
       d_alive_b, d_next_count, d_weights, d_rot_inl, d_trans_inl, d_tls_scratch, d_tim_off,
-      d_pk, d_prep, d_work, d_core, d_small;
+      d_pk, d_prep, d_work, d_core, d_small, d_deg_scratch;
   SolverBuf c_sel, c_colour, c_tent, c_xlist, c_list_a, c_list_b, c_counts, c_bits, c_class, c_mis;
   std::vector<int32_t> colour_x;
   SolverBuf x_order, x_src, x_dst, x_bitmap, x_ctrl, x_clique, x_arena, x_probs, x_probs2, x_keys, x_xbits, x_tasks;
@@ -296,6 +300,7 @@
   int last_unproven = 0;
   bool skip_heuristic_next = false;
   int closure_open_prev = 0;
+  int closure_batch_prev = 0;
   int heu_blocks = 0;
   int heu_rows = 0;
 
@@ -947,6 +952,12 @@
   return TEASER_HIP_OK;
 }
 
+void enqueue_graph_rebuild(teaser_hip_solver* h, int phase) {
+  launch_tim_graph_mfma(h->stream, phase, h->d_desc.as<ProbDesc>(), h->batch, h->max_n, h->total_w, nullptr, nullptr, h->d_pk.p,
+                        h->d_prep.p, h->d_work.p, h->work_cap, h->d_bitmap.as<uint64_t>(), h->d_state.as<ProbState>(),
+                        h->d_deg_scratch.as<int32_t>(), h->params.noise_bound, h->params.cbar2);
+}
+
 int32_t enqueue_heuristic_stage(teaser_hip_solver* h, int batch, int mode, bool record_stagger) {
   hipStream_t s = h->stream;
   const ProbDesc* dd = h->d_desc.as<ProbDesc>();
@@ -957,6 +968,7 @@
     if (h->bm_lower_missing)
       launch_tim_graph_mfma(s, kTimMirrorOpen, dd, batch, h->max_n, 0, nullptr, nullptr, nullptr, nullptr, nullptr, 0,
                             h->d_bitmap.as<uint64_t>(), ds, nullptr, 0.0, 0.0);
+    if (h->bm_rows_missing) enqueue_graph_rebuild(h, kTimRebuildOpen);
     int32_t* heu_trace = nullptr;
     if (setting(S_K4_DEBUG) && batch <= 4) {
       HIPCHK(h, h->s_e.ensure(sizeof(long long) * 8 * kMaxStarts * (size_t)batch));
@@ -1116,8 +1128,15 @@
   }
   const bool closure = need_graph && mode == TEASER_INLIER_PMC_EXACT && max_n <= 65536 && setting(S_DEG_CLOSURE) != 0 &&
                        !(setting(S_TAIL_SKIP) & 2);
-  const bool upper_k1 = mfma_k1 && closure;
-  if (need_graph) h->bm_lower_missing = upper_k1;
+  const bool nostore_k1 = mfma_k1 && closure && h->closure_batch_prev > 0 && h->closure_open_prev * 32 <= h->closure_batch_prev;
+  const bool upper_k1 = mfma_k1 && closure && !nostore_k1;
+  if (need_graph) {
+    h->bm_lower_missing = upper_k1;
+    h->bm_rows_missing = nostore_k1;
+    h->graph_route = nostore_k1 ? 2 : upper_k1 ? 1 : 0;
+    h->rebuilt = 0;
+    if (nostore_k1) HIPCHK(h, h->d_deg_scratch.ensure(4 * (size_t)total_n));
+  }
   const bool k1_only = mfma_k1 && h->is_lane && h->k1_stream && h->k1_kernel_only;
   if (mfma_k1 && h->is_lane && h->k1_stream && !k1_only) {
     s1 = h->k1_stream;
@@ -1153,7 +1172,7 @@
       launch_tim_graph(s, dd, batch, max_n, d_src, d_dst, h->d_bitmap.as<uint64_t>(), P.noise_bound,
                        P.cbar2, P.estimate_scaling ? 1 : 0, ds);
     } else {
-      const int64_t cap = tim_work_items(n, batch);
+      const int64_t cap = h->work_cap = tim_work_items(n, batch);
       const int64_t tail_skip = setting(S_TAIL_SKIP);
       for (int phase = 0; phase < 3; ++phase) {
         if ((phase == 2 && (tail_skip & 1)) || (phase == 0 && (tail_skip & 16))) continue;
@@ -1168,7 +1187,8 @@
         }
         {
           StageScope sc(h, phase == 1 ? ST_TIM : ST_TIMAUX, sp);
-          launch_tim_graph_mfma(sp, (upper_k1 && phase > 0) ? (phase | kTimUpperOnly) : phase, dd, batch, max_n, wo, d_src, d_dst, h->d_pk.p, h->d_prep.p,
+          const int store_flag = phase == 0 ? 0 : nostore_k1 ? kTimNoStore : upper_k1 ? kTimUpperOnly : 0;
+          launch_tim_graph_mfma(sp, phase | store_flag, dd, batch, max_n, wo, d_src, d_dst, h->d_pk.p, h->d_prep.p,
                                 h->d_work.p, cap, h->d_bitmap.as<uint64_t>(), ds, h->d_deg.as<int32_t>(),
                                 P.noise_bound, P.cbar2);
         }
@@ -1198,7 +1218,11 @@
     if (closure) {
       StageScope sc(h, ST_HEU);
       HIPCHK(h, h->d_core.ensure((size_t)degree_closure_scratch_bytes(batch)));
-      launch_degree_closure(s, dd, batch, h->d_bitmap.as<uint64_t>(), h->d_deg.as<int32_t>(), ds,
+      if (nostore_k1)
+        launch_tim_graph_mfma(s, kTimClosurePairs, dd, batch, max_n, wo, d_src, d_dst, h->d_core.p,
+                              h->d_next_count.as<int32_t>() + 2 * (size_t)batch, nullptr, 0, nullptr, ds, h->d_deg.as<int32_t>(),
+                              P.noise_bound, P.cbar2);
+      launch_degree_closure(s, dd, batch, nostore_k1 ? nullptr : h->d_bitmap.as<uint64_t>(), h->d_deg.as<int32_t>(), ds,
                             h->d_clique.as<int32_t>(), h->d_core.p, h->d_next_count.as<int32_t>() + 2 * (size_t)batch);
     }
     h->pend.closure = closure;
@@ -1265,6 +1289,8 @@
     }
     h->skip_heuristic_next = open == 0;
     h->closure_open_prev = open;
+    h->closure_batch_prev = batch;
+    if (h->bm_rows_missing) h->rebuilt += open;
   }
   for (int b = 0; b < batch; ++b) h->heu_size[(size_t)b] = h->states[(size_t)b].lb;
   if (setting(S_K4_DEBUG) && batch <= 4)
@@ -2023,6 +2049,16 @@
   return TEASER_HIP_OK;
 }
 
+static int32_t ensure_graph_rows(teaser_hip_solver* h) {
+  if (!h->bm_rows_missing) return TEASER_HIP_OK;
+  enqueue_graph_rebuild(h, kTimRebuild);
+  HIPCHK(h, hipGetLastError());
+  HIPCHK(h, hipStreamSynchronize(h->stream));
+  h->bm_rows_missing = false;
+  h->rebuilt += h->batch;
+  return TEASER_HIP_OK;
+}
+
 int32_t teaser_hip_get_inlier_graph_bitmap(teaser_hip_solver* h, int32_t problem, uint64_t* buf,
                                            int64_t* len) {
   CHECK_PROBLEM(h, problem);
@@ -2031,6 +2067,10 @@
     return len ? TEASER_HIP_OK : TEASER_HIP_ERR_BAD_ARG;
   }
   const ProbDesc& d = h->descs[(size_t)problem];
+  if (buf) {
+    const int32_t rc = ensure_graph_rows(h);
+    if (rc != TEASER_HIP_OK) return rc;
+  }
   if (buf && h->bm_lower_missing) {
     launch_tim_graph_mfma(h->stream, kTimMirror, h->d_desc.as<ProbDesc>(), h->batch, h->max_n, 0, nullptr, nullptr, nullptr,
                           nullptr, nullptr, 0, h->d_bitmap.as<uint64_t>(), h->d_state.as<ProbState>(), nullptr, 0.0, 0.0);
@@ -2068,7 +2108,18 @@
     if (len) *len = 0;
     return len ? TEASER_HIP_OK : TEASER_HIP_ERR_BAD_ARG;
   }
+  if (buf) {
+    const int32_t rc = ensure_graph_rows(h);
+    if (rc != TEASER_HIP_OK) return rc;
+  }
   return copy_out(h, h->d_bitmap.as<uint64_t>() + d.bm_off, (int64_t)d.n * bm_stride(d.W), buf, len);
+}
+
+int32_t teaser_hip_get_graph_route(teaser_hip_solver* h, int32_t problem, int32_t* route, int64_t* rebuilt) {
+  CHECK_PROBLEM(h, problem);
+  if (route) *route = h->have_graph ? h->graph_route : 0;
+  if (rebuilt) *rebuilt = h->have_graph ? h->rebuilt : 0;
+  return TEASER_HIP_OK;
 }
 
 int32_t teaser_hip_get_degrees(teaser_hip_solver* h, int32_t problem, int32_t* buf, int64_t* len) {
@@ -2254,7 +2305,8 @@
   if (rc != TEASER_HIP_OK) return rc;
   h->batch = 0;
   h->pend.spec_bounds = false;
-  h->bm_lower_missing = false;
+  h->bm_lower_missing = h->bm_rows_missing = false;
+  h->graph_route = 0;
   ProbState& st = h->states[0];
   HIPCHK(h, h->d_desc.ensure(sizeof(ProbDesc)));
   HIPCHK(h, h->d_state.ensure(sizeof(ProbState)));
```

Result: faster. 123,200, median of 6 (+6.7%).
